# Mingrui-Yu/A-Simple-Stereo-SLAM-System-with-Deep-Loop-Closing

Measured on AMD Instinct MI355X. Metric: stereo frames/sec (ORB+match+LCD+BA-build) @1241x376, higher is better.
Workload: dtype u8/int32 (ORB, Hamming), f32 via f16x3 / bf16x6 split products on the matrix cores with f32 accumulate (CALC conv1 / conv2, DB scan), f64 (triangulation, BA)

## Files before the change

### a-simple-stereo-slam-system-with-deep-loop-closing_amd/csrc/orb_engine.hip

```cpp
#include <math.h>
#include <stdlib.h>
#include <string.h>

#include <vector>

#include "common.h"
#include "orb_plan.h"

namespace myslam_hip {

void launch_resize(const ResizeArgs& a, int batch, hipStream_t s);
void launch_resize_chain(const ResizeArgs* lv, int n, int batch, hipStream_t s);
bool resize_is_little(const ResizeArgs& a, int batch);
int resize_chain_max();
int pyr_head_levels();
void launch_pyr_head(const ResizeArgs* lv, int n, int rows, int cols, uint8_t* dst0, int dpitch0, size_t dstride0, int b0, int batch,
                     uint32_t* p0, int n0, uint32_t* p1, int n1, uint32_t* p2, int n2, uint32_t* p3, int n3, hipStream_t s);
void launch_blur(const BlurArgs& a, int batch, hipStream_t s);
bool blur_uses_strips(const BlurArgs& a);
bool resize_uses_strips(const ResizeArgs& a);
void launch_fast(const OrbPlan& P, const uint8_t* pyr, size_t pyrStride, const uint8_t* maskPyr, uint32_t* cand,
                 int32_t* candCount, const uint32_t* statPrev, uint32_t* statCur, int forceMode, int batch, hipStream_t s);
bool launch_octree(const OrbPlan& P, const uint32_t* cand, const int32_t* candCount, uint32_t* sortbuf, const uint32_t* octTab, uint32_t* selOut,
                   int32_t* selCount, int32_t* status, int batch, uint16_t* order, hipStream_t s, const BlurArgs* blurLv, int nBlur);
bool describe_uses_tile_order(bool have_order, int detectOnly, int batch);
void launch_describe(const OrbPlan& P, const uint8_t* pyr, const uint8_t* blur, size_t pyrStride, const uint32_t* selOut,
                     const int32_t* selCount, myslam_keypoint* kps, uint8_t* desc, int32_t* counts, int32_t* status,
                     int cap, int detectOnly, int batch, uint16_t* order, bool order_ready, int blocks_per_cu, hipStream_t s);
void launch_screen(const OrbPlan& P, const uint8_t* pyr, myslam_keypoint* kin, int n, myslam_keypoint* kout, uint8_t* keep,
                   hipStream_t s);
void launch_calc_desc(const OrbPlan& P, const uint8_t* blur, const myslam_keypoint* kps, int n, uint8_t* desc, hipStream_t s);
void launch_unpack_cands(const uint32_t* cand, int n, int32_t* xs, int32_t* ys, int32_t* sc, hipStream_t s);
void launch_blur_levels(const BlurArgs* lv, int n, int batch, hipStream_t s);
bool blur_mfma_tables(int w, int h, const int q[7], std::vector<uint4>& tab, size_t& offH, size_t& offV);
void blur_mfma_ident(std::vector<uint4>& tab, size_t& offI);
void launch_zero_u32(uint32_t* p0, int n0, uint32_t* p1, int n1, uint32_t* p2, int n2, uint32_t* p3, int n3, hipStream_t s);
void launch_ingest_clear(const uint8_t* src, int rows, int cols, int step, size_t sstride, uint8_t* dst, int dpitch, size_t dstride, int batch,
                         uint32_t* p0, int n0, uint32_t* p1, int n1, uint32_t* p2, int n2, uint32_t* p3, int n3, hipStream_t s);
void launch_ingest(const uint8_t* src, int rows, int cols, int step, size_t sstride, uint8_t* dst, int dpitch,
                   size_t dstride, int batch, hipStream_t s);

static inline int cv_round(float v) { return (int)lrintf(v); }
static inline size_t align_up(size_t v, size_t a) { return (v + a - 1) / a * a; }

void gauss_q8(int kind, int q[7]) {
    if (kind == 1) { const int t[7] = {8, 28, 56, 72, 56, 28, 8}; memcpy(q, t, sizeof(t)); return; }
    double g[7], sum = 0;
    for (int i = 0; i < 7; i++) { double x = i - 3; g[i] = exp(-(x * x) / 8.0); sum += g[i]; }
    for (int i = 0; i < 7; i++) q[i] = (int)lrint(g[i] / sum * 256.0);
}

[[maybe_unused]] static void resize_tables(int ssize, int dsize, bool is_x, std::vector<int32_t>& ofs, std::vector<int16_t>& coef) {
    const double inv_scale = (double)dsize / ssize;
    const double scale = 1. / inv_scale;
    ofs.resize(dsize); coef.resize(2 * dsize);
    for (int d = 0; d < dsize; d++) {
        float f = (float)((d + 0.5) * scale - 0.5);
        int s = (int)floorf(f);
        f -= s;
        if (is_x) {
            if (s < 0) { f = 0; s = 0; }
            if (s >= ssize - 1) { f = 0; s = ssize - 1; }
        }
        ofs[d] = s;
        coef[2 * d] = (int16_t)cv_round((1.f - f) * 2048.f);
        coef[2 * d + 1] = (int16_t)cv_round(f * 2048.f);
    }
}

template <typename T>
static int dev_alloc(T*& p, size_t n) {
    if (p) { (void)hipFree(p); p = nullptr; }
    if (n == 0) return MYSLAM_OK;
    MYSLAM_HIP_CHECK(hipMalloc((void**)&p, n * sizeof(T)));
    return MYSLAM_OK;
}

}

using namespace myslam_hip;

struct myslam_orb {
    int nfeatures, nlevels, iniTh, minTh;
    float scaleFactor;
    std::vector<float> scale, invScale;
    std::vector<int> nPerLevel;
    int umax[16];
    hipStream_t stream = nullptr;
    hipStream_t aux = nullptr;
    hipEvent_t evFork = nullptr, evJoin = nullptr;
    hipEvent_t evUserFast = nullptr;
    hipEvent_t evUserGate = nullptr;

    int rows = 0, cols = 0;
    OrbPlan full{}, det{};

    int batchCap = 0;
    bool maskAlloc = false;
    uint8_t *d_pyr = nullptr, *d_blur = nullptr, *d_mask = nullptr;
    uint32_t* d_cand = nullptr;
    uint32_t* d_sort = nullptr;
    int32_t *d_candCount = nullptr, *d_selCount = nullptr, *d_status = nullptr;
    uint32_t* d_sel = nullptr;
    uint16_t* d_order = nullptr;
    uint32_t* d_octTab = nullptr;
    uint32_t* d_stripTab = nullptr;
    uint32_t* d_fastStat = nullptr; int fastFlip = 0;
    int optFastMode = -1;
    int optInternalStream = 1;
    int optCopyInput = 0;
    int optStopAfter = 0;
    int tapsSet = 0, taps[7] = {0};
    int optSideBlocksPerCu = 0;
    int optBlurMfma = 0;
    uint4* d_blurTab = nullptr; bool blurTabValid = false; size_t blurOffI = 0, blurOffH[MAXL] = {0}, blurOffV[MAXL] = {0}; bool blurLvOk[MAXL] = {false}; int blurVconst = 0;
    int ensure_blur_tables();

    struct HostGraph { hipGraphExec_t exec = nullptr; hipGraph_t graph = nullptr; uint64_t gen = 0; int rows = 0, cols = 0, step = 0, dcap = 0, calls = 0; bool mask = false; };
    HostGraph hostGraph[2][2];
    uint64_t gen = 1;
    struct Clear { uint32_t* p[4]; int n[4]; } clr{{nullptr, nullptr, nullptr, nullptr}, {0, 0, 0, 0}};
    hipStream_t hostStream = nullptr;
    uint8_t* h_pin = nullptr; size_t pinBytes = 0;
    int ensure_pin(size_t bytes);
    void drop_host_graphs();
    uint8_t *d_stageImg = nullptr, *d_stageMask = nullptr; size_t stageImgBytes = 0, stageMaskBytes = 0;
    myslam_keypoint *d_stageKps = nullptr, *d_stageKps2 = nullptr; uint8_t* d_stageDesc = nullptr; uint8_t* d_stageKeep = nullptr;
    int32_t* d_stageCounts = nullptr; int stageCap = 0;
    uint8_t* d_stageOut = nullptr; size_t stageOutBytes = 0, stageDescOff = 0;

    int make_tables();
    int make_plan(int r, int c);
    int ensure(int batch, int r, int c, bool needMask);
    int ensure_stage(size_t imgBytes, size_t maskBytes, int cap);
    int build_pyramids(const uint8_t* d_imgs, int batch, int step, size_t stride, const uint8_t* d_masks, int nlev);
    ResizeArgs level_resize_args(uint8_t* base, int l) const;
    BlurArgs level_blur_args(int l) const;
    int blur_levels(int batch, int nlev, hipStream_t s);
    void fill_blur_args(BlurArgs* lv, int nlev) const;
    int run_fast(const OrbPlan& P, const uint8_t* maskPyr, int batch);
    int run_batch(const uint8_t* d_imgs, int batch, int r, int c, int step, size_t stride, const uint8_t* d_masks,
                  myslam_keypoint* d_kps, uint8_t* d_desc, int32_t* d_counts, int32_t* d_stat, int cap, bool detectOnly);
    void free_all();
};

int myslam_orb::make_tables() {
    scale.assign(nlevels, 1.f); invScale.assign(nlevels, 1.f); nPerLevel.assign(nlevels, 0);
    for (int i = 1; i < nlevels; i++) scale[i] = scale[i - 1] * scaleFactor;
    for (int i = 0; i < nlevels; i++) invScale[i] = 1.0f / scale[i];
    float factor = 1.0f / scaleFactor;
    float nDesired = nfeatures * (1 - factor) / (1 - (float)pow((double)factor, (double)nlevels));
    int sum = 0;
    for (int l = 0; l < nlevels - 1; l++) { nPerLevel[l] = cv_round(nDesired); sum += nPerLevel[l]; nDesired *= factor; }
    nPerLevel[nlevels - 1] = std::max(nfeatures - sum, 0);
    int v, v0, vmax = (int)floor(HALF_PATCH * sqrtf(2.f) / 2 + 1), vmin = (int)ceil(HALF_PATCH * sqrtf(2.f) / 2);
    const double hp2 = HALF_PATCH * HALF_PATCH;
    for (v = 0; v < 16; v++) umax[v] = 0;
    for (v = 0; v <= vmax; ++v) umax[v] = (int)lrint(sqrt(hp2 - v * v));
    for (v = HALF_PATCH, v0 = 0; v >= vmin; --v) { while (umax[v0] == umax[v0 + 1]) ++v0; umax[v] = v0; ++v0; }
    const int expect[16] = {15, 15, 15, 15, 14, 14, 14, 13, 13, 12, 11, 10, 9, 8, 6, 3};
    for (v = 0; v < 16; v++) if (umax[v] != expect[v]) return MYSLAM_ERR_INVALID;
    return MYSLAM_OK;
}

static int ceil_log2(int v) { int b = 0; while ((1 << b) < v) b++; return b; }

int myslam_orb::make_plan(int r, int c) {
    OrbPlan P{};
    P.nlevels = nlevels; P.rows = r; P.cols = c; P.iniTh = iniTh; P.minTh = minTh;
    size_t imgOff = 0, keyOff = 0; int cellBase = 0, outBase = 0, stripBase = 0;
    for (int l = 0; l < nlevels; l++) {
        LevelGeom& g = P.lv[l];
        g.w = cv_round((float)c * invScale[l]);
        g.h = cv_round((float)r * invScale[l]);
        if (g.w < 1 || g.h < 1) return MYSLAM_ERR_UNSUPPORTED;
        g.pitch = (int)align_up(g.w, 64);
        g.maxBX = g.w - EDGE_THRESHOLD + 3; g.maxBY = g.h - EDGE_THRESHOLD + 3;
        const float width = (float)(g.maxBX - MIN_BORDER), height = (float)(g.maxBY - MIN_BORDER);
        const float W = 30;
        g.nCols = (int)(width / W); g.nRows = (int)(height / W);
        if (g.nCols < 1 || g.nRows < 1) return MYSLAM_ERR_UNSUPPORTED;
        g.wCell = (int)ceilf(width / g.nCols); g.hCell = (int)ceilf(height / g.nRows);
        if (g.wCell > MAX_CELL || g.hCell > MAX_CELL) return MYSLAM_ERR_UNSUPPORTED;
        if (g.maxBX + 3 > 4095 + MIN_BORDER || g.maxBY + 3 > 4095 + MIN_BORDER) return MYSLAM_ERR_UNSUPPORTED;
        g.cellBase = cellBase; cellBase += g.nCols * g.nRows;
        g.stripBase = stripBase; stripBase += g.nRows * ((g.nCols + 3) / 4);
        g.N = nPerLevel[l];
        g.nIni = (int)roundf((float)(g.maxBX - MIN_BORDER) / (g.maxBY - MIN_BORDER));
        if (g.nIni < 1 || g.nIni > 64) return MYSLAM_ERR_UNSUPPORTED;
        g.hX = (float)(g.maxBX - MIN_BORDER) / g.nIni;
        const int rootW = (int)ceilf(g.hX) + 2, H = g.maxBY - MIN_BORDER;
        g.ndepth = std::min(MAX_DEPTH, ceil_log2(std::max(rootW, H)) + 2);
        g.sortDepth = 0;
        while (g.sortDepth + 1 <= g.ndepth && (g.nIni << (2 * (g.sortDepth + 1))) <= 1024) g.sortDepth++;
        g.keyCap = (int)std::min<size_t>(262143, std::max<size_t>(256, (size_t)((g.w + 1) / 2) * ((g.h + 1) / 2)));
        g.nodeCap = (std::max(g.N + 4, 4 * g.nIni + 4) + 3) & ~3;
        if (g.nodeCap > 4092) return MYSLAM_ERR_UNSUPPORTED;
        g.outBase = outBase; outBase += g.nodeCap;
        g.scale = scale[l];
        g.scaledPatch = (float)(int)(PATCH_SIZE * scale[l]);
        g.imgOff = imgOff; imgOff += align_up((size_t)g.pitch * align_up((size_t)g.h, 8), 256);
        g.keyOff = keyOff; keyOff += g.keyCap;
    }
    for (int l = 0; l < MAXL; l++) P.stripBaseOf[l] = l < P.nlevels ? P.lv[l].stripBase : INT32_MAX;
    P.ncells = cellBase; P.nstrips = stripBase; P.totalKeyCap = (int)keyOff; P.totalOut = outBase; P.pyrBytes = imgOff;
    {
        std::vector<uint32_t> tab;
        for (int l = 0; l < nlevels; l++) {
            LevelGeom& g = P.lv[l];
            g.tabX = g.maxBX - MIN_BORDER + 8; g.tabY = g.maxBY - MIN_BORDER + 8; g.tabOff = (int)tab.size();
            tab.resize(tab.size() + 2 * (size_t)(g.tabX + g.tabY), 0u);
            uint32_t* xcode = tab.data() + g.tabOff; uint32_t* ycode = xcode + g.tabX;
            uint32_t* xcell = ycode + g.tabY; uint32_t* ycell = xcell + g.tabX;
            for (int px = 0; px < g.tabX; px++) {
                int r = (int)((float)px / g.hX);
                r = std::min(std::max(r, 0), g.nIni - 1);
                int UL = (int)(g.hX * (float)r), UR = (int)(g.hX * (float)(r + 1));
                uint32_t code = (uint32_t)r << ROOT_SHIFT;
                for (int k = 1; k <= g.ndepth; k++) {
                    const int mid = UL + ((UR - UL + 1) >> 1);
                    const uint32_t d = px >= mid;
                    code |= d << (ROOT_SHIFT - 2 * k);
                    if (d) UL = mid; else UR = mid;
                }
                xcode[px] = code;
                xcell[px] = (uint32_t)(std::max(px - 3, 0) / g.wCell);
            }
            for (int py = 0; py < g.tabY; py++) {
                int UL = 0, BR = g.maxBY - MIN_BORDER;
                uint32_t code = 0;
                for (int k = 1; k <= g.ndepth; k++) {
                    const int mid = UL + ((BR - UL + 1) >> 1);
                    const uint32_t d = py >= mid;
                    code |= (d << 1) << (ROOT_SHIFT - 2 * k);
                    if (d) UL = mid; else BR = mid;
                }
                ycode[py] = code;
                ycell[py] = (uint32_t)((std::max(py - 3, 0) / g.hCell) * g.nCols);
            }
        }
        int rc = dev_alloc(d_octTab, tab.size());
        if (rc) return rc;
        if ((rc = upload_table(d_octTab, tab.data(), tab.size() * sizeof(uint32_t)))) return rc;
    }
    {
        std::vector<uint32_t> st((size_t)P.nstrips * 8, 0u);
        for (int l = 0; l < nlevels; l++) {
            const LevelGeom& g = P.lv[l];
            const int spr = (g.nCols + 3) / 4;
            for (int strip = 0; strip < g.nRows * spr; strip++) {
                uint32_t* e = st.data() + (size_t)(g.stripBase + strip) * 8;
                const int ci = strip / spr, cj0 = (strip - ci * spr) * 4;
                const int iniY = MIN_BORDER + ci * g.hCell;
                int ncell = 0, pairs = 0; uint32_t wcs = 0; int hr = 0;
                if (iniY < g.maxBY - 3) {
                    hr = std::min(iniY + g.hCell + 6, g.maxBY) - iniY;
                    const int hc = hr - 6;
                    if (hc > 0)
                        for (int c = 0; c < 4; c++) {
                            const int cj = cj0 + c, iniX = MIN_BORDER + cj * g.wCell;
                            int wc = 0;
                            if (cj < g.nCols && iniX < g.maxBX - 6) wc = std::max(0, std::min(iniX + g.wCell + 6, g.maxBX) - iniX - 6);
                            if (wc > 0) ncell = c + 1;
                            wcs |= (uint32_t)wc << (8 * c);
                            pairs += ((wc + 1) >> 1) * hc;
                        }
                }
                if (ncell == 0) wcs = 0;
                e[0] = (uint32_t)l | ((uint32_t)ci << 8) | ((uint32_t)cj0 << 16) | ((uint32_t)ncell << 24);
                e[1] = (uint32_t)iniY | ((uint32_t)hr << 16);
                e[2] = (uint32_t)(MIN_BORDER + cj0 * g.wCell) | ((uint32_t)g.wCell << 16);
                e[3] = wcs; e[4] = (uint32_t)g.pitch; e[5] = (uint32_t)pairs;
                e[6] = (uint32_t)(g.imgOff & 0xffffffffu); e[7] = (uint32_t)(g.imgOff >> 32);
            }
        }
        int rc = dev_alloc(d_stripTab, st.size());
        if (rc) return rc;
        if ((rc = upload_table(d_stripTab, st.data(), st.size() * sizeof(uint32_t)))) return rc;
        P.stripTab = d_stripTab;
    }
    full = P;
    det = P;
    det.nlevels = 1;
    det.ncells = P.lv[0].nCols * P.lv[0].nRows;
    det.nstrips = P.lv[0].nRows * ((P.lv[0].nCols + 3) / 4);
    det.lv[0].N = nfeatures;
    det.lv[0].nodeCap = (std::max(nfeatures + 4, 4 * P.lv[0].nIni + 4) + 3) & ~3;
    if (det.lv[0].nodeCap > 4092) return MYSLAM_ERR_UNSUPPORTED;
    det.lv[0].outBase = 0;
    det.totalOut = det.lv[0].nodeCap;
    rows = r; cols = c;
    return MYSLAM_OK;
}

int myslam_orb::ensure(int batch, int r, int c, bool needMask) {
    if (r != rows || c != cols) {
        MYSLAM_HIP_CHECK(hipStreamSynchronize(stream));
        int rc = make_plan(r, c);
        if (rc) { rows = cols = 0; return rc; }
        batchCap = 0; gen++; blurTabValid = false;
    }
    const int detOut = det.totalOut;
    const size_t selPer = (size_t)std::max(full.totalOut, detOut);
    if (batch > batchCap) {
        MYSLAM_HIP_CHECK(hipStreamSynchronize(stream));
        gen++;
        int rc;
        if ((rc = dev_alloc(d_pyr, (size_t)batch * full.pyrBytes + 64))) return rc;
        if ((rc = dev_alloc(d_blur, (size_t)batch * full.pyrBytes + 4096))) return rc;
        if ((rc = dev_alloc(d_cand, (size_t)batch * full.totalKeyCap))) return rc;
        if ((rc = dev_alloc(d_sort, (size_t)batch * full.totalKeyCap * 2))) return rc;
        if ((rc = dev_alloc(d_candCount, (size_t)batch * MAXL))) return rc;
        if ((rc = dev_alloc(d_selCount, (size_t)batch * MAXL))) return rc;
        if ((rc = dev_alloc(d_status, (size_t)batch))) return rc;
        if ((rc = dev_alloc(d_sel, (size_t)batch * selPer))) return rc;
        if ((rc = dev_alloc(d_order, (size_t)batch * selPer))) return rc;
        if ((rc = dev_alloc(d_mask, 0))) return rc;
        maskAlloc = false;
        batchCap = batch;
    }
    if (needMask && !maskAlloc) {
        int rc = dev_alloc(d_mask, (size_t)batchCap * full.pyrBytes + 64);
        if (rc) return rc;
        maskAlloc = true;
    }
    return MYSLAM_OK;
}

int myslam_orb::build_pyramids(const uint8_t* d_imgs, int batch, int step, size_t stride, const uint8_t* d_masks, int nlev) {
    const OrbPlan& P = full;
    for (int pass = 0; pass < (d_masks ? 2 : 1); pass++) {
        uint8_t* base = pass ? d_mask : d_pyr;
        const uint8_t* src = pass ? d_masks : d_imgs;
        const int n0 = pass ? 0 : P.ext0N;
        int l = 1;
        const int nhead = std::min(pyr_head_levels(), nlev - 1);
        if (nhead >= 1 && batch > n0 && (size_t)batch * P.lv[1].w * P.lv[1].h < (size_t)1500000) {
            ScopedProf sp(P_RESIZE, stream);
            ResizeArgs grp[3];
            for (int j = 0; j < nhead; j++) grp[j] = level_resize_args(base, 1 + j);
            grp[0].src = src; grp[0].spitch = step; grp[0].sstride = stride;
            const bool c0 = pass == 0 && clr.n[0] > 0;
            launch_pyr_head(grp, nhead, P.rows, P.cols, base + P.lv[0].imgOff, P.lv[0].pitch, P.pyrBytes, n0, batch,
                            c0 ? clr.p[0] : nullptr, c0 ? clr.n[0] : 0, c0 ? clr.p[1] : nullptr, c0 ? clr.n[1] : 0, c0 ? clr.p[2] : nullptr,
                            c0 ? clr.n[2] : 0, c0 ? clr.p[3] : nullptr, c0 ? clr.n[3] : 0, stream);
            if (c0) clr.n[0] = 0;
            l = 1 + nhead;
        } else if (batch > n0) {
            uint8_t* dst0 = base + (size_t)n0 * P.pyrBytes + P.lv[0].imgOff;
            if (pass == 0 && clr.n[0] > 0) {
                launch_ingest_clear(src + (size_t)n0 * stride, P.rows, P.cols, step, stride, dst0, P.lv[0].pitch, P.pyrBytes, batch - n0,
                                    clr.p[0], clr.n[0], clr.p[1], clr.n[1], clr.p[2], clr.n[2], clr.p[3], clr.n[3], stream);
                clr.n[0] = 0;
            } else {
                launch_ingest(src + (size_t)n0 * stride, P.rows, P.cols, step, stride, dst0, P.lv[0].pitch, P.pyrBytes, batch - n0, stream);
            }
        }
        for (; l < nlev;) {
            ScopedProf sp(P_RESIZE, stream);
            ResizeArgs a = level_resize_args(base, l);
            if (l == 1 && n0 > 0) { a.src0 = d_imgs; a.spitch0 = step; a.sstride0 = stride; a.n0 = n0; }
            ResizeArgs grp[4]; int ng = 0;
            const int gmax = resize_chain_max();
            if (gmax > 1 && resize_is_little(a, batch)) {
                static const double kEvals[4] = {1, 5, 21, 85};
                double evals = (double)batch * a.dw * a.dh;
                grp[ng++] = a;
                while (ng < gmax && l + ng < nlev) {
                    const ResizeArgs nx = level_resize_args(base, l + ng);
                    evals += (double)batch * nx.dw * nx.dh * kEvals[ng];
                    if (!resize_is_little(nx, batch) || evals > 6e6) break;
                    grp[ng++] = nx;
                }
            }
            if (ng > 1) { launch_resize_chain(grp, ng, batch, stream); l += ng; }
            else { launch_resize(a, batch, stream); l++; }
        }
    }
    return MYSLAM_OK;
}
ResizeArgs myslam_orb::level_resize_args(uint8_t* base, int l) const {
    const OrbPlan& P = full;
    ResizeArgs a;
    a.src = base + P.lv[l - 1].imgOff; a.sw = P.lv[l - 1].w; a.sh = P.lv[l - 1].h; a.spitch = P.lv[l - 1].pitch; a.sstride = P.pyrBytes;
    a.src0 = nullptr; a.spitch0 = 0; a.n0 = 0; a.sstride0 = 0;
    a.dst = base + P.lv[l].imgOff; a.dw = P.lv[l].w; a.dh = P.lv[l].h; a.dpitch = P.lv[l].pitch; a.dstride = P.pyrBytes;
    a.scale_x = 1. / ((double)a.dw / a.sw); a.scale_y = 1. / ((double)a.dh / a.sh);
    return a;
}
int myslam_orb::ensure_blur_tables() {
    if (blurTabValid) return MYSLAM_OK;
    std::vector<uint4> tab;
    int q[7];
    if (tapsSet) memcpy(q, taps, sizeof(q)); else gauss_q8(0, q);
    int sum = 0;
    for (int t = 0; t < 7; t++) sum += q[t];
    blurVconst = sum * 128 * sum + 32768;
    blur_mfma_ident(tab, blurOffI);
    for (int l = 0; l < full.nlevels; l++) blurLvOk[l] = blur_mfma_tables(full.lv[l].w, full.lv[l].h, q, tab, blurOffH[l], blurOffV[l]);
    MYSLAM_HIP_CHECK(hipStreamSynchronize(stream));
    int rc = dev_alloc(d_blurTab, tab.size());
    if (rc) return rc;
    if ((rc = upload_table(d_blurTab, tab.data(), tab.size() * sizeof(uint4)))) return rc;
    blurTabValid = true; gen++;
    return MYSLAM_OK;
}

BlurArgs myslam_orb::level_blur_args(int l) const {
    const OrbPlan& P = full;
    BlurArgs a;
    a.src = d_pyr + P.lv[l].imgOff; a.dst = d_blur + P.lv[l].imgOff;
    a.w = P.lv[l].w; a.h = P.lv[l].h; a.spitch = a.dpitch = P.lv[l].pitch; a.sstride = a.dstride = P.pyrBytes;
    a.src0 = nullptr; a.spitch0 = 0; a.n0 = 0; a.sstride0 = 0;
    a.dtiled = 1;
    if (tapsSet) memcpy(a.q, taps, sizeof(taps)); else gauss_q8(0, a.q);
    if (optBlurMfma && blurTabValid && blurLvOk[l]) { a.tabH = d_blurTab + blurOffH[l]; a.tabV = d_blurTab + blurOffV[l]; a.ident = d_blurTab + blurOffI; a.vconst = blurVconst; }
    return a;
}
void myslam_orb::fill_blur_args(BlurArgs* lv, int nlev) const {
    const OrbPlan& P = full;
    for (int l = 0; l < nlev; l++) {
        lv[l] = level_blur_args(l);
        if (l == 0 && P.ext0N > 0) { lv[l].src0 = P.ext0; lv[l].spitch0 = P.ext0Pitch; lv[l].sstride0 = P.ext0Stride; lv[l].n0 = P.ext0N; }
    }
}
int myslam_orb::blur_levels(int batch, int nlev, hipStream_t stream) {
    BlurArgs lv[MAXL];
    fill_blur_args(lv, nlev);
    ScopedProf sp(P_BLUR, stream);
    launch_blur_levels(lv, nlev, batch, stream);
    return MYSLAM_OK;
}

int myslam_orb::run_batch(const uint8_t* d_imgs, int batch, int r, int c, int step, size_t stride, const uint8_t* d_masks,
                          myslam_keypoint* d_kps, uint8_t* d_desc, int32_t* d_counts, int32_t* d_stat, int cap, bool detectOnly) {
    if (!d_imgs || batch <= 0 || r <= 0 || c <= 0 || step < c || cap <= 0 || !d_kps || !d_counts) return MYSLAM_ERR_INVALID;
    if (!detectOnly && !d_desc) return MYSLAM_ERR_INVALID;
    int rc = ensure(batch, r, c, d_masks != nullptr);
    if (rc) return rc;
    if (optBlurMfma && !detectOnly && (rc = ensure_blur_tables())) return rc;
    const OrbPlan& P = detectOnly ? det : full;
    int32_t* stat = d_stat ? d_stat : d_status;
    if (!d_fastStat) {
        MYSLAM_HIP_CHECK(hipMalloc((void**)&d_fastStat, sizeof(uint32_t) * 2 * MAXL * 4));
        MYSLAM_HIP_CHECK(hipMemsetAsync(d_fastStat, 0, sizeof(uint32_t) * 2 * MAXL * 4, stream));
    }
    clr = {{reinterpret_cast<uint32_t*>(d_candCount), reinterpret_cast<uint32_t*>(d_selCount), reinterpret_cast<uint32_t*>(stat), d_fastStat + (size_t)fastFlip * MAXL * 4},
           {batch * MAXL, batch * MAXL, batch, MAXL * 4}};
    const int stop = optStopAfter;
    {
        int n0 = 0;
        if (!optCopyInput && stop == 0 && batch > 1 && full.nlevels >= 1 && stride >= (size_t)r * (size_t)step) {
            bool ok = blur_uses_strips(level_blur_args(0));
            if (full.nlevels > 1) ok = ok && resize_uses_strips(level_resize_args(d_pyr, 1));
            if (ok) n0 = batch - 1;
        }
        full.ext0 = det.ext0 = d_imgs; full.ext0Stride = det.ext0Stride = stride; full.ext0Pitch = det.ext0Pitch = step; full.ext0N = det.ext0N = n0;
    }
    if (stop == 1) {
        launch_ingest_clear(d_imgs, full.rows, full.cols, step, stride, d_pyr + full.lv[0].imgOff, full.lv[0].pitch, full.pyrBytes, batch,
                            clr.p[0], clr.n[0], clr.p[1], clr.n[1], clr.p[2], clr.n[2], clr.p[3], clr.n[3], stream);
        clr.n[0] = 0;
        return MYSLAM_OK;
    }
    if ((rc = build_pyramids(d_imgs, batch, step, stride, d_masks, P.nlevels))) return rc;
    if (stop == 2) return MYSLAM_OK;
    hipStreamCaptureStatus capst = hipStreamCaptureStatusNone;
    if (stream && hipStreamIsCapturing(stream, &capst) != hipSuccess) { (void)hipGetLastError(); capst = hipStreamCaptureStatusNone; }
    const int aux_mode = capst == hipStreamCaptureStatusActive ? 0 : optInternalStream;
    const bool fork = aux_mode > 0 && !detectOnly && stop == 0;
    if (fork && !aux) {
        MYSLAM_HIP_CHECK(hipStreamCreateWithFlags(&aux, hipStreamNonBlocking));
        MYSLAM_HIP_CHECK(hipEventCreateWithFlags(&evFork, hipEventDisableTiming));
        MYSLAM_HIP_CHECK(hipEventCreateWithFlags(&evJoin, hipEventDisableTiming));
    }
    auto fork_blur = [&]() -> int {
        MYSLAM_HIP_CHECK(hipEventRecord(evFork, stream));
        MYSLAM_HIP_CHECK(hipStreamWaitEvent(aux, evFork, 0));
        int rc2 = blur_levels(batch, P.nlevels, aux);
        if (rc2) return rc2;
        MYSLAM_HIP_CHECK(hipEventRecord(evJoin, aux));
        return MYSLAM_OK;
    };
    if (fork && aux_mode == 2 && (rc = fork_blur())) return rc;
    if (evUserGate) MYSLAM_HIP_CHECK(hipStreamWaitEvent(stream, evUserGate, 0));
    if ((rc = run_fast(P, d_masks ? d_mask : nullptr, batch))) return rc;
    if (evUserFast) MYSLAM_HIP_CHECK(hipEventRecord(evUserFast, stream));
    if (fork && aux_mode != 2 && (rc = fork_blur())) return rc;
    bool blurred = false;
    {
        ScopedProf sp(P_OCTREE, stream);
        BlurArgs blv[MAXL];
        const bool tryBlur = !fork && !detectOnly && stop == 0 && !optBlurMfma;
        if (tryBlur) fill_blur_args(blv, P.nlevels);
        blurred = launch_octree(P, d_cand, d_candCount, d_sort, d_octTab, d_sel, d_selCount, stat, batch,
                                describe_uses_tile_order(d_order != nullptr, detectOnly ? 1 : 0, batch) ? d_order : nullptr, stream,
                                tryBlur ? blv : nullptr, tryBlur ? P.nlevels : 0);
    }
    if (stop == 3) return MYSLAM_OK;
    if (fork) MYSLAM_HIP_CHECK(hipStreamWaitEvent(stream, evJoin, 0));
    else if (!detectOnly && !blurred && (rc = blur_levels(batch, P.nlevels, stream))) return rc;
    if (stop == 4) return MYSLAM_OK;
    {
        ScopedProf sp(P_DESC, stream);
        launch_describe(P, d_pyr, d_blur, full.pyrBytes, d_sel, d_selCount, d_kps, d_desc, d_counts, stat, cap,
                        detectOnly ? 1 : 0, batch, d_order, true, optSideBlocksPerCu, stream);
    }
    MYSLAM_HIP_CHECK(hipGetLastError());
    return MYSLAM_OK;
}

int myslam_orb::run_fast(const OrbPlan& P, const uint8_t* maskPyr, int batch) {
    uint32_t* cur = d_fastStat + (size_t)fastFlip * MAXL * 4;
    const uint32_t* prev = d_fastStat + (size_t)(fastFlip ^ 1) * MAXL * 4;
    fastFlip ^= 1;
    ScopedProf sp(P_FAST, stream);
    launch_fast(P, d_pyr, full.pyrBytes, maskPyr, d_cand, d_candCount, prev, cur, optFastMode, batch, stream);
    return MYSLAM_OK;
}

int myslam_orb::ensure_pin(size_t bytes) {
    if (bytes <= pinBytes) return MYSLAM_OK;
    if (h_pin) { (void)hipHostFree(h_pin); h_pin = nullptr; pinBytes = 0; }
    gen++;
    const size_t want = (bytes + (bytes >> 2) + 4095) & ~(size_t)4095;
    MYSLAM_HIP_CHECK(hipHostMalloc((void**)&h_pin, want));
    pinBytes = want;
    return MYSLAM_OK;
}

void myslam_orb::drop_host_graphs() {
    for (auto& row : hostGraph)
        for (auto& g : row) { if (g.exec) (void)hipGraphExecDestroy(g.exec); if (g.graph) (void)hipGraphDestroy(g.graph); g = HostGraph(); }
}

int myslam_orb::ensure_stage(size_t imgBytes, size_t maskBytes, int cap) {
    if (imgBytes > stageImgBytes) { gen++; int rc = dev_alloc(d_stageImg, imgBytes); if (rc) return rc; stageImgBytes = imgBytes; }
    if (maskBytes > stageMaskBytes) { gen++; int rc = dev_alloc(d_stageMask, maskBytes); if (rc) return rc; stageMaskBytes = maskBytes; }
    if (cap > stageCap) {
        gen++;
        int rc;
        const size_t oK = 256, oD = oK + (((size_t)cap * sizeof(myslam_keypoint) + 255) & ~(size_t)255), total = oD + (size_t)cap * 32;
        if ((rc = dev_alloc(d_stageOut, total))) return rc;
        stageOutBytes = total; stageDescOff = oD;
        d_stageCounts = reinterpret_cast<int32_t*>(d_stageOut);
        d_stageKps = reinterpret_cast<myslam_keypoint*>(d_stageOut + oK);
        d_stageDesc = d_stageOut + oD;
        if ((rc = dev_alloc(d_stageKps2, (size_t)cap))) return rc;
        if ((rc = dev_alloc(d_stageKeep, (size_t)cap))) return rc;
        stageCap = cap;
    }
    return MYSLAM_OK;
}

void myslam_orb::free_all() {
    void* ptrs[] = {d_blurTab, d_fastStat, d_octTab, d_stripTab, d_pyr, d_blur, d_mask, d_cand, d_sort, d_candCount, d_selCount, d_status, d_sel, d_order, d_stageImg, d_stageMask,
                    d_stageOut, d_stageKps2, d_stageKeep};
    for (void* p : ptrs) if (p) (void)hipFree(p);
    if (aux) { (void)hipStreamSynchronize(aux); (void)hipStreamDestroy(aux); (void)hipEventDestroy(evFork); (void)hipEventDestroy(evJoin); aux = nullptr; }
    drop_host_graphs();
    if (hostStream) { (void)hipStreamSynchronize(hostStream); (void)hipStreamDestroy(hostStream); hostStream = nullptr; }
    if (h_pin) { (void)hipHostFree(h_pin); h_pin = nullptr; pinBytes = 0; }
}

extern "C" {

int myslam_orb_create(myslam_orb** out, int nfeatures, float scale_factor, int nlevels, int ini_th_fast, int min_th_fast) {
    if (!out || nfeatures < 1 || nlevels < 1 || nlevels > MAXL || !(scale_factor > 1.0f) || ini_th_fast < 0 ||
        min_th_fast < 1 || min_th_fast > ini_th_fast || ini_th_fast > 255 || scale_factor > 2.5f)
        return MYSLAM_ERR_INVALID;
    int ndev = 0;
    if (hipGetDeviceCount(&ndev) != hipSuccess || ndev < 1) return MYSLAM_ERR_HIP;
    myslam_orb* h = new myslam_orb();
    h->nfeatures = nfeatures; h->scaleFactor = scale_factor; h->nlevels = nlevels; h->iniTh = ini_th_fast; h->minTh = min_th_fast;
    int rc = h->make_tables();
    if (rc) { delete h; return rc; }
    *out = h;
    return MYSLAM_OK;
}

int myslam_orb_destroy(myslam_orb* h) {
    if (!h) return MYSLAM_ERR_INVALID;
    (void)hipStreamSynchronize(h->stream);
    h->free_all();
    delete h;
    return MYSLAM_OK;
}

int myslam_orb_set_stream(myslam_orb* h, void* s) {
    if (!h) return MYSLAM_ERR_INVALID;
    (void)hipStreamSynchronize(h->stream);
    h->stream = (hipStream_t)s; h->gen++;
    return MYSLAM_OK;
}

int myslam_orb_set_fast_event(myslam_orb* h, void* ev) {
    if (!h) return MYSLAM_ERR_INVALID;
    h->evUserFast = (hipEvent_t)ev; h->gen++;
    return MYSLAM_OK;
}

int myslam_orb_set_fast_gate(myslam_orb* h, void* ev) {
    if (!h) return MYSLAM_ERR_INVALID;
    h->evUserGate = (hipEvent_t)ev; h->gen++;
    return MYSLAM_OK;
}

int myslam_orb_set_option(myslam_orb* h, int option, int value) {
    if (!h) return MYSLAM_ERR_INVALID;
    h->gen++;
    switch (option) {
        case MYSLAM_ORB_OPT_FAST_MODE: if (value < -1 || value > 1) return MYSLAM_ERR_INVALID; h->optFastMode = value; return MYSLAM_OK;
        case MYSLAM_ORB_OPT_INTERNAL_STREAM: if (value < 0 || value > 2) return MYSLAM_ERR_INVALID; h->optInternalStream = value; return MYSLAM_OK;
        case MYSLAM_ORB_OPT_COPY_INPUT: if (value < 0 || value > 1) return MYSLAM_ERR_INVALID; h->optCopyInput = value; return MYSLAM_OK;
        case MYSLAM_ORB_OPT_STOP_AFTER: if (value < 0 || value > 4) return MYSLAM_ERR_INVALID; h->optStopAfter = value; return MYSLAM_OK;
        case MYSLAM_ORB_OPT_BLUR_MFMA: if (value < 0 || value > 1) return MYSLAM_ERR_INVALID; h->optBlurMfma = value; return MYSLAM_OK;
        case MYSLAM_ORB_OPT_SIDE_BLOCKS_PER_CU: if (value < 0 || value > 64) return MYSLAM_ERR_INVALID; h->optSideBlocksPerCu = value; return MYSLAM_OK;
    }
    return MYSLAM_ERR_INVALID;
}

int myslam_orb_set_gauss_taps(myslam_orb* h, const int32_t* q7) {
    if (!h) return MYSLAM_ERR_INVALID;
    h->blurTabValid = false;
    if (!q7) { h->tapsSet = 0; h->gen++; return MYSLAM_OK; }
    int sum = 0;
    for (int i = 0; i < 7; i++) { if (q7[i] < 0 || q7[i] > 255) return MYSLAM_ERR_INVALID; sum += q7[i]; }
    if (sum < 1 || sum > 257) return MYSLAM_ERR_INVALID;
    for (int i = 0; i < 7; i++) h->taps[i] = q7[i];
    h->tapsSet = 1; h->gen++;
    return MYSLAM_OK;
}

int myslam_orb_get_tables(const myslam_orb* h, float* scale, float* inv_scale, int* fpl, int* umax16) {
    if (!h) return MYSLAM_ERR_INVALID;
    for (int i = 0; i < h->nlevels; i++) {
        if (scale) scale[i] = h->scale[i];
        if (inv_scale) inv_scale[i] = h->invScale[i];
        if (fpl) fpl[i] = h->nPerLevel[i];
    }
    if (umax16) for (int i = 0; i < 16; i++) umax16[i] = h->umax[i];
    return MYSLAM_OK;
}

int myslam_orb_max_keypoints(const myslam_orb* h) {
    if (!h) return MYSLAM_ERR_INVALID;
    int s = 0;
    for (int l = 0; l < h->nlevels; l++) s += std::max(h->nPerLevel[l] + 3, 32);
    return std::max(s, std::max(h->nfeatures + 3, 32));
}

int myslam_orb_max_keypoints_for(const myslam_orb* h, int rows, int cols) {
    if (!h || rows < 1 || cols < 1) return MYSLAM_ERR_INVALID;
    int s = 0, first = 0;
    for (int l = 0; l < h->nlevels; l++) {
        const int w = cv_round((float)cols * h->invScale[l]), hh = cv_round((float)rows * h->invScale[l]);
        const int bx = w - EDGE_THRESHOLD + 3 - MIN_BORDER, by = hh - EDGE_THRESHOLD + 3 - MIN_BORDER;
        const int nIni = (bx > 0 && by > 0) ? std::max(1, (int)roundf((float)bx / (float)by)) : 1;
        s += std::max(h->nPerLevel[l] + 3, 4 * nIni);
        if (l == 0) first = std::max(h->nfeatures + 3, 4 * nIni);
    }
    return std::max(std::max(s, first), 32);
}

int myslam_orb_detect_and_compute_batch(myslam_orb* h, const uint8_t* d_imgs, int batch, int rows, int cols, int step,
                                        size_t img_stride, const uint8_t* d_masks, myslam_keypoint* d_kps, uint8_t* d_desc,
                                        int32_t* d_counts, int32_t* d_status, int cap) {
    if (!h) return MYSLAM_ERR_INVALID;
    return h->run_batch(d_imgs, batch, rows, cols, step, img_stride, d_masks, d_kps, d_desc, d_counts, d_status, cap, false);
}

int myslam_orb_detect_batch(myslam_orb* h, const uint8_t* d_imgs, int batch, int rows, int cols, int step, size_t img_stride,
                            const uint8_t* d_masks, myslam_keypoint* d_kps, int32_t* d_counts, int32_t* d_status, int cap) {
    if (!h) return MYSLAM_ERR_INVALID;
    return h->run_batch(d_imgs, batch, rows, cols, step, img_stride, d_masks, d_kps, nullptr, d_counts, d_status, cap, true);
}

static int host_extract(myslam_orb* h, const uint8_t* img, int rows, int cols, int step, const uint8_t* mask, int mask_step,
                        myslam_keypoint* kps, uint8_t* desc, int cap, int* n, bool detectOnly) {
    if (!h || !n) return MYSLAM_ERR_INVALID;
    *n = 0;
    if (!img || rows <= 0 || cols <= 0) return MYSLAM_OK;
    if (detectOnly && !mask) {  }
    if (step < cols || cap <= 0 || !kps || (!detectOnly && !desc)) return MYSLAM_ERR_INVALID;
    if (mask && mask_step < cols) return MYSLAM_ERR_INVALID;
    int rc = h->ensure(1, rows, cols, mask != nullptr);
    if (rc) return rc;
    if (mask && mask_step != step) return MYSLAM_ERR_INVALID;
    const int dcap = std::max(cap, std::max(h->full.totalOut, h->det.totalOut));
    const size_t imgBytes = (size_t)rows * step, maskBytes = mask ? imgBytes : 0;
    if ((rc = h->ensure_stage(imgBytes, maskBytes, dcap))) return rc;
    if (h->optBlurMfma && !detectOnly && (rc = h->ensure_blur_tables())) return rc;
    const size_t oOut = (imgBytes + maskBytes + 255) & ~(size_t)255, oCnt = oOut, oKps = oOut + 256, oDesc = oOut + h->stageDescOff;
    const size_t outBytes = detectOnly ? 256 + sizeof(myslam_keypoint) * (size_t)dcap : h->stageDescOff + (size_t)32 * dcap;
    if ((rc = h->ensure_pin(oOut + h->stageOutBytes))) return rc;
    hipStream_t caller = h->stream;
    if (!caller) {
        if (!h->hostStream) { MYSLAM_HIP_CHECK(hipStreamCreateWithFlags(&h->hostStream, hipStreamNonBlocking)); h->gen++; }
        MYSLAM_HIP_CHECK(hipStreamSynchronize(nullptr));
    }
    hipStream_t hs = caller ? caller : h->hostStream;
    struct Swap { myslam_orb* h; hipStream_t keep; ~Swap() { h->stream = keep; } } swap{h, caller};
    h->stream = hs;
    memcpy(h->h_pin, img, imgBytes);
    if (mask) memcpy(h->h_pin + imgBytes, mask, maskBytes);
    auto enqueue = [&]() -> int {
        MYSLAM_HIP_CHECK(hipMemcpyAsync(h->d_stageImg, h->h_pin, imgBytes, hipMemcpyHostToDevice, hs));
        if (mask) MYSLAM_HIP_CHECK(hipMemcpyAsync(h->d_stageMask, h->h_pin + imgBytes, maskBytes, hipMemcpyHostToDevice, hs));
        int r2 = h->run_batch(h->d_stageImg, 1, rows, cols, step, imgBytes, mask ? h->d_stageMask : nullptr,
                              h->d_stageKps, h->d_stageDesc, h->d_stageCounts, h->d_stageCounts + 1, dcap, detectOnly);
        if (r2) return r2;
        MYSLAM_HIP_CHECK(hipMemcpyAsync(h->h_pin + oOut, h->d_stageOut, outBytes, hipMemcpyDeviceToHost, hs));
        return MYSLAM_OK;
    };
    const bool graphable = !prof_is_on() && !h->evUserGate && !h->evUserFast && h->optStopAfter == 0;
    myslam_orb::HostGraph& G = h->hostGraph[detectOnly ? 1 : 0][h->fastFlip & 1];
    const bool same = G.gen == h->gen && G.rows == rows && G.cols == cols && G.step == step && G.dcap == dcap && G.mask == (mask != nullptr);
    if (!same) { if (G.exec) (void)hipGraphExecDestroy(G.exec); if (G.graph) (void)hipGraphDestroy(G.graph); G = myslam_orb::HostGraph(); G.gen = h->gen; G.rows = rows; G.cols = cols; G.step = step; G.dcap = dcap; G.mask = mask != nullptr; }
    bool done = false;
    if (graphable && G.exec) {
        if (hipGraphLaunch(G.exec, hs) == hipSuccess) { h->fastFlip ^= 1; done = true; }
        else { (void)hipGetLastError(); (void)hipGraphExecDestroy(G.exec); G.exec = nullptr; if (G.graph) { (void)hipGraphDestroy(G.graph); G.graph = nullptr; } G.calls = -1000000; }
    } else if (graphable && G.calls >= 1) {
        const int flip0 = h->fastFlip;
        if (hipStreamBeginCapture(hs, hipStreamCaptureModeThreadLocal) == hipSuccess) {
            const int r2 = enqueue();
            hipGraph_t graph = nullptr;
            const hipError_t e = hipStreamEndCapture(hs, &graph);
            if (r2 == MYSLAM_OK && e == hipSuccess && graph && hipGraphInstantiate(&G.exec, graph, nullptr, nullptr, 0) == hipSuccess &&
                hipGraphLaunch(G.exec, hs) == hipSuccess) {
                done = true; G.graph = graph;
            } else {
                (void)hipGetLastError();
                if (G.exec) { (void)hipGraphExecDestroy(G.exec); G.exec = nullptr; }
                if (graph) (void)hipGraphDestroy(graph);
                G.calls = -1000000; h->fastFlip = flip0;
            }
        } else {
            (void)hipGetLastError(); G.calls = -1000000;
        }
    }
    if (!done && (rc = enqueue())) return rc;
    G.calls++;
    MYSLAM_HIP_CHECK(hipStreamSynchronize(hs));
    int32_t res[2];
    memcpy(res, h->h_pin + oCnt, sizeof(res));
    if (res[1] != 0) return res[1];
    if (res[0] > cap) { *n = res[0]; return MYSLAM_ERR_CAPACITY; }
    memcpy(kps, h->h_pin + oKps, sizeof(myslam_keypoint) * (size_t)res[0]);
    if (!detectOnly) memcpy(desc, h->h_pin + oDesc, (size_t)32 * res[0]);
    *n = res[0];
    return MYSLAM_OK;
}

int myslam_orb_detect_and_compute(myslam_orb* h, const uint8_t* img, int rows, int cols, int step, const uint8_t* mask,
                                  int mask_step, myslam_keypoint* kps, uint8_t* desc, int cap, int* n) {
    return host_extract(h, img, rows, cols, step, mask, mask_step, kps, desc, cap, n, false);
}

int myslam_orb_detect(myslam_orb* h, const uint8_t* img, int rows, int cols, int step, const uint8_t* mask, int mask_step,
                      myslam_keypoint* kps, int cap, int* n) {
    return host_extract(h, img, rows, cols, step, mask, mask_step, kps, nullptr, cap, n, true);
}

static int host_pyramid(myslam_orb* h, const uint8_t* img, int rows, int cols, int step, int ncap) {
    int rc = h->ensure(1, rows, cols, false);
    if (rc) return rc;
    if ((rc = h->ensure_stage((size_t)rows * step, 0, ncap))) return rc;
    MYSLAM_HIP_CHECK(hipMemcpyAsync(h->d_stageImg, img, (size_t)rows * step, hipMemcpyHostToDevice, h->stream));
    h->full.ext0N = h->det.ext0N = 0;
    return h->build_pyramids(h->d_stageImg, 1, step, (size_t)rows * step, nullptr, h->nlevels);
}

int myslam_orb_screen_and_compute_params(myslam_orb* h, const uint8_t* img, int rows, int cols, int step,
                                         myslam_keypoint* kps_in, int n_in, myslam_keypoint* kps_out, int cap, int* n_out) {
    if (!h || !n_out) return MYSLAM_ERR_INVALID;
    *n_out = 0;
    if (!img || rows <= 0 || cols <= 0 || n_in <= 0) return MYSLAM_OK;
    if (!kps_in || !kps_out || step < cols) return MYSLAM_ERR_INVALID;
    for (int i = 0; i < n_in; i++) if (kps_in[i].octave < 0 || kps_in[i].octave >= h->nlevels) return MYSLAM_ERR_INVALID;
    int rc = host_pyramid(h, img, rows, cols, step, n_in);
    if (rc) return rc;
    MYSLAM_HIP_CHECK(hipMemcpyAsync(h->d_stageKps, kps_in, sizeof(myslam_keypoint) * n_in, hipMemcpyHostToDevice, h->stream));
    {
        ScopedProf sp(P_SCREEN, h->stream);
        launch_screen(h->full, h->d_pyr, h->d_stageKps, n_in, h->d_stageKps2, h->d_stageKeep, h->stream);
    }
    std::vector<myslam_keypoint> tmp(n_in);
    std::vector<uint8_t> keep(n_in);
    MYSLAM_HIP_CHECK(hipMemcpyAsync(kps_in, h->d_stageKps, sizeof(myslam_keypoint) * n_in, hipMemcpyDeviceToHost, h->stream));
    MYSLAM_HIP_CHECK(hipMemcpyAsync(tmp.data(), h->d_stageKps2, sizeof(myslam_keypoint) * n_in, hipMemcpyDeviceToHost, h->stream));
    MYSLAM_HIP_CHECK(hipMemcpyAsync(keep.data(), h->d_stageKeep, n_in, hipMemcpyDeviceToHost, h->stream));
    MYSLAM_HIP_CHECK(hipStreamSynchronize(h->stream));
    int m = 0;
    for (int i = 0; i < n_in; i++)
        if (keep[i]) { if (m >= cap) return MYSLAM_ERR_CAPACITY; kps_out[m++] = tmp[i]; }
    *n_out = m;
    return MYSLAM_OK;
}

int myslam_orb_calc_descriptors(myslam_orb* h, const uint8_t* img, int rows, int cols, int step, const myslam_keypoint* kps,
                                int n, uint8_t* desc) {
    if (!h) return MYSLAM_ERR_INVALID;
    if (!img || rows <= 0 || cols <= 0 || n <= 0) return MYSLAM_OK;
    if (!kps || !desc || step < cols) return MYSLAM_ERR_INVALID;
    for (int i = 0; i < n; i++) if (kps[i].octave < 0 || kps[i].octave >= h->nlevels) return MYSLAM_ERR_INVALID;
    int rc = host_pyramid(h, img, rows, cols, step, n);
    if (rc) return rc;
    if ((rc = h->blur_levels(1, h->nlevels, h->stream))) return rc;
    MYSLAM_HIP_CHECK(hipMemcpyAsync(h->d_stageKps, kps, sizeof(myslam_keypoint) * n, hipMemcpyHostToDevice, h->stream));
    {
        ScopedProf sp(P_DESC, h->stream);
        launch_calc_desc(h->full, h->d_blur, h->d_stageKps, n, h->d_stageDesc, h->stream);
    }
    MYSLAM_HIP_CHECK(hipMemcpyAsync(desc, h->d_stageDesc, (size_t)32 * n, hipMemcpyDeviceToHost, h->stream));
    MYSLAM_HIP_CHECK(hipStreamSynchronize(h->stream));
    return MYSLAM_OK;
}

static int download_tiled_plane(const uint8_t* d_plane, const LevelGeom& g, uint8_t* out, int out_step, hipStream_t stream) {
    std::vector<uint8_t> tmp((size_t)g.pitch * align_up((size_t)g.h, 8));
    MYSLAM_HIP_CHECK(hipMemcpyAsync(tmp.data(), d_plane, tmp.size(), hipMemcpyDeviceToHost, stream));
    MYSLAM_HIP_CHECK(hipStreamSynchronize(stream));
    for (int y = 0; y < g.h; y++)
        for (int x = 0; x < g.w; x++) out[(size_t)y * out_step + x] = tmp[tiled_off(x, y, g.pitch)];
    return MYSLAM_OK;
}

int myslam_orb_debug_pyramid(myslam_orb* h, const uint8_t* img, int rows, int cols, int step, int level, int blurred,
                             uint8_t* out, int out_step, int* w, int* hgt) {
    if (!h || !img || level < 0 || level >= h->nlevels) return MYSLAM_ERR_INVALID;
    int rc = host_pyramid(h, img, rows, cols, step, 16);
    if (rc) return rc;
    if (blurred && (rc = h->blur_levels(1, h->nlevels, h->stream))) return rc;
    const LevelGeom& g = h->full.lv[level];
    if (w) *w = g.w;
    if (hgt) *hgt = g.h;
    if (out) {
        if (out_step < g.w) return MYSLAM_ERR_INVALID;
        if (blurred) return download_tiled_plane(h->d_blur + g.imgOff, g, out, out_step, h->stream);
        MYSLAM_HIP_CHECK(hipMemcpy2DAsync(out, out_step, h->d_pyr + g.imgOff, g.pitch, g.w, g.h, hipMemcpyDeviceToHost, h->stream));
    }
    MYSLAM_HIP_CHECK(hipStreamSynchronize(h->stream));
    return MYSLAM_OK;
}

int myslam_orb_debug_candidates(myslam_orb* h, const uint8_t* img, int rows, int cols, int step, const uint8_t* mask,
                                int mask_step, int level, int32_t* xs, int32_t* ys, int32_t* scores, int cap, int* n) {
    if (!h || !img || !n || level < 0 || level >= h->nlevels) return MYSLAM_ERR_INVALID;
    if (mask && mask_step != step) return MYSLAM_ERR_INVALID;
    int rc = h->ensure(1, rows, cols, mask != nullptr);
    if (rc) return rc;
    if ((rc = h->ensure_stage((size_t)rows * step, mask ? (size_t)rows * step : 0, 16))) return rc;
    MYSLAM_HIP_CHECK(hipMemcpyAsync(h->d_stageImg, img, (size_t)rows * step, hipMemcpyHostToDevice, h->stream));
    if (mask) MYSLAM_HIP_CHECK(hipMemcpyAsync(h->d_stageMask, mask, (size_t)rows * step, hipMemcpyHostToDevice, h->stream));
    if (!h->d_fastStat) {
        MYSLAM_HIP_CHECK(hipMalloc((void**)&h->d_fastStat, sizeof(uint32_t) * 2 * MAXL * 4));
        MYSLAM_HIP_CHECK(hipMemsetAsync(h->d_fastStat, 0, sizeof(uint32_t) * 2 * MAXL * 4, h->stream));
    }
    launch_zero_u32(reinterpret_cast<uint32_t*>(h->d_candCount), MAXL, h->d_fastStat + (size_t)h->fastFlip * MAXL * 4, MAXL * 4, nullptr, 0, nullptr, 0, h->stream);
    h->full.ext0N = h->det.ext0N = 0;
    if ((rc = h->build_pyramids(h->d_stageImg, 1, step, (size_t)rows * step, mask ? h->d_stageMask : nullptr, h->nlevels))) return rc;
    if ((rc = h->run_fast(h->full, mask ? h->d_mask : nullptr, 1))) return rc;
    int32_t counts[MAXL];
    MYSLAM_HIP_CHECK(hipMemcpyAsync(counts, h->d_candCount, sizeof(counts), hipMemcpyDeviceToHost, h->stream));
    MYSLAM_HIP_CHECK(hipStreamSynchronize(h->stream));
    const LevelGeom& g = h->full.lv[level];
    *n = counts[level];
    if (counts[level] > g.keyCap || counts[level] > cap) return MYSLAM_ERR_CAPACITY;
    int32_t* d_tmp = nullptr;
    const int m = counts[level];
    if (m > 0) {
        MYSLAM_HIP_CHECK(hipMalloc((void**)&d_tmp, sizeof(int32_t) * 3 * m));
        launch_unpack_cands(h->d_cand + g.keyOff, m, d_tmp, d_tmp + m, d_tmp + 2 * m, h->stream);
        MYSLAM_HIP_CHECK(hipMemcpyAsync(xs, d_tmp, 4 * m, hipMemcpyDeviceToHost, h->stream));
        MYSLAM_HIP_CHECK(hipMemcpyAsync(ys, d_tmp + m, 4 * m, hipMemcpyDeviceToHost, h->stream));
        MYSLAM_HIP_CHECK(hipMemcpyAsync(scores, d_tmp + 2 * m, 4 * m, hipMemcpyDeviceToHost, h->stream));
        MYSLAM_HIP_CHECK(hipStreamSynchronize(h->stream));
        (void)hipFree(d_tmp);
    }
    return MYSLAM_OK;
}

int myslam_orb_debug_readback(myslam_orb* h, int what, int b, int level, void* out, size_t cap_bytes, int detect_plan) {
    if (!h || !out || h->rows == 0 || b < 0 || b >= h->batchCap || level < 0 || level >= h->nlevels) return MYSLAM_ERR_INVALID;
    MYSLAM_HIP_CHECK(hipStreamSynchronize(h->stream));
    const OrbPlan& P = detect_plan ? h->det : h->full;
    const LevelGeom& g = P.lv[level];
    switch (what) {
        case 0: case 1: {
            if (cap_bytes < (size_t)g.w * g.h) return MYSLAM_ERR_CAPACITY;
            const uint8_t* base = (what ? h->d_blur : h->d_pyr) + (size_t)b * h->full.pyrBytes + g.imgOff;
            if (what) return download_tiled_plane(base, g, static_cast<uint8_t*>(out), g.w, h->stream);
            MYSLAM_HIP_CHECK(hipMemcpy2D(out, g.w, base, g.pitch, g.w, g.h, hipMemcpyDeviceToHost));
            return MYSLAM_OK;
        }
        case 2: case 4: {
            if (cap_bytes < 4) return MYSLAM_ERR_CAPACITY;
            MYSLAM_HIP_CHECK(hipMemcpy(out, (what == 2 ? h->d_candCount : h->d_selCount) + b * MAXL + level, 4, hipMemcpyDeviceToHost));
            return MYSLAM_OK;
        }
        case 3: {
            if (cap_bytes < (size_t)g.keyCap * 4) return MYSLAM_ERR_CAPACITY;
            MYSLAM_HIP_CHECK(hipMemcpy(out, h->d_cand + (size_t)b * P.totalKeyCap + g.keyOff, (size_t)g.keyCap * 4, hipMemcpyDeviceToHost));
            return MYSLAM_OK;
        }
        case 6: {
            if (cap_bytes < 16) return MYSLAM_ERR_CAPACITY;
            if (!h->d_fastStat) return MYSLAM_ERR_INVALID;
            MYSLAM_HIP_CHECK(hipMemcpy(out, h->d_fastStat + ((size_t)(h->fastFlip ^ 1) * MAXL + level) * 4, 16, hipMemcpyDeviceToHost));
            return MYSLAM_OK;
        }
        case 5: {
            if (cap_bytes < (size_t)g.nodeCap * 4) return MYSLAM_ERR_CAPACITY;
            MYSLAM_HIP_CHECK(hipMemcpy(out, h->d_sel + (size_t)b * P.totalOut + g.outBase, (size_t)g.nodeCap * 4, hipMemcpyDeviceToHost));
            return MYSLAM_OK;
        }
    }
    return MYSLAM_ERR_INVALID;
}

}
```

### a-simple-stereo-slam-system-with-deep-loop-closing_amd/csrc/orb_kernels.hip

```cpp
#include <stdio.h>
#include <stdlib.h>

#include <type_traits>

#include "common.h"
#include "orb_plan.h"

namespace myslam_hip {

typedef unsigned short u16x2 __attribute__((ext_vector_type(2)));

#ifdef MYSLAM_BLOCK_TRACE
__device__ unsigned long long* g_bt_buf = nullptr;
__device__ unsigned int g_bt_cap = 0, g_bt_n = 0;
struct BlockTrace {
    unsigned long long t0 = 0, marks = 0, aux = 0; int kid; unsigned hw = 0; bool on = false;
    __device__ __forceinline__ void mark(int i) {
        if (on) marks |= ((__builtin_amdgcn_s_memrealtime() - t0) & 0xffffull) << (16 * i);
    }
    __device__ __forceinline__ BlockTrace(int kid_) : kid(kid_) {
        if (threadIdx.x != 0 || g_bt_buf == nullptr) return;
        const unsigned xcc = __builtin_amdgcn_s_getreg((3 << 11) | 20) & 0xf;
        if (xcc != 0) return;
        hw = __builtin_amdgcn_s_getreg((31 << 11) | 4);
// ... 708 lines not shown
    auto pick = [&](int row, int a) -> s16x2 {
        const int d0 = a >> 2, d1 = ((a & 3) == 3) ? d0 + 1 : d0;
        const uint32_t u = __builtin_amdgcn_perm(r[row][d1], r[row][d0],
                                                 0x0c000c00u | ((((a & 3) == 3) ? 4u : (uint32_t)(a & 3) + 1u) << 16) | (uint32_t)(a & 3));
        s16x2 q; __builtin_memcpy(&q, &u, 4);
        return q;
    };
    const s16x2 vv = pick(ROW + 3, xc);
    s16x2 p[16];
#pragma unroll
    for (int i = 0; i < 16; i++) p[i] = pick(ROW + 3 + RY[i], xc + RX[i]);
#if MYSLAM_FAST_PHASE == 3
    { s16x2 x = vv ^ thv; for (int i = 0; i < 16; i++) x = x ^ p[i]; return x; }
#endif
    s16x2 n2[8], x2[8], n4[8], x4[8], ub[8], ud[8];
#pragma unroll
    for (int k = 0; k < 8; k++) { n2[k] = pmin(p[2 * k], p[2 * k + 1]); x2[k] = pmax(p[2 * k], p[2 * k + 1]); }
#pragma unroll
    for (int k = 0; k < 8; k++) { n4[k] = pmin(n2[k], n2[(k + 1) & 7]); x4[k] = pmax(x2[k], x2[(k + 1) & 7]); }
#pragma unroll
    for (int k = 0; k < 8; k++) {
        const s16x2 a = p[(2 * k + 8) & 15], c = p[(2 * k + 15) & 15];
        ub[k] = pmin3(n4[k], n4[(k + 2) & 7], pmax(a, c));
        ud[k] = pmax3(x4[k], x4[(k + 2) & 7], pmin(a, c));
    }
    const s16x2 brt = pmax(pmax3(pmax3(ub[0], ub[1], ub[2]), pmax3(ub[3], ub[4], ub[5]), ub[6]), ub[7]);
    const s16x2 drk = pmin(pmin3(pmin3(ud[0], ud[1], ud[2]), pmin3(ud[3], ud[4], ud[5]), ud[6]), ud[7]);
    const s16x2 sraw = pmax(brt - vv, vv - drk);
    return pmax(sraw, thv) - thv;
}

template <int A>
__device__ __forceinline__ s16x2 pick16(uint32_t lo, uint32_t hi) {
    const uint32_t u = __builtin_amdgcn_perm(hi, lo, 0x0c000c00u | ((uint32_t)(A + 1) << 16) | (uint32_t)A);
    s16x2 q; __builtin_memcpy(&q, &u, 4);
    return q;
}

__device__ __forceinline__ bool fast9_compass_pair(s16x2 v, s16x2 p0, s16x2 p4, s16x2 p8, s16x2 p12, s16x2 thv) {
    const s16x2 dmin = pmin(pmin(pmax(p0, p4), pmax(p4, p8)), pmin(pmax(p8, p12), pmax(p12, p0)));
    const s16x2 bmax = pmax(pmax(pmin(p0, p4), pmin(p4, p8)), pmax(pmin(p8, p12), pmin(p12, p0)));
    const s16x2 t1 = (v - thv) - dmin;
    const s16x2 t2 = bmax - (v + thv);
    const s16x2 zero = {0, 0};
    const s16x2 m = pmax(pmax(t1, t2), zero);
    uint32_t u; __builtin_memcpy(&u, &m, 4);
    return u != 0;
}

template <int PAIR, int ROW = 0, int NR = 3>
__device__ __forceinline__ int nms_pair(const uint32_t (&m)[NR][3], uint32_t& zc) {
    constexpr int x = 4 + 2 * PAIR;
    auto pick = [&](int row, int a) -> s16x2 {
        const int d0 = a >> 2, d1 = ((a & 3) == 3) ? d0 + 1 : d0;
        const uint32_t u = __builtin_amdgcn_perm(m[row][d1], m[row][d0],
                                                 0x0c000c00u | ((((a & 3) == 3) ? 4u : (uint32_t)(a & 3) + 1u) << 16) | (uint32_t)(a & 3));
        s16x2 q; __builtin_memcpy(&q, &u, 4);
        return q;
    };
    const s16x2 c = pick(ROW + 1, x);
    s16x2 nb = pmax(pick(ROW, x - 1), pick(ROW, x));
    nb = pmax(nb, pick(ROW, x + 1));
    nb = pmax(nb, pmax(pick(ROW + 1, x - 1), pick(ROW + 1, x + 1)));
    nb = pmax(nb, pmax(pick(ROW + 2, x - 1), pick(ROW + 2, x)));
    nb = pmax(nb, pick(ROW + 2, x + 1));
    const s16x2 d = c - nb;
    __builtin_memcpy(&zc, &c, 4);
    return ((int)d.x > 0 ? 1 : 0) | ((int)d.y > 0 ? 2 : 0);
}

struct NmsRow { s16x2 hA, hB, lrA, lrB, cA, cB; };
__device__ __forceinline__ NmsRow nms_row(uint32_t d0, uint32_t d1, uint32_t d2) {
    const s16x2 pm1 = pick16<3>(d0, d1), p0 = pick16<0>(d1, d1), p1 = pick16<1>(d1, d1), p2 = pick16<2>(d1, d1), p3 = pick16<3>(d1, d2);
    NmsRow r;
    r.lrA = pmax(pm1, p1); r.hA = pmax(r.lrA, p0);
    r.lrB = pmax(p1, p3);  r.hB = pmax(r.lrB, p2);
    r.cA = p0; r.cB = p2;
    return r;
}
struct NmsRowH { s16x2 hA, hB; };
__device__ __forceinline__ NmsRowH nms_row_h(uint32_t d0, uint32_t d1, uint32_t d2) {
    const s16x2 pm1 = pick16<3>(d0, d1), p0 = pick16<0>(d1, d1), p1 = pick16<1>(d1, d1), p2 = pick16<2>(d1, d1), p3 = pick16<3>(d1, d2);
    NmsRowH r;
    r.hA = pmax3(pm1, p0, p1); r.hB = pmax3(p1, p2, p3);
    return r;
}
typedef unsigned short u16x2 __attribute__((ext_vector_type(2)));
template <class RU, class RD>
__device__ __forceinline__ uint32_t nms_strict4(const RU& U, const NmsRow& M, const RD& D, u16x2& zacc) {
    auto keep = [](s16x2 c, s16x2 nb) -> s16x2 {
        u16x2 cu, nu; __builtin_memcpy(&cu, &c, 4); __builtin_memcpy(&nu, &nb, 4);
        const u16x2 t = __builtin_elementwise_sub_sat(cu, nu);
        const u16x2 k = __builtin_elementwise_min(cu, (u16x2)(t << (unsigned short)8));
        s16x2 ks; __builtin_memcpy(&ks, &k, 4);
        return ks;
    };
    const s16x2 ka = keep(M.cA, pmax3(U.hA, D.hA, M.lrA)), kb = keep(M.cB, pmax3(U.hB, D.hB, M.lrB));
    s16x2 zs; __builtin_memcpy(&zs, &zacc, 4);
    zs = pmax3(zs, ka, kb);
    __builtin_memcpy(&zacc, &zs, 4);
    uint32_t za, zb; __builtin_memcpy(&za, &ka, 4); __builtin_memcpy(&zb, &kb, 4);
    return __builtin_amdgcn_perm(zb, za, 0x06040200u);
}

__device__ __forceinline__ int wave_incl_scan_dpp(int v) {
    v += __builtin_amdgcn_update_dpp(0, v, 0x111, 0xf, 0xf, false);
    v += __builtin_amdgcn_update_dpp(0, v, 0x112, 0xf, 0xf, false);
    v += __builtin_amdgcn_update_dpp(0, v, 0x114, 0xf, 0xf, false);
    v += __builtin_amdgcn_update_dpp(0, v, 0x118, 0xf, 0xf, false);
    v += __builtin_amdgcn_update_dpp(0, v, 0x142, 0xa, 0xf, false);
    v += __builtin_amdgcn_update_dpp(0, v, 0x143, 0xc, 0xf, false);
    return v;
}

__device__ __forceinline__ int rank_below(unsigned long long ballot, int acc) {
    return (int)__builtin_amdgcn_mbcnt_hi((uint32_t)(ballot >> 32), __builtin_amdgcn_mbcnt_lo((uint32_t)ballot, (uint32_t)acc));
}

struct FastCtl { const uint32_t* prev; uint32_t* cur; int force; };

#ifndef MYSLAM_FAST_LDS_BLOCK
#define MYSLAM_FAST_LDS_BLOCK (163840 / 6 - 128)
#endif
#ifndef MYSLAM_FAST_BLOCKS_PER_CU
#define MYSLAM_FAST_BLOCKS_PER_CU 6
#endif
#ifndef MYSLAM_FAST_MS_BLOCKS_PER_CU
#define MYSLAM_FAST_MS_BLOCKS_PER_CU 5
#endif
template <int CW, int G, int CH, int NS = 1>
struct FastLds {
    static constexpr int CP = (CW + 6 + 15) & ~15, TP = G * CP, TROWS = CH + 6 + 1, SP = (CW + 4 + 8 + 3) & ~3, SROWS = CH + 2 + 4;
    static constexpr int NPAIR = G * CH * ((CW + 1) / 2);
    static constexpr int EST = (NS > 1 ? 2 : 1) * (TROWS * TP + 16) + G * (SROWS * SP + 16) + 2 * NPAIR + (NS > 1 ? 128 : 64);
    static constexpr int BLOCKS = NS > 1 ? MYSLAM_FAST_MS_BLOCKS_PER_CU : MYSLAM_FAST_BLOCKS_PER_CU;
    static constexpr int BLOCK = NS > 1 ? 163840 / MYSLAM_FAST_MS_BLOCKS_PER_CU - 128 : MYSLAM_FAST_LDS_BLOCK;
    static constexpr int PAD = (CW <= 32 && EST < (NS > 1 ? BLOCK : 163840 / 7)) ? BLOCK - EST : 0;
    static_assert(CW > 32 || (BLOCKS * (EST + PAD) <= 163840 && (BLOCKS + 1) * (EST + PAD) > 163840), "exactly BLOCKS blocks per CU");
};
#ifndef MYSLAM_FAST_WAVES_PER_EU
#define MYSLAM_FAST_WAVES_PER_EU 6
#endif
#ifndef MYSLAM_FAST_NS
#define MYSLAM_FAST_NS 1
#endif
#ifdef MYSLAM_FAST_NUM_VGPR
#define MYSLAM_FAST_VGPR_ATTR __attribute__((amdgpu_num_vgpr(MYSLAM_FAST_NUM_VGPR)))
#else
#define MYSLAM_FAST_VGPR_ATTR
#endif
template <int CW, int G, int CH = CW, int NS = 1>
__global__ __launch_bounds__(256) __attribute__((amdgpu_waves_per_eu(CW <= 40 ? MYSLAM_FAST_WAVES_PER_EU : 3))) MYSLAM_FAST_VGPR_ATTR void k_fast_strip(OrbPlan P, const uint8_t* __restrict__ pyr, size_t pyrStride,
                                                    const uint8_t* __restrict__ maskPyr,
                                                    uint32_t* __restrict__ cand, int32_t* __restrict__ candCount, FastCtl ctl, int batch) {
    constexpr int T = 256;
    constexpr int CP = (CW + 6 + 15) & ~15;
    constexpr int TP = G * CP;
    constexpr int NQC = CP / 16;
    constexpr int TROWS = CH + 6 + 1;
    constexpr int SP = (CW + 4 + 8 + 3) & ~3;
    constexpr int SROWS = CH + 2 + 4;
    constexpr int NLIST = G * ((CW + 1) / 2) * ((CH + 1) / 2);
    constexpr int NPAIR = G * CH * ((CW + 1) / 2);
    static_assert(CW <= 63 && CH <= 63 && G <= 4, "pair list entry = cell << 11 | row << 5 | pair index");
    constexpr int NB2 = NS > 1 ? 2 : 1;
    static_assert(NS == 1 || (CW <= 32 && G == 4 && MYSLAM_FAST_PHASE == 0), "the multi-strip form exists for the usual plans' instance only");
    __shared__ __attribute__((aligned(16))) uint8_t s_tile0[TROWS * TP + 16];
    extern __shared__ __attribute__((aligned(16))) uint8_t s_dyn[];
    __shared__ __attribute__((aligned(16))) uint8_t s_score[G][SROWS * SP + 16];
    __shared__ uint16_t s_pairs[NPAIR];
    static_assert(NLIST * 5 <= TROWS * TP, "maxima list must fit into the staged tile");
    static_assert(NLIST * 4 <= TROWS * TP && NLIST <= NPAIR, "row records must fit");
    __shared__ int s_ini2[NB2][G], s_wc2[NB2][G], s_cnt2[NB2][4];
    static_assert(FastLds<CW, G, CH, NS>::CP == CP && FastLds<CW, G, CH, NS>::TROWS == TROWS && FastLds<CW, G, CH, NS>::SP == SP && FastLds<CW, G, CH, NS>::SROWS == SROWS && FastLds<CW, G, CH, NS>::NPAIR == NPAIR,
                  "FastLds restates this kernel's LDS arrays");

    const int nwg = gridDim.x, bid = blockIdx.x;
    const int xq = nwg >> 3, xr = nwg & 7, xcd = bid & 7;
    const int logical = (xcd < xr ? xcd * (xq + 1) : xr * (xq + 1) + (xcd - xr) * xq) + (bid >> 3);
    MYSLAM_BT(0);
    int a_nstrips = P.nstrips, a_batch = batch, a_ext0N = P.ext0N, a_ext0Pitch = P.ext0Pitch;
    size_t a_ext0Stride = P.ext0Stride, a_pyrStride = pyrStride;
    uintptr_t a_ext0i = (uintptr_t)P.ext0, a_pyri = (uintptr_t)pyr, a_tabi = (uintptr_t)P.stripTab;
    asm volatile("" : "+s"(a_nstrips), "+s"(a_batch), "+s"(a_ext0N), "+s"(a_ext0Pitch), "+s"(a_ext0Stride), "+s"(a_pyrStride), "+s"(a_ext0i), "+s"(a_pyri), "+s"(a_tabi));
    typedef const uint8_t __attribute__((address_space(1))) * GlobalU8;
    const GlobalU8 a_ext0 = (GlobalU8)a_ext0i, a_pyr = (GlobalU8)a_pyri;
    const int total_strips = a_nstrips * a_batch;
    const int gs_first = logical * NS, gs_end = min(gs_first + NS, total_strips);
    if (gs_first >= total_strips) return;
    typedef const uint32_t __attribute__((address_space(4))) * ConstU32;
    struct StripRec { uint32_t t[8]; int b; };
    auto load_rec = [&](int gs) __attribute__((always_inline)) -> StripRec {
        StripRec r;
        r.b = gs / a_nstrips;
        const int sidx = gs - r.b * a_nstrips;
        const ConstU32 tb = (ConstU32)(a_tabi + (uintptr_t)sidx * 32);
        uint32_t t0 = tb[0], t1 = tb[1], t2 = tb[2], t3 = tb[3], t4 = tb[4], t5 = tb[5], t6 = tb[6], t7 = tb[7];
        asm volatile("" : "+s"(t0), "+s"(t1), "+s"(t2), "+s"(t3), "+s"(t4), "+s"(t5), "+s"(t6), "+s"(t7));
        r.t[0] = t0; r.t[1] = t1; r.t[2] = t2; r.t[3] = t3; r.t[4] = t4; r.t[5] = t5; r.t[6] = t6; r.t[7] = t7;
        return r;
    };
    auto issue_tile = [&](const StripRec& r, int q, int tid) __attribute__((always_inline)) {
        const int level = (int)(r.t[0] & 0xffu), hr = (int)(r.t[1] >> 16), iniY = (int)(r.t[1] & 0xffffu), iniX0 = (int)(r.t[2] & 0xffffu), wCell = (int)(r.t[2] >> 16);
        const bool ext = level == 0 && r.b < a_ext0N;
        const uint8_t* img = (const uint8_t*)(ext ? a_ext0 + (size_t)r.b * a_ext0Stride : a_pyr + (size_t)r.b * a_pyrStride + ((size_t)r.t[6] | ((size_t)r.t[7] << 32)));
        const int ipitch = ext ? a_ext0Pitch : (int)r.t[4];
        const uint32_t lds = (uint32_t)__builtin_amdgcn_readfirstlane((int)(uint32_t)(uintptr_t)(q ? &s_dyn[0] : &s_tile0[0])) + 1024u * (uint32_t)__builtin_amdgcn_readfirstlane(tid >> 6);
#pragma unroll
        for (int j = 0; j < (TROWS * 12 + 255) / 256; j++) {
            const int pc = 256 * j + tid;
            const int rr = pc / 12, col = pc - 12 * rr, c = col / 3, k = col - 3 * c;
            const int x = min(iniX0 + c * wCell + 16 * k, ipitch - 16);
            const uint8_t* src = img + (size_t)(iniY + min(rr, hr - 1)) * ipitch + x;
            const uint32_t d = lds + 4096u * (uint32_t)j;
            uint32_t keep;
            if (pc < TROWS * 12)
                asm volatile("s_mov_b32 %0, m0\n\ts_mov_b32 m0, %2\n\ts_nop 0\n\tglobal_load_lds_dwordx4 %1, off\n\ts_mov_b32 m0, %0" : "=&s"(keep) : "v"(src), "s"(d) : "memory");
        }
    };
    StripRec rec = load_rec(gs_first);
    if constexpr (NS > 1) {
        static_assert(NS == 1 || (G * ((CW + 6 + 15) / 16) == 12), "a tile row of the multi-strip form is 12 pieces");
        if ((rec.t[0] >> 24) != 0) issue_tile(rec, 0, (int)threadIdx.x);
    }
    int par = 0;
    bool fresh = true;
  for (int gs = gs_first; gs < gs_end; gs++) {
    int tid_ = threadIdx.x;
    if constexpr (NS > 1) asm volatile("" : "+v"(tid_));
    const int tid = tid_;
    uint8_t* const s_tile = (NS > 1 && par) ? s_dyn : s_tile0;
    uint32_t* const s_list = reinterpret_cast<uint32_t*>(s_tile);
    uint8_t* const s_listc = s_tile + 4 * NLIST;
    uint32_t* const s_recz = reinterpret_cast<uint32_t*>(s_tile);
    int* const s_ini = s_ini2[par];
    int* const s_wc = s_wc2[par];
    int& s_nlist = s_cnt2[par][0]; int& s_npair = s_cnt2[par][1]; int& s_ncorner = s_cnt2[par][2];
    const int b = rec.b;
    StripRec rec_next = rec;
    if constexpr (NS > 1) { if (gs + 1 < gs_end) rec_next = load_rec(gs + 1); }
    const bool sampled = gs % max(1, total_strips >> 12) == 0;
    const uint4 e0 = make_uint4(rec.t[0], rec.t[1], rec.t[2], rec.t[3]), e1 = make_uint4(rec.t[4], rec.t[5], rec.t[6], rec.t[7]);
    const int level = (int)(e0.x & 0xffu), ci = (int)((e0.x >> 8) & 0xffu), cj0 = (int)((e0.x >> 16) & 0xffu), ncell = (int)(e0.x >> 24);
    if (ncell == 0) { rec = rec_next; if constexpr (NS > 1) { if (gs + 1 < gs_end && (rec.t[0] >> 24) != 0) { issue_tile(rec, par, tid); fresh = true; } } continue; }
    const int iniY = (int)(e0.y & 0xffffu), hr = (int)(e0.y >> 16), hc = hr - 6;
    const int iniX0 = (int)(e0.z & 0xffffu), t_wCell = (int)(e0.z >> 16);
    const int pairs_total = (int)e1.y;
    if (tid < G) s_wc[tid] = (int)((e0.w >> (8 * tid)) & 0xffu);
    auto wc_of = [&](int c) __attribute__((always_inline)) -> int { return s_wc[c]; };
    const bool ext = level == 0 && b < a_ext0N;
    const uint8_t* img = (const uint8_t*)(ext ? a_ext0 + (size_t)b * a_ext0Stride : a_pyr + (size_t)b * a_pyrStride + ((size_t)e1.z | ((size_t)e1.w << 32)));
    const int ipitch = ext ? a_ext0Pitch : (int)e1.x;
    const LevelGeom g = P.lv[level];
    bool dense = false;
    auto prep = [&]() __attribute__((always_inline)) {
        {
            constexpr int NB = G * (SROWS * SP + 16), NV = NB / 16;
            for (int i = tid; i < NV; i += T) reinterpret_cast<uint4*>(&s_score[0][0])[i] = make_uint4(0, 0, 0, 0);
            if (NB % 16 != 0 && tid < (NB - 16 * NV) / 4) reinterpret_cast<uint32_t*>(&s_score[0][0])[4 * NV + tid] = 0;
        }
        if (tid < G) s_ini[tid] = 0;
        if (tid == 0) { s_nlist = 0; s_npair = 0; s_ncorner = 0; }
        {
            typedef const uint32_t __attribute__((address_space(4))) * ConstStat;
            const ConstStat pv = (ConstStat)((uintptr_t)ctl.prev + (uintptr_t)level * 16);
            const uint32_t pv0 = pv[0], pv1 = pv[1], pv2 = pv[2];
            const float ps = (float)pv0, pt = (float)pv1;
            const bool was_dense = pv2 != 0;
            dense = ctl.force >= 0 ? ctl.force != 0 : (pt > 0.f && (was_dense ? ps > 0.165f * pt : ps > 0.41f * pt));
        }
    };
    MYSLAM_BT_MARK(3);
    if constexpr (NS > 1) {
        prep();
        if (fresh) { asm volatile("s_waitcnt vmcnt(0)" ::: "memory"); fresh = false; }
        __syncthreads();
        if (gs + 1 < gs_end && (rec_next.t[0] >> 24) != 0) issue_tile(rec_next, par ^ 1, tid);
    } else if constexpr (G * NQC <= 16) {
        constexpr int CPR = G * NQC, NIT = (TROWS + 15) / 16;
        const int col = threadIdx.x & 15, r0 = threadIdx.x >> 4;
        const int c = col / NQC, k = col - c * NQC;
        const int x = iniX0 + c * t_wCell + 16 * k;
        const bool lane_on = col < CPR && c < ncell, in_row = x < ipitch;
        const uint8_t* src = img + (size_t)(iniY + r0) * ipitch + x;
        uint4 v[NIT];
#pragma unroll
        for (int u = 0; u < NIT; u++) {
            if (lane_on && in_row && r0 + 16 * u < hr) {
                uint4 t;
                __builtin_memcpy(&t, src + (size_t)(16 * u) * ipitch, 16);
                v[u] = t;
            } else v[u] = make_uint4(0, 0, 0, 0);
        }
        prep();
#pragma unroll
        for (int u = 0; u < NIT; u++)
            if (lane_on && r0 + 16 * u < hr) *reinterpret_cast<uint4*>(&s_tile[(r0 + 16 * u) * TP + 16 * col]) = v[u];
        __syncthreads();
    } else {
        constexpr int NIT = (TROWS * G * NQC + T - 1) / T;
        uint4 v[NIT];
#pragma unroll
        for (int u = 0; u < NIT; u++) {
            const int i = threadIdx.x + u * T, r = i / (G * NQC), rem = i - r * (G * NQC), c = rem / NQC, k = rem - c * NQC;
            const int x = iniX0 + c * t_wCell + 16 * k;
            if (r < hr && c < ncell && x < ipitch) {
                const uint8_t* src = img + (size_t)(iniY + r) * ipitch + x;
                uint4 t;
                __builtin_memcpy(&t, src, 16);
                v[u] = t;
            } else v[u] = make_uint4(0, 0, 0, 0);
        }
        prep();
#pragma unroll
        for (int u = 0; u < NIT; u++) {
            const int i = threadIdx.x + u * T, r = i / (G * NQC), rem = i - r * (G * NQC), c = rem / NQC, k = rem - c * NQC;
            if (r < hr && c < ncell) *reinterpret_cast<uint4*>(&s_tile[r * TP + c * CP + 16 * k]) = v[u];
        }
        __syncthreads();
    }
    MYSLAM_BT_MARK(0);
#if MYSLAM_FAST_PHASE == 1
    if (dense) return;
#endif

    const s16x2 thv = {(short)P.minTh, (short)P.minTh};
    const int zoff = P.minTh - 1;
    const int hc2 = (hc + 1) >> 1;
    const int ngr = (g.wCell + 3) >> 2, per_cell = ngr * hc2, nitems = ncell * per_cell;
    auto split = [&](int q, float inv_pc, float inv_ngr, int& c, int& cy, int& gi) __attribute__((always_inline)) {
        c = (int)(((float)q + 0.5f) * inv_pc);
        int rem = q - c * per_cell;
        if (rem < 0) { c--; rem += per_cell; } else if (rem >= per_cell) { c++; rem -= per_cell; }
        cy = (int)(((float)rem + 0.5f) * inv_ngr);
        gi = rem - cy * ngr;
        if (gi < 0) { cy--; gi += ngr; } else if (gi >= ngr) { cy++; gi -= ngr; }
    };
    const int lane = (unsigned)tid & 63;
    auto push_maxima = [&](int mk, uint32_t zc0, uint32_t zc1, int zshift, int c, int px0, int py0) __attribute__((always_inline)) {
        int incl = __popc(mk);
        const int cnt = incl;
        incl = wave_incl_scan_dpp(incl);
        const int total = __builtin_amdgcn_readlane(incl, 63);
        if (total == 0) return;
        int base = 0;
        if (lane == 63) base = atomicAdd(&s_nlist, total);
        base = __builtin_amdgcn_readlane(base, 63);
        if (mk) {
            int dst = base + incl - cnt, zmax = 0, bits = mk;
            while (bits) {
                const int k2 = __ffs(bits) - 1;
                bits &= bits - 1;
                const uint32_t z = (((k2 & 4) ? zc1 : zc0) >> (zshift * (k2 & 3))) & 0xff;
                if (dst < NLIST) { s_list[dst] = ((uint32_t)(py0 + (k2 >> 2)) << 20) | ((uint32_t)(px0 + (k2 & 3)) << 8) | z; s_listc[dst] = (uint8_t)c; }
                dst++;
                zmax = max(zmax, (int)z);
            }
            if (zmax + zoff >= P.iniTh) s_ini[c] = 1;
        }
    };

    constexpr bool BITMAP = CW <= 32 && G == 4;
    if (!dense) {
        const float inv_pc = 1.0f / (float)per_cell, inv_ngr = 1.0f / (float)ngr;
        for (int q0 = 0; q0 < nitems; q0 += T) {
            const int q = q0 + (unsigned)tid;
            int pm = 0, c = 0, cy = 0, cx = 0;
            if (q < nitems) {
                int cy2, gi;
                split(q, inv_pc, inv_ngr, c, cy2, gi);
                cx = 4 * gi; cy = 2 * cy2;
                const int wc = wc_of(c);
                if (cx < wc) {
                    const uint8_t* base = &s_tile[cy * TP + c * CP + cx];
                    uint32_t rc[2][3], ru[2][2], rd[2][2];
#pragma unroll
                    for (int r = 0; r < 2; r++) {
                        const uint32_t* pu = reinterpret_cast<const uint32_t*>(base + (r + 0) * TP);
                        const uint32_t* pc = reinterpret_cast<const uint32_t*>(base + (r + 3) * TP);
                        const uint32_t* pd = reinterpret_cast<const uint32_t*>(base + (r + 6) * TP);
                        ru[r][0] = pu[0]; ru[r][1] = pu[1];
                        rc[r][0] = pc[0]; rc[r][1] = pc[1]; rc[r][2] = pc[2];
                        rd[r][0] = pd[0]; rd[r][1] = pd[1];
                    }
#pragma unroll
                    for (int r = 0; r < 2; r++) {
                        const uint32_t c0 = rc[r][0], c1 = rc[r][1], c2 = rc[r][2];
                        const bool a = fast9_compass_pair(pick16<3>(c0, c1), pick16<3>(rd[r][0], rd[r][1]), pick16<2>(c1, c1), pick16<3>(ru[r][0], ru[r][1]),
                                                          pick16<0>(c0, c0), thv);
                        const bool bb = fast9_compass_pair(pick16<1>(c1, c1), pick16<1>(rd[r][1], rd[r][1]), pick16<0>(c2, c2), pick16<1>(ru[r][1], ru[r][1]),
                                                           pick16<2>(c0, c0), thv);
                        pm |= (a ? 1 : 0) << (2 * r);
                        pm |= (bb ? 2 : 0) << (2 * r);
                    }
                    if (cx + 2 >= wc) pm &= 5;
                    if (cy + 1 >= hc) pm &= 3;
                }
            }
            int incl = __popc(pm);
            const int cnt = incl;
            incl = wave_incl_scan_dpp(incl);
            const int total = __builtin_amdgcn_readlane(incl, 63);
            if (total == 0) continue;
            int base = 0;
            if (lane == 63) base = atomicAdd(&s_npair, total);
            base = __builtin_amdgcn_readlane(base, 63);
            int dst = base + incl - cnt;
#pragma unroll
            for (int k2 = 0; k2 < 4; k2++)
                if (pm & (1 << k2)) s_pairs[dst++] = (uint16_t)((c << 11) | ((cy + (k2 >> 1)) << 5) | ((cx >> 1) + (k2 & 1)));
        }
        __syncthreads();
        const int np = min(s_npair, NPAIR);
        for (int q = (unsigned)tid; q < np; q += T) {
            const uint32_t e = s_pairs[q];
// ... 34 lines not shown
                        m[j][0] = __builtin_amdgcn_alignbyte(w1, w0, sh2);
                        m[j][1] = __builtin_amdgcn_alignbyte(w2, w1, sh2);
                        m[j][2] = 0u;
                    }
                    uint32_t z16;
                    mk = nms_pair<0, 0, 3>(m, z16);
                    zc = z16;
                }
            }
            push_maxima(mk, zc, 0u, 16, c, cx + 3 + (cj0 + c) * g.wCell, row + 3 + ci * g.hCell);
        }
    } else {
        auto score_item = [&](int c, int cy, int cx, uint32_t keepm) __attribute__((always_inline)) {
            uint32_t r[8][3];
#pragma unroll
            for (int j = 0; j < 8; j++) {
                const uint32_t* rp = reinterpret_cast<const uint32_t*>(&s_tile[(cy + j) * TP + c * CP + cx]);
                r[j][0] = rp[0]; r[j][1] = rp[1]; r[j][2] = rp[2];
            }
#if MYSLAM_FAST_PHASE == 2
            {
                uint32_t x = 0;
                for (int j = 0; j < 8; j++) x ^= r[j][0] ^ r[j][1] ^ r[j][2];
                *reinterpret_cast<uint32_t*>(&s_score[c][(cy + 1) * SP + 4 + cx]) = x & keepm;
                if (cy + 1 < hc) *reinterpret_cast<uint32_t*>(&s_score[c][(cy + 2) * SP + 4 + cx]) = ~x & keepm;
                return;
            }
#endif
            {
                const s16x2 za = fast9_score_pair<0, 0, 8>(r, thv), zb = fast9_score_pair<1, 0, 8>(r, thv);
                uint32_t ua, ub;
                __builtin_memcpy(&ua, &za, 4); __builtin_memcpy(&ub, &zb, 4);
                const uint32_t z4 = __builtin_amdgcn_perm(ub, ua, 0x06040200u) & keepm;
                *reinterpret_cast<uint32_t*>(&s_score[c][(cy + 1) * SP + 4 + cx]) = z4;
            }
            if (cy + 1 < hc) {
                const s16x2 za = fast9_score_pair<0, 1, 8>(r, thv), zb = fast9_score_pair<1, 1, 8>(r, thv);
                uint32_t ua, ub;
                __builtin_memcpy(&ua, &za, 4); __builtin_memcpy(&ub, &zb, 4);
                const uint32_t z4 = __builtin_amdgcn_perm(ub, ua, 0x06040200u) & keepm;
                *reinterpret_cast<uint32_t*>(&s_score[c][(cy + 2) * SP + 4 + cx]) = z4;
            }
        };
        if constexpr (BITMAP) {
            const int gi = tid & 7, c = (tid >> 3) & 3, cx = 4 * gi;
            const int wc = wc_of(c);
            if (cx < wc) {
                const uint32_t keepm = (wc - cx < 4) ? (1u << (8 * (wc - cx))) - 1u : 0xffffffffu;
                for (int cy2 = tid >> 5; cy2 < hc2; cy2 += T / 32) score_item(c, 2 * cy2, cx, keepm);
            }
        } else {
            const float inv_pc = 1.0f / (float)per_cell, inv_ngr = 1.0f / (float)ngr;
            int c, cy2, gi;
            split(tid, inv_pc, inv_ngr, c, cy2, gi);
            const int dc = T / per_cell, drem = T - dc * per_cell, dcy = drem / ngr, dgi = drem - dcy * ngr;
            auto advance = [&](int& c_, int& cy2_, int& gi_) __attribute__((always_inline)) {
                gi_ += dgi; cy2_ += dcy; c_ += dc;
                if (gi_ >= ngr) { gi_ -= ngr; cy2_++; }
                if (cy2_ >= hc2) { cy2_ -= hc2; c_++; }
            };
            for (int q = (unsigned)tid; q < nitems; q += T, advance(c, cy2, gi)) {
                const int wc = wc_of(c);
                const int cx = 4 * gi, cy = 2 * cy2;
                if (cx >= wc) continue;
                score_item(c, cy, cx, (wc - cx < 4) ? (1u << (8 * (wc - cx))) - 1u : 0xffffffffu);
            }
        }
        __syncthreads();
        MYSLAM_BT_MARK(1);
#if MYSLAM_FAST_PHASE >= 2 && MYSLAM_FAST_PHASE <= 4
        return;
#endif
        int nquad = 0;
        const int hc4 = (hc + 3) >> 2, per_cell4 = ngr * hc4;
        const int nitems4 = BITMAP ? 32 * hc4 : ncell * per_cell4;
        int c, gi, cy4;
        int ec = 0, ecy = 0, egi = 0;
        if constexpr (BITMAP) {
            gi = tid & 7; c = (tid >> 3) & 3; cy4 = tid >> 5;
        } else {
            const float inv_ngr = 1.0f / (float)ngr;
            const int q = tid;
            c = (int)(((float)q + 0.5f) * (1.0f / (float)per_cell4));
            int rem = q - c * per_cell4;
            if (rem < 0) { c--; rem += per_cell4; } else if (rem >= per_cell4) { c++; rem -= per_cell4; }
            cy4 = (int)(((float)rem + 0.5f) * inv_ngr);
            gi = rem - cy4 * ngr;
            if (gi < 0) { cy4--; gi += ngr; } else if (gi >= ngr) { cy4++; gi -= ngr; }
            ec = T / per_cell4; const int erem = T - ec * per_cell4; ecy = erem / ngr; egi = erem - ecy * ngr;
        }
        const int wc_lane = BITMAP ? wc_of(c) : 0;
        const int zini = P.iniTh - zoff;
        for (int q0 = 0; q0 < nitems4; q0 += T) {
            const int q = q0 + (unsigned)tid;
            uint32_t zm[4] = {0u, 0u, 0u, 0u};
            u16x2 zacc = {0, 0};
            if (BITMAP ? (cy4 < hc4 && 4 * gi < wc_lane) : (q < nitems4 && 4 * gi < wc_of(c))) {
                uint32_t m[6][3];
#pragma unroll
                for (int j = 0; j < 6; j++) {
                    const uint32_t* rp = reinterpret_cast<const uint32_t*>(&s_score[c][(4 * cy4 + j) * SP + 4 * gi]);
                    m[j][0] = rp[0]; m[j][1] = rp[1]; m[j][2] = rp[2];
                }
                if (sampled)
                    nquad += __popcll(__ballot(m[1][1] != 0)) + __popcll(__ballot(m[2][1] != 0)) + __popcll(__ballot(m[3][1] != 0)) + __popcll(__ballot(m[4][1] != 0));
                if ((m[1][1] | m[2][1] | m[3][1] | m[4][1]) != 0) {
                    const NmsRowH Rt = nms_row_h(m[0][0], m[0][1], m[0][2]), Rb = nms_row_h(m[5][0], m[5][1], m[5][2]);
                    NmsRow R[4];
#pragma unroll
                    for (int j = 0; j < 4; j++) R[j] = nms_row(m[j + 1][0], m[j + 1][1], m[j + 1][2]);
                    zm[0] = nms_strict4(Rt, R[0], R[1], zacc);
                    zm[1] = nms_strict4(R[0], R[1], R[2], zacc);
                    zm[2] = nms_strict4(R[1], R[2], R[3], zacc);
                    zm[3] = nms_strict4(R[2], R[3], Rb, zacc);
                }
            }
            const unsigned long long b0 = __ballot(zm[0] != 0), b1 = __ballot(zm[1] != 0), b2 = __ballot(zm[2] != 0), b3 = __ballot(zm[3] != 0);
            const int total = (int)(__popcll(b0) + __popcll(b1) + __popcll(b2) + __popcll(b3));
            if (total != 0) {
                int base = 0;
                if (lane == 0) base = atomicAdd(&s_nlist, total);
                base = __builtin_amdgcn_readfirstlane(base);
                const int code = (c << 10) | (cy4 << 6) | gi;
                int pos = rank_below(b0, rank_below(b1, rank_below(b2, rank_below(b3, base))));
#pragma unroll
                for (int j = 0; j < 4; j++)
                    if (zm[j] != 0) {
                        s_recz[pos] = zm[j]; s_pairs[pos] = (uint16_t)(code | (j << 4));
                        pos++;
                    }
                if (max((int)zacc.x, (int)zacc.y) >= zini) s_ini[c] = 1;
            }
            if constexpr (BITMAP) cy4 += T / 32;
            else {
                gi += egi; cy4 += ecy; c += ec;
                if (gi >= ngr) { gi -= ngr; cy4++; }
                if (cy4 >= hc4) { cy4 -= hc4; c++; }
            }
        }
        if (lane == 0 && nquad) atomicAdd(&s_ncorner, nquad);
#if MYSLAM_FAST_PHASE == 5
        return;
#endif
    }
    __syncthreads();
    MYSLAM_BT_MARK(2);
    if constexpr (NS > 1) asm volatile("s_waitcnt vmcnt(0)" ::: "memory");
    if ((unsigned)tid == 0 && sampled) {
        atomicAdd(&ctl.cur[level * 4], (uint32_t)(dense ? s_ncorner : min(s_npair, NPAIR)));
        atomicAdd(&ctl.cur[level * 4 + 1], (uint32_t)pairs_total);
        ctl.cur[level * 4 + 2] = dense ? 1u : 0u;
    }
    const uint8_t* mimg = maskPyr ? maskPyr + (size_t)b * pyrStride + g.imgOff : nullptr;
    uint32_t* out = cand + (size_t)b * P.totalKeyCap + g.keyOff;
    if (dense) {
        const int nrec = min(s_nlist, NLIST);
        for (int i0 = 0; i0 < nrec; i0 += T) {
            if (i0 + (int)((unsigned)tid & ~63u) >= nrec) continue;
            const int i = i0 + (unsigned)tid;
            uint32_t z = 0;
            int px0 = 0, py = 0, ini = 0;
            if (i < nrec) {
                const int code = s_pairs[i], c = code >> 10;
                z = s_recz[i];
                px0 = 4 * (code & 15) + 3 + (cj0 + c) * g.wCell;
                py = ((code >> 4) & 63) + 3 + ci * g.hCell;
                ini = s_ini[c];
            }
            uint32_t kp[2];
            unsigned long long bm[2];
            bool passk[2];
#pragma unroll
            for (int k = 0; k < 2; k++) {
                const uint32_t h = k ? z >> 16 : z & 0xffffu;
                const uint32_t second = h >> 8;
                const int sc = (int)(second ? second : h) + zoff;
                const int px = px0 + 2 * k + (second ? 1 : 0);
                bool pass = h != 0 && !(ini && sc < P.iniTh);
                if (pass && mimg) pass = mimg[(size_t)py * g.pitch + px] != 0;
                kp[k] = ((uint32_t)py << 20) | ((uint32_t)px << 8) | (uint32_t)sc;
                bm[k] = __ballot(pass); passk[k] = pass;
            }
            const int total = (int)(__popcll(bm[0]) + __popcll(bm[1]));
            if (total == 0) continue;
            int gbase = 0;
            if (lane == 0) gbase = atomicAdd(&candCount[b * MAXL + level], total);
            gbase = __builtin_amdgcn_readfirstlane(gbase);
            int dst = rank_below(bm[0], rank_below(bm[1], gbase));
            if (passk[0]) {
                if (dst < g.keyCap) out[dst] = kp[0];
                dst++;
            }
            if (passk[1]) {
                if (dst < g.keyCap) out[dst] = kp[1];
            }
        }
    } else {
    const int nl = min(s_nlist, NLIST);
    for (int i0 = 0; i0 < nl; i0 += T) {
        const int i = i0 + (unsigned)tid;
        bool pass = false;
        uint32_t kp = 0;
        if (i < nl) {
            const uint32_t e = s_list[i];
            const int sc = (int)(e & 0xff) + zoff;
            kp = (e & 0xffffff00u) | (uint32_t)sc;
            pass = !(s_ini[s_listc[i]] && sc < P.iniTh);
            if (pass && mimg) pass = mimg[(size_t)(e >> 20) * g.pitch + ((e >> 8) & 0xfff)] != 0;
        }
        const unsigned long long bm = __ballot(pass);
        if (bm == 0) continue;
        int gbase = 0;
        if (lane == 0) gbase = atomicAdd(&candCount[b * MAXL + level], __popcll(bm));
        gbase = __builtin_amdgcn_readfirstlane(gbase);
        if (pass) {
            const int dst = gbase + __popcll(bm & ((1ull << lane) - 1ull));
            if (dst < g.keyCap) out[dst] = kp;
        }
    }
    }
    rec = rec_next; par ^= (NS > 1 ? 1 : 0);
  }
}

constexpr int OT_MAXB = 1024;

__device__ __forceinline__ uint64_t wave_incl_scan64(uint64_t v) {
#define MYSLAM_SCAN64_STEP(CTRL, ROWS)                                                                                   \
    {                                                                                                                    \
        const uint32_t l2 = (uint32_t)__builtin_amdgcn_update_dpp(0, (int)(uint32_t)v, CTRL, ROWS, 0xf, false);          \
        const uint32_t h2 = (uint32_t)__builtin_amdgcn_update_dpp(0, (int)(uint32_t)(v >> 32), CTRL, ROWS, 0xf, false);  \
        v += ((uint64_t)h2 << 32) | l2;                                                                                  \
    }
    MYSLAM_SCAN64_STEP(0x111, 0xf)
    MYSLAM_SCAN64_STEP(0x112, 0xf)
    MYSLAM_SCAN64_STEP(0x114, 0xf)
    MYSLAM_SCAN64_STEP(0x118, 0xf)
    MYSLAM_SCAN64_STEP(0x142, 0xa)
    MYSLAM_SCAN64_STEP(0x143, 0xc)
#undef MYSLAM_SCAN64_STEP
    return v;
}

template <int OT>
__device__ __forceinline__ uint64_t block_excl_scan64(uint64_t v, uint64_t* s_w, uint64_t& total) {
    const int lane = threadIdx.x & 63, wid = threadIdx.x >> 6;
    const uint64_t incl = wave_incl_scan64(v);
    __syncthreads();
    if (lane == 63) s_w[wid] = incl;
    __syncthreads();
    uint64_t base = 0, tot = 0;
#pragma unroll
    for (int w = 0; w < OT / 64; w++) { const uint64_t x = s_w[w]; if (w < wid) base += x; tot += x; }
    total = tot;
    return base + incl - v;
}

__device__ __forceinline__ uint32_t oct_code(int px, int py, const LevelGeom& g) {
    int r = (int)__fdiv_rn((float)px, g.hX);
    r = min(max(r, 0), g.nIni - 1);
    int ULx = (int)__fmul_rn(g.hX, (float)r), URx = (int)__fmul_rn(g.hX, (float)(r + 1));
    int ULy = 0, BRy = g.maxBY - MIN_BORDER;
    uint32_t code = (uint32_t)r << ROOT_SHIFT;
    for (int k = 1; k <= g.ndepth; k++) {
        const int midX = ULx + ((URx - ULx + 1) >> 1);
        const int midY = ULy + ((BRy - ULy + 1) >> 1);
        const uint32_t dx = px >= midX, dy = py >= midY;
        code |= (dx | (dy << 1)) << (ROOT_SHIFT - 2 * k);
        if (dx) ULx = midX; else URx = midX;
        if (dy) ULy = midY; else BRy = midY;
    }
    return code;
}

__device__ __noinline__ void partition4(uint32_t* __restrict__ S, uint32_t* __restrict__ Cd, int lo, int hi, int sh, int& b1, int& b2, int& b3) {
    int c0 = 0, c1 = 0, c2 = 0;
    for (int i = lo; i < hi; i++) {
        const int d = (int)((Cd[i] >> sh) & 3);
        c0 += (d == 0); c1 += (d == 1); c2 += (d == 2);
    }
    b1 = lo + c0; b2 = b1 + c1; b3 = b2 + c2;
    int p0 = lo, p1 = b1, p2 = b2, p3 = b3;
    auto take = [&](int d) -> int { int r; if (d == 0) r = p0++; else if (d == 1) r = p1++; else if (d == 2) r = p2++; else r = p3++; return r; };
    const int ends[4] = {b1, b2, b3, hi};
#pragma unroll
    for (int k = 0; k < 3; k++) {
        int i = (k == 0) ? p0 : (k == 1) ? p1 : p2;
        while (i < ends[k]) {
            uint32_t v = S[i], cv = Cd[i];
            int d = (int)((cv >> sh) & 3);
            while (d != k) {
                const int j = take(d);
                const uint32_t w = S[j], cw = Cd[j];
                S[j] = v; Cd[j] = cv; v = w; cv = cw;
                d = (int)((cv >> sh) & 3);
            }
            S[i] = v; Cd[i] = cv;
            i++;
            if (k == 0) p0 = i; else if (k == 1) p1 = i; else p2 = i;
        }
    }
}

struct OctLds {
    uint32_t *lo0, *lo1, *hi0, *hi1;
    uint16_t *pfx0, *pfx1;
    uint8_t *dep0, *dep1;
    uint32_t *nb1, *nb2, *nb3;
    uint32_t *ckey0, *ckey1;
    uint16_t *cpos0, *cpos1;
    uint16_t* ord;
    uint16_t *kinc, *binc;
    uint8_t* kk;
    uint8_t* mark;
    uint32_t* offs;
    __device__ __forceinline__ uint32_t* lo(int i) const { return i ? lo1 : lo0; }
    __device__ __forceinline__ uint32_t* hi(int i) const { return i ? hi1 : hi0; }
    __device__ __forceinline__ uint16_t* pfx(int i) const { return i ? pfx1 : pfx0; }
    __device__ __forceinline__ uint8_t* dep(int i) const { return i ? dep1 : dep0; }
    __device__ __forceinline__ uint32_t* ckey(int i) const { return i ? ckey1 : ckey0; }
    __device__ __forceinline__ uint16_t* cpos(int i) const { return i ? cpos1 : cpos0; }
};

__device__ __forceinline__ void child_bounds(const OctLds& L, uint32_t* __restrict__ S, uint32_t* __restrict__ Cd, int D, int lo, int hi, int d, int pfx,
                                             int& b1, int& b2, int& b3) {
    if (d < D) {
        const int sb = 2 * (D - d - 1);
        const int base = pfx << 2;
        b1 = L.offs[(base + 1) << sb]; b2 = L.offs[(base + 2) << sb]; b3 = L.offs[(base + 3) << sb];
    } else {
        partition4(S, Cd, lo, hi, ROOT_SHIFT - 2 * (d + 1), b1, b2, b3);
    }
}

__device__ __forceinline__ uint32_t half_row_max_u32(uint32_t v) {
    v = max(v, (uint32_t)__builtin_amdgcn_update_dpp(0, (int)v, 0x141, 0xf, 0xf, false));
    v = max(v, (uint32_t)__builtin_amdgcn_update_dpp(0, (int)v, 0xb1, 0xf, 0xf, false));
    v = max(v, (uint32_t)__builtin_amdgcn_update_dpp(0, (int)v, 0x4e, 0xf, 0xf, false));
    return v;
}

__device__ __forceinline__ int sel_order_bin(uint32_t pay, int ts) {
    const int tx = (int)((pay >> 8) & 0xfff) >> ts, ty = (int)(pay >> 20) >> ts;
    int z = 0;
#pragma unroll
    for (int k = 0; k < 4; k++) z |= (((tx >> k) & 1) << (2 * k)) | (((ty >> k) & 1) << (2 * k + 1));
    return ((tx >> 4) << 8) | z;
}

constexpr int OCT_WIDE_BELOW = 64;
constexpr int OCT_FL = 4;
template <int OT>
__global__ __launch_bounds__(OT) void k_octree(OrbPlan P, const uint32_t* __restrict__ cand,
                                               const int32_t* __restrict__ candCount, uint32_t* __restrict__ sortbuf,
                                               const uint32_t* __restrict__ octTab,
                                               uint32_t* __restrict__ selOut, int32_t* __restrict__ selCount,
                                               int32_t* __restrict__ status, int NCmax, uint16_t* __restrict__ order, BlurMulti BM) {
    MYSLAM_SIDE_PRIO();
    MYSLAM_BT(2);
    extern __shared__ __attribute__((aligned(16))) uint8_t smem[];
    const int t = threadIdx.x;
    if constexpr (OT == 512) {
        if ((int)blockIdx.y >= P.nlevels) {
            const int wv = __builtin_amdgcn_readfirstlane(t >> 6);
            blur7_strip_wave(BM, ((int)blockIdx.y - P.nlevels) * 8 + wv, blockIdx.x, smem + wv * (16 * B3_TS));
            return;
        }
    }
    const int level = blockIdx.y, b = blockIdx.x;
    const LevelGeom& g = P.lv[level];
    const int NC = NCmax;

    uint64_t* s_w = reinterpret_cast<uint64_t*>(smem);
    int* s_i = reinterpret_cast<int*>(smem + 128);
    uint8_t* pcur = smem + 192;
    uint32_t* s_cursor = reinterpret_cast<uint32_t*>(pcur); pcur += 4 * OT_MAXB;
    OctLds L;
    L.offs = reinterpret_cast<uint32_t*>(pcur); pcur += 4 * (OT_MAXB + 2);
    uint32_t* const s_tab = reinterpret_cast<uint32_t*>(pcur);
    L.lo0 = reinterpret_cast<uint32_t*>(pcur); pcur += 4 * NC;
    L.lo1 = reinterpret_cast<uint32_t*>(pcur); pcur += 4 * NC;
    L.hi0 = reinterpret_cast<uint32_t*>(pcur); pcur += 4 * NC;
    L.hi1 = reinterpret_cast<uint32_t*>(pcur); pcur += 4 * NC;
    L.nb1 = reinterpret_cast<uint32_t*>(pcur); pcur += 4 * NC;
    L.nb2 = reinterpret_cast<uint32_t*>(pcur); pcur += 4 * NC;
    L.nb3 = reinterpret_cast<uint32_t*>(pcur); pcur += 4 * NC;
    L.ckey0 = reinterpret_cast<uint32_t*>(pcur); pcur += 4 * NC;
    L.ckey1 = reinterpret_cast<uint32_t*>(pcur); pcur += 4 * NC;
    L.pfx0 = reinterpret_cast<uint16_t*>(pcur); pcur += 2 * NC;
    L.pfx1 = reinterpret_cast<uint16_t*>(pcur); pcur += 2 * NC;
    L.cpos0 = reinterpret_cast<uint16_t*>(pcur); pcur += 2 * NC;
    L.cpos1 = reinterpret_cast<uint16_t*>(pcur); pcur += 2 * NC;
    L.ord = reinterpret_cast<uint16_t*>(pcur); pcur += 2 * NC;
    L.kinc = reinterpret_cast<uint16_t*>(pcur); pcur += 2 * NC;
    L.binc = reinterpret_cast<uint16_t*>(pcur); pcur += 2 * NC;
    L.dep0 = pcur; pcur += NC;
    L.dep1 = pcur; pcur += NC;
    L.kk = pcur; pcur += NC;
    L.mark = pcur; pcur += NC;

    const int cnt = candCount[b * MAXL + level];
    int32_t* myCount = selCount + b * MAXL + level;
    if (cnt > g.keyCap) {
        if (t == 0) { *myCount = 0; status[b] = MYSLAM_ERR_CAPACITY; }
        return;
    }
    const int n = cnt;
    if (n == 0) { if (t == 0) *myCount = 0; return; }

    const uint32_t* keys = cand + (size_t)b * P.totalKeyCap + g.keyOff;
    uint32_t* S = sortbuf + ((size_t)b * P.totalKeyCap + g.keyOff) * 2;
    uint32_t* Cd = S + g.keyCap;
    const int D = g.sortDepth;
    const int NB = g.nIni << (2 * D);
    const int bsh = ROOT_SHIFT - 2 * D;

    const uint32_t* xcode = octTab + g.tabOff; const uint32_t* ycode = xcode + g.tabX;
    const uint32_t* xcell = ycode + g.tabY; const uint32_t* ycell = xcell + g.tabX;
    const int ntab = 2 * (g.tabX + g.tabY);
    const bool tabLds = (size_t)ntab * 4 <= (size_t)54 * NC;
    for (int i = t; i < NB; i += OT) s_cursor[i] = 0;
    if (tabLds) for (int i = t; i < ntab; i += OT) s_tab[i] = xcode[i];
    __syncthreads();
    const bool rankkey = g.nCols * g.nRows <= 1024;
    const float inv_ncols = 1.0f / (float)g.nCols;
    auto passes = [&](auto in_lds) __attribute__((always_inline)) {
        constexpr bool LDS = decltype(in_lds)::value;
        const int oyc = g.tabX, oxl = g.tabX + g.tabY, oyl = 2 * g.tabX + g.tabY;
        auto XC = [&](uint32_t i) -> uint32_t { if constexpr (LDS) return s_tab[i]; else return xcode[i]; };
        auto YC = [&](uint32_t i) -> uint32_t { if constexpr (LDS) return s_tab[oyc + i]; else return ycode[i]; };
        auto XL = [&](uint32_t i) -> uint32_t { if constexpr (LDS) return s_tab[oxl + i]; else return xcell[i]; };
        auto YL = [&](uint32_t i) -> uint32_t { if constexpr (LDS) return s_tab[oyl + i]; else return ycell[i]; };
        for (int i0 = t; i0 < n; i0 += OCT_FL * OT) {
            uint32_t pay[OCT_FL], cx[OCT_FL], cy[OCT_FL];
#pragma unroll
            for (int u = 0; u < OCT_FL; u++) pay[u] = (i0 + u * OT < n) ? keys[i0 + u * OT] : 0u;
#pragma unroll
            for (int u = 0; u < OCT_FL; u++) { cx[u] = XC((pay[u] >> 8) & 0xfff); cy[u] = YC(pay[u] >> 20); }
#pragma unroll
            for (int u = 0; u < OCT_FL; u++)
                if (i0 + u * OT < n) atomicAdd(&s_cursor[(cx[u] | cy[u]) >> bsh], 1u);
        }
        __syncthreads();
        {
            const int c = (NB + OT - 1) / OT;
            const int beg = min(NB, t * c), end = min(NB, beg + c);
            uint64_t sum = 0;
            for (int i = beg; i < end; i++) sum += s_cursor[i];
            uint64_t total;
            uint64_t run = block_excl_scan64<OT>(sum, s_w, total);
            for (int i = beg; i < end; i++) {
                const uint32_t h = s_cursor[i];
                L.offs[i] = (uint32_t)run;
                s_cursor[i] = (uint32_t)run;
                run += h;
            }
            if (t == 0) L.offs[NB] = (uint32_t)n;
        }
        __syncthreads();
        for (int i0 = t; i0 < n; i0 += OCT_FL * OT) {
            uint32_t pay[OCT_FL], cx[OCT_FL], cy[OCT_FL], qx[OCT_FL], qy[OCT_FL];
#pragma unroll
            for (int u = 0; u < OCT_FL; u++) pay[u] = (i0 + u * OT < n) ? keys[i0 + u * OT] : 0u;
#pragma unroll
            for (int u = 0; u < OCT_FL; u++) {
                const uint32_t px = (pay[u] >> 8) & 0xfff, py = pay[u] >> 20;
                cx[u] = XC(px); cy[u] = YC(py);
                qx[u] = rankkey ? XL(px) : 0u; qy[u] = rankkey ? YL(py) : 0u;
            }
#pragma unroll
            for (int u = 0; u < OCT_FL; u++) {
                if (i0 + u * OT >= n) continue;
                uint32_t low = pay[u];
                if (rankkey) {
                    const int px = (int)((pay[u] >> 8) & 0xfff), py = (int)(pay[u] >> 20);
                    const int ci = (int)(((float)qy[u] + 0.5f) * inv_ncols);
                    const uint32_t pxc = (uint32_t)(px - 3 - (int)qx[u] * g.wCell), pyc = (uint32_t)(py - 3 - ci * g.hCell);
                    low = ((pay[u] & 0xffu) << 22) | (0x3fffffu - (((qy[u] + qx[u]) << 12) | (pyc << 6) | pxc));
                }
                const uint32_t code = cx[u] | cy[u];
                const uint32_t pos = atomicAdd(&s_cursor[code >> bsh], 1u);
                S[pos] = low; Cd[pos] = code;
            }
        }
        __syncthreads();
    };
    if (tabLds) passes(std::true_type{}); else passes(std::false_type{});

    MYSLAM_BT_MARK(0);
    MYSLAM_BT_AUX((unsigned long long)level | ((unsigned long long)n << 8));
    if (t == 0) {
        int m = 0;
        for (int r = 0; r < g.nIni; r++) {
            const int lo = L.offs[r << (2 * D)], hi = L.offs[(r + 1) << (2 * D)];
            if (hi > lo) { L.lo0[m] = (uint32_t)lo; L.hi0[m] = (uint32_t)hi; L.dep0[m] = 0; L.pfx0[m] = (uint16_t)r; m++; }
        }
        s_i[0] = m; s_i[1] = 0;
    }
    __syncthreads();

    int cur = 0, ccur = 0, mode = 0;
    const int N = g.N;
    for (int round = 0; round < 96; round++) {
        const int m = s_i[0];
        const int prevSize = m;
        int newM;
        if (mode == 0) {
            const int c = (m + OT - 1) / OT;
            const int beg = min(m, t * c), end = min(m, beg + c);
            uint64_t packed = 0;
            for (int p = beg; p < end; p++) {
                const int lo = (int)L.lo(cur)[p], hi = (int)L.hi(cur)[p], d = L.dep(cur)[p];
                int k = 0;
                if (hi - lo > 1 && d < g.ndepth) {
                    int b1, b2, b3;
                    child_bounds(L, S, Cd, D, lo, hi, d, L.pfx(cur)[p], b1, b2, b3);
                    L.nb1[p] = (uint32_t)b1; L.nb2[p] = (uint32_t)b2; L.nb3[p] = (uint32_t)b3;
                    const int c0 = b1 - lo, c1 = b2 - b1, c2 = b3 - b2, c3 = hi - b3;
                    k = (c0 > 0) + (c1 > 0) + (c2 > 0) + (c3 > 0);
                    const int big = (c0 > 1) + (c1 > 1) + (c2 > 1) + (c3 > 1);
                    packed += (uint64_t)k | ((uint64_t)big << 42);
                } else {
                    packed += 1ull << 21;
                }
                L.kk[p] = (uint8_t)k;
            }
            uint64_t total;
            uint64_t run = block_excl_scan64<OT>(packed, s_w, total);
            const int Ktot = (int)(total & 0x1fffff), Ntot = (int)((total >> 21) & 0x1fffff), Btot = (int)(total >> 42);
            const int nxt = cur ^ 1, cnxt = ccur ^ 1;
            for (int p = beg; p < end; p++) {
                const int lo = (int)L.lo(cur)[p], hi = (int)L.hi(cur)[p], d = L.dep(cur)[p];
                const int pf = L.pfx(cur)[p];
                const int k = L.kk[p];
                if (k) {
                    const int bnd[5] = {lo, (int)L.nb1[p], (int)L.nb2[p], (int)L.nb3[p], hi};
                    const int rk = (int)(run & 0x1fffff);
                    int pos = Ktot - (rk + k);
                    int cidx = (int)(run >> 42);
                    int childPos[4];
#pragma unroll
                    for (int q = 3; q >= 0; q--) {
                        childPos[q] = pos;
                        if (bnd[q + 1] > bnd[q]) {
                            L.lo(nxt)[pos] = (uint32_t)bnd[q]; L.hi(nxt)[pos] = (uint32_t)bnd[q + 1];
                            L.dep(nxt)[pos] = (uint8_t)(d + 1);
                            L.pfx(nxt)[pos] = (uint16_t)((pf << 2) | q);
                            pos++;
                        }
                    }
#pragma unroll
                    for (int q = 0; q < 4; q++) {
                        const int sz = bnd[q + 1] - bnd[q];
                        if (sz > 1) {
                            L.ckey(cnxt)[cidx] = ((uint32_t)sz << 14) | (uint32_t)cidx;
                            L.cpos(cnxt)[cidx] = (uint16_t)childPos[q];
                            cidx++;
                        }
                    }
                    const int big = cidx - (int)(run >> 42);
                    run += (uint64_t)k | ((uint64_t)big << 42);
                } else {
                    const int rn = (int)((run >> 21) & 0x1fffff);
                    L.lo(nxt)[Ktot + rn] = (uint32_t)lo; L.hi(nxt)[Ktot + rn] = (uint32_t)hi;
                    L.dep(nxt)[Ktot + rn] = (uint8_t)d;
                    L.pfx(nxt)[Ktot + rn] = (uint16_t)pf;
                    run += 1ull << 21;
                }
            }
            newM = Ktot + Ntot;
            __syncthreads();
            if (t == 0) { s_i[0] = newM; s_i[1] = Btot; }
            cur = nxt; ccur = cnxt;
            __syncthreads();
            if (newM >= N || newM == prevSize) break;
            if (newM + 3 * Btot > N) mode = 1;
        } else {
            const int nc = s_i[1];
            if (nc == 0) break;
            for (int ci = t; ci < nc; ci += OT) {
                const uint32_t key = L.ckey(ccur)[ci];
                int rank = 0;
                for (int cj = 0; cj < nc; cj++) rank += (L.ckey(ccur)[cj] > key);
                L.ord[rank] = (uint16_t)ci;
            }
            for (int p = t; p < m; p += OT) L.mark[p] = 0;
            if (t == 0) s_i[2] = nc - 1;
            __syncthreads();
            const int c = (nc + OT - 1) / OT;
            const int beg = min(nc, t * c), end = min(nc, beg + c);
            uint64_t packed = 0;
            for (int j = beg; j < end; j++) {
                const int p = L.cpos(ccur)[L.ord[j]];
                const int lo = (int)L.lo(cur)[p], hi = (int)L.hi(cur)[p], d = L.dep(cur)[p];
                int k = 1, big = 1, b1 = hi, b2 = hi, b3 = hi;
                if (d < g.ndepth) {
                    child_bounds(L, S, Cd, D, lo, hi, d, L.pfx(cur)[p], b1, b2, b3);
                    const int c0 = b1 - lo, c1 = b2 - b1, c2 = b3 - b2, c3 = hi - b3;
                    k = (c0 > 0) + (c1 > 0) + (c2 > 0) + (c3 > 0);
                    big = (c0 > 1) + (c1 > 1) + (c2 > 1) + (c3 > 1);
                }
                L.nb1[j] = (uint32_t)b1; L.nb2[j] = (uint32_t)b2; L.nb3[j] = (uint32_t)b3;
                L.kk[j] = (uint8_t)(k | (big << 4));
                packed += (uint64_t)k | ((uint64_t)big << 32);
            }
            uint64_t total;
            uint64_t run = block_excl_scan64<OT>(packed, s_w, total);
            for (int j = beg; j < end; j++) {
                const int k = L.kk[j] & 15, big = L.kk[j] >> 4;
                run += (uint64_t)k | ((uint64_t)big << 32);
                const int kincl = (int)(run & 0xffffffffu);
                L.kinc[j] = (uint16_t)kincl;
                L.binc[j] = (uint16_t)(run >> 32);
                if (m + kincl - (j + 1) >= N) atomicMin(&s_i[2], j);
            }
            __syncthreads();
            const int ncmt = min(s_i[2] + 1, nc);
            const int Kc = L.kinc[ncmt - 1];
            const int nxt = cur ^ 1, cnxt = ccur ^ 1;
            for (int j = t; j < ncmt; j += OT) L.mark[L.cpos(ccur)[L.ord[j]]] = 1;
            __syncthreads();
            for (int j = t; j < ncmt; j += OT) {
                const int p = L.cpos(ccur)[L.ord[j]];
                const int lo = (int)L.lo(cur)[p], hi = (int)L.hi(cur)[p], d = L.dep(cur)[p];
                const int pf = L.pfx(cur)[p];
// ... 482 lines not shown
            const uint8_t* center = reinterpret_cast<const uint8_t*>(s_b[wave]) + (j % NBUF) * (DB_N * 16) + DB_R * DB_P + offB + DB_R;
            uint32_t nib = 0;
#pragma unroll
            for (int q = 0; q < 4; q++) {
                const float x0 = pat[4 * q], y0 = pat[4 * q + 1], x1 = pat[4 * q + 2], y1 = pat[4 * q + 3];
                constexpr float RM = 12582912.f; constexpr uint32_t RK = 0x4B400000u;
                const uint32_t r0 = __float_as_uint(__fadd_rn(__fadd_rn(__fmul_rn(x0, sb), __fmul_rn(y0, ca)), RM));
                const uint32_t c0 = __float_as_uint(__fadd_rn(__fsub_rn(__fmul_rn(x0, ca), __fmul_rn(y0, sb)), RM));
                const uint32_t r1 = __float_as_uint(__fadd_rn(__fadd_rn(__fmul_rn(x1, sb), __fmul_rn(y1, ca)), RM));
                const uint32_t c1 = __float_as_uint(__fadd_rn(__fsub_rn(__fmul_rn(x1, ca), __fmul_rn(y1, sb)), RM));
                static_assert(DB_P == 64, "row pitch of the LDS window as a shift");
                const int t0 = center[(int)((r0 << 6) + c0 - 65u * RK)], t1 = center[(int)((r1 << 6) + c1 - 65u * RK)];
                nib |= (uint32_t)(t0 < t1) << q;
            }
            const uint32_t byte = nib | (__shfl_down(nib, 1, 64) << 4);
            uint32_t w = byte | (__shfl_down(byte, 2, 64) << 8);
            w |= (__shfl_down(byte, 4, 64) << 16) | (__shfl_down(byte, 6, 64) << 24);
            if ((lane & 7) == 0) reinterpret_cast<uint32_t*>(desc + ((size_t)b * cap + s_out[k]) * 32)[lane >> 3] = w;
        }
    }
    return;
#endif
    for (int j = 0; j < KD_KPB / 4; j++) {
        const int k = 4 * j + wave;
        const int level = __builtin_amdgcn_readfirstlane(s_lv[k]);
        if (level < 0) continue;
        const LevelGeom& g = P.lv[level];
        const int x = __builtin_amdgcn_readfirstlane(s_x[k]), y = __builtin_amdgcn_readfirstlane(s_y[k]);
        const float ca = s_ca[k], sb = s_sb[k];
        const int xb0 = (x - DB_R) & ~15, offB = (x - DB_R) - xb0;
        const int y0 = y - DB_R;
        const uint8_t* bl = blur + (size_t)b * pyrStride + g.imgOff + (size_t)(y0 >> 3) * g.pitch * 8 + (size_t)(xb0 >> 4) * 128;
        uint4 rb[DB_IT];
#pragma unroll
        for (int q = 0; q < DB_IT; q++) {
            const int i = lane + 64 * q;
            const int wr = ((i >> 5) << 3) + (i & 7) - (y0 & 7);
            rb[q] = (wr >= 0 && wr < DB_ROWS) ? *reinterpret_cast<const uint4*>(bl + (uint32_t)(__mul24(i >> 5, g.pitch * 8) + 16 * (i & 31))) : make_uint4(0, 0, 0, 0);
        }
        __builtin_amdgcn_wave_barrier();
#pragma unroll
        for (int q = 0; q < DB_IT; q++) {
            const int i = lane + 64 * q;
            const int wr = ((i >> 5) << 3) + (i & 7) - (y0 & 7);
            if (wr >= 0 && wr < DB_ROWS) s_b[wave][wr * 4 + ((i >> 3) & 3)] = rb[q];
        }
        __builtin_amdgcn_fence(__ATOMIC_RELEASE, "wavefront");
        __builtin_amdgcn_wave_barrier();
        __builtin_amdgcn_fence(__ATOMIC_ACQUIRE, "wavefront");
        const uint8_t* center = reinterpret_cast<const uint8_t*>(s_b[wave]) + DB_R * DB_P + offB + DB_R;
        uint32_t nib = 0;
#pragma unroll
        for (int q = 0; q < 4; q++) {
            const float x0 = pat[4 * q], y0 = pat[4 * q + 1], x1 = pat[4 * q + 2], y1 = pat[4 * q + 3];
            constexpr float RM = 12582912.f; constexpr uint32_t RK = 0x4B400000u;
            const uint32_t r0 = __float_as_uint(__fadd_rn(__fadd_rn(__fmul_rn(x0, sb), __fmul_rn(y0, ca)), RM));
            const uint32_t c0 = __float_as_uint(__fadd_rn(__fsub_rn(__fmul_rn(x0, ca), __fmul_rn(y0, sb)), RM));
            const uint32_t r1 = __float_as_uint(__fadd_rn(__fadd_rn(__fmul_rn(x1, sb), __fmul_rn(y1, ca)), RM));
            const uint32_t c1 = __float_as_uint(__fadd_rn(__fsub_rn(__fmul_rn(x1, ca), __fmul_rn(y1, sb)), RM));
            static_assert(DB_P == 64, "row pitch of the LDS window as a shift");
            const int t0 = center[(int)((r0 << 6) + c0 - 65u * RK)], t1 = center[(int)((r1 << 6) + c1 - 65u * RK)];
            nib |= (uint32_t)(t0 < t1) << q;
        }
        const uint32_t byte = nib | (__shfl_down(nib, 1, 64) << 4);
        uint32_t w = byte | (__shfl_down(byte, 2, 64) << 8);
        w |= (__shfl_down(byte, 4, 64) << 16) | (__shfl_down(byte, 6, 64) << 24);
        if ((lane & 7) == 0) reinterpret_cast<uint32_t*>(desc + ((size_t)b * cap + s_out[k]) * 32)[lane >> 3] = w;
    }
}

__global__ __launch_bounds__(256) void k_describe2(OrbPlan P, const uint8_t* __restrict__ pyr, const uint8_t* __restrict__ blur,
                                                   size_t pyrStride, const uint32_t* __restrict__ selOut,
                                                   const int32_t* __restrict__ selCount, myslam_keypoint* __restrict__ kps,
                                                   uint8_t* __restrict__ desc, int32_t* __restrict__ counts,
                                                   int32_t* __restrict__ status, int cap, int nchunk, int batch, int detectOnly,
                                                   const uint16_t* __restrict__ order) {
    MYSLAM_SIDE_PRIO();
    const int total = nchunk * batch, nwg = gridDim.x, bid = blockIdx.x;
    const int xcd = bid & 7, j = bid >> 3, per = (nwg + 7 - xcd) >> 3;
    const int tq = total >> 3, tr = total & 7;
    const int lo = xcd < tr ? xcd * (tq + 1) : tr * (tq + 1) + (xcd - tr) * tq, n = tq + (xcd < tr ? 1 : 0);
#pragma nounroll
    for (int k = j; k < n; k += per) {
        MYSLAM_BT(4);
        describe_block(P, pyr, blur, pyrStride, selOut, selCount, kps, desc, counts, status, cap, nchunk, batch, detectOnly, order, lo + k MYSLAM_BT_ARG);
        __syncthreads();
    }
}

__device__ __forceinline__ bool is_fast_corner(const uint8_t* __restrict__ img, int pitch, int x, int y, int th) {
    constexpr int RX[16] = {0, 1, 2, 3, 3, 3, 2, 1, 0, -1, -2, -3, -3, -3, -2, -1};
    constexpr int RY[16] = {3, 3, 2, 1, 0, -1, -2, -3, -3, -3, -2, -1, 0, 1, 2, 3};
    th = min(max(th, 0), 255);
    const uint8_t* p = img + (size_t)y * pitch + x;
    const int v = p[0];
    unsigned dm = 0, bm = 0;
#pragma unroll
    for (int k = 0; k < 16; k++) {
        const int pv = p[RX[k] + RY[k] * pitch];
        dm |= (unsigned)(pv < v - th) << k;
        bm |= (unsigned)(pv > v + th) << k;
    }
    auto run9 = [](unsigned m) {
        unsigned x = m | (m << 16);
        unsigned r = x & (x >> 1);
        r &= r >> 2;
        r &= r >> 4;
        r &= x >> 8;
        return (r & 0xffffu) != 0;
    };
    return run9(dm) || run9(bm);
}

__global__ __launch_bounds__(256) void k_screen(OrbPlan P, const uint8_t* __restrict__ pyr, myslam_keypoint* __restrict__ kin,
                                                int n, myslam_keypoint* __restrict__ kout, uint8_t* __restrict__ keep) {
    const int i = blockIdx.x * 4 + (threadIdx.x >> 6);
    const int lane = threadIdx.x & 63;
    if (i >= n) return;
    myslam_keypoint k = kin[i];
    const int level = k.octave;
    if (level < 0 || level >= P.nlevels) { if (lane == 0) keep[i] = 0; return; }
    const LevelGeom& g = P.lv[level];
    const float scale = g.scale;
    k.x = __fdiv_rn(k.x, scale); k.y = __fdiv_rn(k.y, scale);
    bool ok = (__fsub_rn(k.y, (float)EDGE_THRESHOLD) >= 0 && __fadd_rn(k.y, (float)EDGE_THRESHOLD) < (float)g.h &&
               __fsub_rn(k.x, (float)EDGE_THRESHOLD) >= 0 && __fadd_rn(k.x, (float)EDGE_THRESHOLD) < (float)g.w);
    const uint8_t* img = pyr + g.imgOff;
    int px = 0, py = 0;
    if (ok) {
        px = __float2int_rn(k.x); py = __float2int_rn(k.y);
        ok = is_fast_corner(img, g.pitch, px, py, P.minTh);
    }
    if (ok) {
        k.angle = wave_ic_angle(img, g.pitch, px, py);
        k.size = __fmul_rn((float)PATCH_SIZE, scale);
    }
    k.x = __fmul_rn(k.x, scale); k.y = __fmul_rn(k.y, scale);
    if (lane == 0) { kin[i] = k; kout[i] = k; keep[i] = ok ? 1 : 0; }
}

__global__ __launch_bounds__(256) void k_calc_desc(OrbPlan P, const uint8_t* __restrict__ blur, const myslam_keypoint* __restrict__ kps,
                                                   int n, uint8_t* __restrict__ desc) {
    const int i = blockIdx.x * 4 + (threadIdx.x >> 6);
    const int lane = threadIdx.x & 63;
    if (i >= n) return;
    const myslam_keypoint k = kps[i];
    const int level = min(max(k.octave, 0), P.nlevels - 1);
    const LevelGeom& g = P.lv[level];
    const int px = __float2int_rn(__fdiv_rn(k.x, g.scale)), py = __float2int_rn(__fdiv_rn(k.y, g.scale));
    const uint32_t w = wave_brief<true>(blur + g.imgOff, g.pitch, px, py, k.angle);
    if ((lane & 7) == 0) reinterpret_cast<uint32_t*>(desc + (size_t)i * 32)[lane >> 3] = w;
}

__global__ void k_unpack_cands(const uint32_t* __restrict__ cand, int n, int32_t* xs, int32_t* ys, int32_t* sc) {
    const int i = blockIdx.x * blockDim.x + threadIdx.x;
    if (i >= n) return;
    const uint32_t p = cand[i];
    xs[i] = (p >> 8) & 0xfff; ys[i] = p >> 20; sc[i] = p & 0xff;
}

struct ZeroArgs { uint32_t* p[4]; int n[4]; };
__device__ __forceinline__ void zero_part(const ZeroArgs& z, int tid, int T) {
#pragma unroll
    for (int k = 0; k < 4; k++)
        for (int i = tid; i < z.n[k]; i += T) z.p[k][i] = 0u;
}
__device__ __forceinline__ void ingest_part(const uint8_t* __restrict__ src, int rows, int cols, int step, size_t sstride,
                                            uint8_t* __restrict__ dst, int dpitch, size_t dstride, int tpr, int rpb, int bx, int by, int b) {
    const int y = by * rpb + (int)threadIdx.x / tpr;
    const int x16 = (bx * 256 + (int)threadIdx.x % tpr) * 16;
    if ((int)threadIdx.x >= tpr * rpb || y >= rows || x16 >= cols) return;
    const uint8_t* s = src + (size_t)b * sstride + (size_t)y * step + x16;
    const uint32_t sh = (uint32_t)(reinterpret_cast<uintptr_t>(s) & 3);
    const uint32_t* sa = reinterpret_cast<const uint32_t*>(s - sh);
    const int nvalid = cols - x16;
    uint32_t d[5];
#pragma unroll
    for (int j = 0; j < 5; j++) d[j] = (4 * j < (int)sh + nvalid) ? sa[j] : 0u;
    uint4 o;
    o.x = __builtin_amdgcn_alignbyte(d[1], d[0], sh); o.y = __builtin_amdgcn_alignbyte(d[2], d[1], sh);
    o.z = __builtin_amdgcn_alignbyte(d[3], d[2], sh); o.w = __builtin_amdgcn_alignbyte(d[4], d[3], sh);
    uint8_t* q = dst + (size_t)b * dstride + (size_t)y * dpitch + x16;
    if (x16 + 16 <= dpitch) *reinterpret_cast<uint4*>(q) = o;
    else { uint32_t w[4] = {o.x, o.y, o.z, o.w}; for (int j = 0; j < 4 && x16 + 4 * j < dpitch; j++) reinterpret_cast<uint32_t*>(q)[j] = w[j]; }
}
__global__ __launch_bounds__(256) void k_ingest(const uint8_t* __restrict__ src, int rows, int cols, int step, size_t sstride,
                                                uint8_t* __restrict__ dst, int dpitch, size_t dstride, int tpr, int rpb, ZeroArgs z) {
    zero_part(z, (int)((blockIdx.z * gridDim.y + blockIdx.y) * gridDim.x + blockIdx.x) * 256 + (int)threadIdx.x, (int)(gridDim.x * gridDim.y * gridDim.z) * 256);
    ingest_part(src, rows, cols, step, sstride, dst, dpitch, dstride, tpr, rpb, blockIdx.x, blockIdx.y, blockIdx.z);
}

struct IngestPart { const uint8_t* src; int rows, cols, step; size_t sstride; uint8_t* dst; int dpitch; size_t dstride; int tpr, rpb, gx, b0; };
__global__ __launch_bounds__(256) void k_pyr_head(ResizeChain c, IngestPart g, ZeroArgs z) {
    const int blk = blockIdx.x, b = blockIdx.y;
    zero_part(z, (int)(blockIdx.y * gridDim.x + blockIdx.x) * 256 + (int)threadIdx.x, (int)(gridDim.x * gridDim.y) * 256);
    if (blk < c.blk0[RC_MAX]) { rc_block(c, blk, b); return; }
    if (b < g.b0) return;
    const int ib = blk - c.blk0[RC_MAX];
    ingest_part(g.src, g.rows, g.cols, g.step, g.sstride, g.dst, g.dpitch, g.dstride, g.tpr, g.rpb, ib % g.gx, ib / g.gx, b);
}

__global__ __launch_bounds__(256) void k_zero_u32(ZeroArgs a) {
    const int i = blockIdx.x * 256 + threadIdx.x;
#pragma unroll
    for (int k = 0; k < 4; k++)
        if (a.p[k] && i < a.n[k]) a.p[k][i] = 0u;
}
void launch_zero_u32(uint32_t* p0, int n0, uint32_t* p1, int n1, uint32_t* p2, int n2, uint32_t* p3, int n3, hipStream_t s) {
    ZeroArgs a{{p0, p1, p2, p3}, {n0, n1, n2, n3}};
    const int n = max(max(n0, n1), max(n2, n3));
    if (n > 0) hipLaunchKernelGGL(k_zero_u32, dim3((n + 255) / 256), dim3(256), 0, s, a);
}

static void ingest_launch(const uint8_t* src, int rows, int cols, int step, size_t sstride, uint8_t* dst, int dpitch,
                          size_t dstride, int batch, const ZeroArgs& z, hipStream_t s) {
    const int t = (cols + 15) / 16;
    const int tpr = t < 256 ? t : 256, rpb = t < 256 ? 256 / t : 1;
    dim3 grid((t + 255) / 256, (rows + rpb - 1) / rpb, batch);
    hipLaunchKernelGGL(k_ingest, grid, dim3(256), 0, s, src, rows, cols, step, sstride, dst, dpitch, dstride, tpr, rpb, z);
}
void launch_ingest(const uint8_t* src, int rows, int cols, int step, size_t sstride, uint8_t* dst, int dpitch,
                   size_t dstride, int batch, hipStream_t s) {
    ingest_launch(src, rows, cols, step, sstride, dst, dpitch, dstride, batch, ZeroArgs{{nullptr, nullptr, nullptr, nullptr}, {0, 0, 0, 0}}, s);
}
void launch_ingest_clear(const uint8_t* src, int rows, int cols, int step, size_t sstride, uint8_t* dst, int dpitch, size_t dstride, int batch,
                         uint32_t* p0, int n0, uint32_t* p1, int n1, uint32_t* p2, int n2, uint32_t* p3, int n3, hipStream_t s) {
    ingest_launch(src, rows, cols, step, sstride, dst, dpitch, dstride, batch, ZeroArgs{{p0, p1, p2, p3}, {n0, n1, n2, n3}}, s);
}

bool resize_uses_strips(const ResizeArgs& a) { return (double)RS_R * a.scale_y + 2.0 <= (double)RS_MAXR && a.scale_x <= 1.6; }

bool resize_is_little(const ResizeArgs& a, int batch) { return a.n0 == 0 && (size_t)batch * a.dw * a.dh < (size_t)1500000; }

#ifndef MYSLAM_RESIZE_CHAIN_MAX
#define MYSLAM_RESIZE_CHAIN_MAX 3
#endif
int resize_chain_max() { return MYSLAM_RESIZE_CHAIN_MAX < RC_MAX ? MYSLAM_RESIZE_CHAIN_MAX : RC_MAX; }

static ResizeChain make_chain(const ResizeArgs* lv, int n) {
    ResizeChain c;
    c.src = lv[0].src; c.sw = lv[0].sw; c.sh = lv[0].sh; c.spitch = lv[0].spitch; c.sstride = lv[0].sstride;
    c.n = n; c.dstride = lv[0].dstride; c.blk0[0] = 0;
    for (int j = 0; j < RC_MAX; j++) {
        const ResizeArgs& a = lv[j < n ? j : n - 1];
        c.dst[j] = a.dst; c.dw[j] = a.dw; c.dh[j] = a.dh; c.dpitch[j] = a.dpitch; c.scale_x[j] = a.scale_x; c.scale_y[j] = a.scale_y;
        c.blk0[j + 1] = c.blk0[j] + (j < n ? (((a.dw + 3) / 4) * (4 / rc_px(j + 1)) * a.dh + 255) / 256 : 0);
    }
    return c;
}
void launch_resize_chain(const ResizeArgs* lv, int n, int batch, hipStream_t s) {
    const ResizeChain c = make_chain(lv, n);
    hipLaunchKernelGGL(k_resize_chain, dim3(c.blk0[RC_MAX], batch), dim3(256), 0, s, c);
}
void launch_pyr_head(const ResizeArgs* lv, int n, int rows, int cols, uint8_t* dst0, int dpitch0, size_t dstride0, int b0, int batch,
                     uint32_t* p0, int n0, uint32_t* p1, int n1, uint32_t* p2, int n2, uint32_t* p3, int n3, hipStream_t s) {
    const ResizeChain c = make_chain(lv, n);
    const int t = (cols + 15) / 16;
    IngestPart g{lv[0].src, rows, cols, lv[0].spitch, lv[0].sstride, dst0, dpitch0, dstride0, t < 256 ? t : 256, t < 256 ? 256 / t : 1, (t + 255) / 256, b0};
    const int iblocks = g.gx * ((rows + g.rpb - 1) / g.rpb);
    hipLaunchKernelGGL(k_pyr_head, dim3(c.blk0[RC_MAX] + iblocks, batch), dim3(256), 0, s, c, g, ZeroArgs{{p0, p1, p2, p3}, {n0, n1, n2, n3}});
}
#ifndef MYSLAM_PYR_HEAD_LEVELS
#define MYSLAM_PYR_HEAD_LEVELS 2
#endif
int pyr_head_levels() { return MYSLAM_PYR_HEAD_LEVELS < 3 ? MYSLAM_PYR_HEAD_LEVELS : 3; }

void launch_resize(const ResizeArgs& a, int batch, hipStream_t s) {
    const bool little = resize_is_little(a, batch);
    if (resize_uses_strips(a) && !little) {
        const int nstrips = (a.dw + 255) / 256, nbands = (a.dh + RS_R - 1) / RS_R;
        const int ngroups = (nbands + RS_NB - 1) / RS_NB;
        hipLaunchKernelGGL(k_resize_strip, dim3((nstrips * ngroups + 3) / 4, 1, batch), dim3(256), 0, s, a, nstrips, nbands);
        return;
    }
    dim3 grid((a.dw + 255) / 256, (a.dh + 3) / 4, batch);
    hipLaunchKernelGGL(k_resize, grid, dim3(256), 0, s, a);
}

bool blur_uses_strips(const BlurArgs& a) {
    return a.w >= 8 && a.h >= 8 && (a.spitch & 3) == 0 && ((reinterpret_cast<uintptr_t>(a.src) | a.sstride) & 3) == 0;
}

void launch_blur_levels(const BlurArgs* lv, int n, int batch, hipStream_t s) {
    BlurMulti M; M.n = 0; M.wave0[0] = 0;
    BlurMfmaMulti X; X.n = 0; X.wave0[0] = 0;
    for (int i = 0; i < n; i++) {
        const BlurArgs& a = lv[i];
        if (a.tabH && a.tabV && a.ident && a.dtiled && (a.dpitch & 15) == 0 && ((reinterpret_cast<uintptr_t>(a.dst) | a.dstride) & 15) == 0) {
            X.a[X.n] = a; X.tabHOff[X.n] = 0; X.tabVOff[X.n] = 0; X.wave0[X.n + 1] = X.wave0[X.n] + (a.w + 31) / 32; X.n++;
        } else if (blur_uses_strips(a)) {
            const int nstrips = (a.w + 255) / 256, nbands = (a.h + B3_R - 1) / B3_R;
            M.a[M.n] = a; M.nstrips[M.n] = nstrips; M.wave0[M.n + 1] = M.wave0[M.n] + nstrips * nbands; M.n++;
        } else {
            dim3 grid((a.w + B2_W - 1) / B2_W, (a.h + B2_H - 1) / B2_H, batch);
            hipLaunchKernelGGL(k_blur7_dot, grid, dim3(256), 0, s, a);
        }
    }
    if (M.n) hipLaunchKernelGGL(k_blur7_strip, dim3((M.wave0[M.n] + 3) / 4, 1, batch), dim3(256), 0, s, M);
    if (X.n) hipLaunchKernelGGL(k_blur7_mfma, dim3((X.wave0[X.n] + 3) / 4, 1, batch), dim3(256), 0, s, X);
}
void launch_blur(const BlurArgs& a, int batch, hipStream_t s) { launch_blur_levels(&a, 1, batch, s); }

#ifndef MYSLAM_BLUR_WITH_OCTREE
#define MYSLAM_BLUR_WITH_OCTREE 1
#endif
bool blur_multi_for_octree(const BlurArgs* lv, int n, int batch, BlurMulti& M) {
    if (!MYSLAM_BLUR_WITH_OCTREE || batch >= OCT_WIDE_BELOW || batch >= 16) return false;
    M.n = 0; M.wave0[0] = 0;
    for (int i = 0; i < n; i++) {
        const BlurArgs& a = lv[i];
        if ((a.tabH && a.tabV) || !blur_uses_strips(a)) return false;
        const int nstrips = (a.w + 255) / 256, nbands = (a.h + B3_R - 1) / B3_R;
        M.a[M.n] = a; M.nstrips[M.n] = nstrips; M.wave0[M.n + 1] = M.wave0[M.n] + nstrips * nbands; M.n++;
    }
    return M.n > 0;
}

void launch_fast(const OrbPlan& P, const uint8_t* pyr, size_t pyrStride, const uint8_t* maskPyr, uint32_t* cand,
                 int32_t* candCount, const uint32_t* statPrev, uint32_t* statCur, int forceMode, int batch, hipStream_t s) {
    int cw = 0, ch = 0;
    for (int l = 0; l < P.nlevels; l++) { cw = max(cw, P.lv[l].wCell); ch = max(ch, P.lv[l].hCell); }
    const FastCtl ctl{statPrev, statCur, forceMode};
    const dim3 grid((unsigned)P.nstrips * (unsigned)batch);
    constexpr int pad = FastLds<32, 4, 40>::PAD;
#if MYSLAM_FAST_NS > 1
    if (cw <= 32 && ch <= 40 && (size_t)P.nstrips * batch >= (size_t)MYSLAM_FAST_NS * 256 * 6 * 4) {
        const dim3 gridms((unsigned)(((size_t)P.nstrips * batch + MYSLAM_FAST_NS - 1) / MYSLAM_FAST_NS));
        constexpr int padms = FastLds<32, 4, 40, MYSLAM_FAST_NS>::PAD + FastLds<32, 4, 40, MYSLAM_FAST_NS>::TROWS * FastLds<32, 4, 40, MYSLAM_FAST_NS>::TP + 16;
        hipLaunchKernelGGL((k_fast_strip<32, 4, 40, MYSLAM_FAST_NS>), gridms, dim3(256), padms, s, P, pyr, pyrStride, maskPyr, cand, candCount, ctl, batch);
        return;
    }
#endif
    if (cw <= 32 && ch <= 40) hipLaunchKernelGGL((k_fast_strip<32, 4, 40>), grid, dim3(256), pad, s, P, pyr, pyrStride, maskPyr, cand, candCount, ctl, batch);
    else if (max(cw, ch) <= 40) hipLaunchKernelGGL((k_fast_strip<40, 4>), grid, dim3(256), 0, s, P, pyr, pyrStride, maskPyr, cand, candCount, ctl, batch);
    else hipLaunchKernelGGL((k_fast_strip<MAX_CELL, 4>), grid, dim3(256), 0, s, P, pyr, pyrStride, maskPyr, cand, candCount, ctl, batch);
}

size_t octree_lds_bytes(int nodeCap) { return 192 + 4 * (size_t)OT_MAXB + 4 * (size_t)(OT_MAXB + 2) + (size_t)nodeCap * 54 + 16; }

bool blur_multi_for_octree(const BlurArgs* lv, int n, int batch, BlurMulti& M);
bool launch_octree(const OrbPlan& P, const uint32_t* cand, const int32_t* candCount, uint32_t* sortbuf, const uint32_t* octTab, uint32_t* selOut,
                   int32_t* selCount, int32_t* status, int batch, uint16_t* order, hipStream_t s, const BlurArgs* blurLv, int nBlur) {
    BlurMulti BMh;
    const BlurMulti* blurWith = (blurLv && nBlur > 0 && blur_multi_for_octree(blurLv, nBlur, batch, BMh)) ? &BMh : nullptr;
    int ncmax = 0;
    for (int l = 0; l < P.nlevels; l++) ncmax = max(ncmax, P.lv[l].nodeCap);
    const size_t lds = std::max(octree_lds_bytes(ncmax), (size_t)8 * 16 * B3_TS);
    (void)hipFuncSetAttribute(reinterpret_cast<const void*>(k_octree<256>), hipFuncAttributeMaxDynamicSharedMemorySize, 160 * 1024);
    (void)hipFuncSetAttribute(reinterpret_cast<const void*>(k_octree<512>), hipFuncAttributeMaxDynamicSharedMemorySize, 160 * 1024);
    if (batch >= OCT_WIDE_BELOW)
        hipLaunchKernelGGL(k_octree<256>, dim3(batch, P.nlevels), dim3(256), lds, s, P, cand, candCount, sortbuf, octTab, selOut, selCount, status, ncmax, order, BlurMulti{});
    else
    {
        BlurMulti M = blurWith ? *blurWith : BlurMulti{};
        if (!blurWith) M.n = 0;
        const int brows = blurWith ? (M.wave0[M.n] + 7) / 8 : 0;
        hipLaunchKernelGGL(k_octree<512>, dim3(batch, P.nlevels + brows), dim3(512), lds, s, P, cand, candCount, sortbuf, octTab, selOut, selCount, status, ncmax, order, M);
    }
    return blurWith != nullptr;
}

bool describe_uses_tile_order(bool have_order, int detectOnly, int batch) { return have_order && !detectOnly && batch >= 8; }

void launch_describe(const OrbPlan& P, const uint8_t* pyr, const uint8_t* blur, size_t pyrStride, const uint32_t* selOut,
                     const int32_t* selCount, myslam_keypoint* kps, uint8_t* desc, int32_t* counts, int32_t* status,
                     int cap, int detectOnly, int batch, uint16_t* order, bool order_ready, int blocks_per_cu, hipStream_t s) {
    const int slots = min(cap, P.totalOut);
    const int nchunk = (slots + KD_KPB - 1) / KD_KPB;
    const bool tiled = describe_uses_tile_order(order != nullptr, detectOnly, batch);
    if (tiled && !order_ready) hipLaunchKernelGGL(k_sel_order, dim3(P.nlevels, batch), dim3(256), 0, s, P, selOut, selCount, order, batch);
    const int total = nchunk * batch;
    const int grid = blocks_per_cu > 0 ? min(total, 256 * blocks_per_cu) : total;
    hipLaunchKernelGGL(k_describe2, dim3(grid), dim3(256), 0, s, P, pyr, blur, pyrStride, selOut, selCount,
                       kps, desc, counts, status, cap, nchunk, batch, detectOnly, tiled ? order : nullptr);
}

void launch_screen(const OrbPlan& P, const uint8_t* pyr, myslam_keypoint* kin, int n, myslam_keypoint* kout, uint8_t* keep,
                   hipStream_t s) {
    hipLaunchKernelGGL(k_screen, dim3((n + 3) / 4), dim3(256), 0, s, P, pyr, kin, n, kout, keep);
}

void launch_calc_desc(const OrbPlan& P, const uint8_t* blur, const myslam_keypoint* kps, int n, uint8_t* desc, hipStream_t s) {
    hipLaunchKernelGGL(k_calc_desc, dim3((n + 3) / 4), dim3(256), 0, s, P, blur, kps, n, desc);
}

void launch_unpack_cands(const uint32_t* cand, int n, int32_t* xs, int32_t* ys, int32_t* sc, hipStream_t s) {
    if (n <= 0) return;
    hipLaunchKernelGGL(k_unpack_cands, dim3((n + 255) / 256), dim3(256), 0, s, cand, n, xs, ys, sc);
}

}

#ifdef MYSLAM_BLOCK_TRACE
extern "C" int myslam_debug_block_trace(void* d_buf, unsigned cap_records, unsigned* n) {
    using namespace myslam_hip;
    unsigned long long* p = (unsigned long long*)d_buf;
    const unsigned zero = 0;
    if (n) MYSLAM_HIP_CHECK(hipMemcpyFromSymbol(n, HIP_SYMBOL(g_bt_n), sizeof(unsigned)));
    if (d_buf) MYSLAM_HIP_CHECK(hipMemcpyToSymbol(HIP_SYMBOL(g_bt_n), &zero, sizeof(unsigned)));
    MYSLAM_HIP_CHECK(hipMemcpyToSymbol(HIP_SYMBOL(g_bt_cap), &cap_records, sizeof(unsigned)));
    MYSLAM_HIP_CHECK(hipMemcpyToSymbol(HIP_SYMBOL(g_bt_buf), &p, sizeof(p)));
    return MYSLAM_OK;
}
#endif
```

### a-simple-stereo-slam-system-with-deep-loop-closing_amd/csrc/orb_plan.h

```cpp
#pragma once
#include <stddef.h>
#include <stdint.h>

namespace myslam_hip {

constexpr int MAXL = 12;
constexpr int EDGE_THRESHOLD = 19;
constexpr int MIN_BORDER = 16;
constexpr int PATCH_SIZE = 31;
constexpr int HALF_PATCH = 15;
constexpr int MAX_CELL = 59;
constexpr int MAX_DEPTH = 13;
constexpr int ROOT_SHIFT = 26;

struct LevelGeom {
    int w, h, pitch;
    int nCols, nRows, wCell, hCell;
    int maxBX, maxBY;
    int cellBase;
    int stripBase;
    int N;
    int nIni;
    float hX;
    int sortDepth;
    int ndepth;
    int keyCap;
    int nodeCap;
    int outBase;
    float scale;
    float scaledPatch;
    size_t imgOff;
    size_t keyOff;
    int tabOff, tabX, tabY;
};

struct OrbPlan {
    int nlevels;
    int rows, cols;
    int ncells;
    int nstrips;
    int iniTh, minTh;
    int totalKeyCap;
    int totalOut;
    size_t pyrBytes;
    const uint8_t* ext0; size_t ext0Stride; int ext0Pitch, ext0N;
    int stripBaseOf[MAXL];
    const uint32_t* stripTab;
    LevelGeom lv[MAXL];
};

struct ResizeArgs {
    const uint8_t* src; int sw, sh, spitch; size_t sstride;
    const uint8_t* src0 = nullptr; int spitch0 = 0, n0 = 0; size_t sstride0 = 0;
    uint8_t* dst; int dw, dh, dpitch; size_t dstride;
    double scale_x, scale_y;
};

struct BlurArgs {
    const uint8_t* src; uint8_t* dst; int w, h, spitch, dpitch; size_t sstride, dstride;
    const uint8_t* src0 = nullptr; int spitch0 = 0, n0 = 0; size_t sstride0 = 0;
    int q[7];
    int dtiled = 0;
    const uint4* tabH = nullptr; const uint4* tabV = nullptr; const uint4* ident = nullptr; int vconst = 0;
};

__host__ __device__ inline size_t tiled_off(int x, int y, int pitch) {
    return (size_t)(y >> 3) * (size_t)pitch * 8 + (size_t)((x >> 4) << 7) + (size_t)(((y & 7) << 4) | (x & 15));
}

}
```

Before: 79200.

## Write FAST candidates into per-strip segments instead of per-level atomic append

FAST now writes candidates into fixed per-strip segments, sized at plan time from a worst-case bound, and records a count per strip. Before, every strip appended to one per-level list through a shared counter. The octree kernel walks the strip segments with a prefix table in LDS to gather keys, and the host debug paths gather per strip. This removes per-level global atomic contention and the clearing of those counters, at the cost of larger candidate buffers, an indirect gather, and more LDS in the octree kernel.

```diff
diff --git a/a-simple-stereo-slam-system-with-deep-loop-closing_amd/csrc/orb_engine.hip b/a-simple-stereo-slam-system-with-deep-loop-closing_amd/csrc/orb_engine.hip
--- a/a-simple-stereo-slam-system-with-deep-loop-closing_amd/csrc/orb_engine.hip
+++ b/a-simple-stereo-slam-system-with-deep-loop-closing_amd/csrc/orb_engine.hip
@@ -20,8 +20,8 @@
 bool blur_uses_strips(const BlurArgs& a);
 bool resize_uses_strips(const ResizeArgs& a);
 void launch_fast(const OrbPlan& P, const uint8_t* pyr, size_t pyrStride, const uint8_t* maskPyr, uint32_t* cand,
-                 int32_t* candCount, const uint32_t* statPrev, uint32_t* statCur, int forceMode, int batch, hipStream_t s);
-bool launch_octree(const OrbPlan& P, const uint32_t* cand, const int32_t* candCount, uint32_t* sortbuf, const uint32_t* octTab, uint32_t* selOut,
+                 int32_t* stripCount, const uint32_t* statPrev, uint32_t* statCur, int forceMode, int batch, hipStream_t s);
+bool launch_octree(const OrbPlan& P, const uint32_t* cand, const int32_t* stripCount, uint32_t* sortbuf, const uint32_t* octTab, uint32_t* selOut,
                    int32_t* selCount, int32_t* status, int batch, uint16_t* order, hipStream_t s, const BlurArgs* blurLv, int nBlur);
 bool describe_uses_tile_order(bool have_order, int detectOnly, int batch);
 void launch_describe(const OrbPlan& P, const uint8_t* pyr, const uint8_t* blur, size_t pyrStride, const uint32_t* selOut,
@@ -30,7 +30,6 @@
 void launch_screen(const OrbPlan& P, const uint8_t* pyr, myslam_keypoint* kin, int n, myslam_keypoint* kout, uint8_t* keep,
                    hipStream_t s);
 void launch_calc_desc(const OrbPlan& P, const uint8_t* blur, const myslam_keypoint* kps, int n, uint8_t* desc, hipStream_t s);
-void launch_unpack_cands(const uint32_t* cand, int n, int32_t* xs, int32_t* ys, int32_t* sc, hipStream_t s);
 void launch_blur_levels(const BlurArgs* lv, int n, int batch, hipStream_t s);
 bool blur_mfma_tables(int w, int h, const int q[7], std::vector<uint4>& tab, size_t& offH, size_t& offV);
 void blur_mfma_ident(std::vector<uint4>& tab, size_t& offI);
@@ -100,7 +99,9 @@
     uint8_t *d_pyr = nullptr, *d_blur = nullptr, *d_mask = nullptr;
     uint32_t* d_cand = nullptr;
     uint32_t* d_sort = nullptr;
-    int32_t *d_candCount = nullptr, *d_selCount = nullptr, *d_status = nullptr;
+    int32_t *d_stripCount = nullptr;
+    std::vector<uint32_t> segOff;
+    int32_t *d_selCount = nullptr, *d_status = nullptr;
     uint32_t* d_sel = nullptr;
     uint16_t* d_order = nullptr;
     uint32_t* d_octTab = nullptr;
@@ -139,6 +140,7 @@
     int blur_levels(int batch, int nlev, hipStream_t s);
     void fill_blur_args(BlurArgs* lv, int nlev) const;
     int run_fast(const OrbPlan& P, const uint8_t* maskPyr, int batch);
+    int gather_cands(const OrbPlan& P, int b, int level, std::vector<uint32_t>* list, int* total);
     int run_batch(const uint8_t* d_imgs, int batch, int r, int c, int step, size_t stride, const uint8_t* d_masks,
                   myslam_keypoint* d_kps, uint8_t* d_desc, int32_t* d_counts, int32_t* d_stat, int cap, bool detectOnly);
     void free_all();
@@ -168,7 +170,7 @@
 int myslam_orb::make_plan(int r, int c) {
     OrbPlan P{};
     P.nlevels = nlevels; P.rows = r; P.cols = c; P.iniTh = iniTh; P.minTh = minTh;
-    size_t imgOff = 0, keyOff = 0; int cellBase = 0, outBase = 0, stripBase = 0;
+    size_t imgOff = 0; int cellBase = 0, outBase = 0, stripBase = 0;
     for (int l = 0; l < nlevels; l++) {
         LevelGeom& g = P.lv[l];
         g.w = cv_round((float)c * invScale[l]);
@@ -200,10 +202,9 @@
         g.scale = scale[l];
         g.scaledPatch = (float)(int)(PATCH_SIZE * scale[l]);
         g.imgOff = imgOff; imgOff += align_up((size_t)g.pitch * align_up((size_t)g.h, 8), 256);
-        g.keyOff = keyOff; keyOff += g.keyCap;
     }
     for (int l = 0; l < MAXL; l++) P.stripBaseOf[l] = l < P.nlevels ? P.lv[l].stripBase : INT32_MAX;
-    P.ncells = cellBase; P.nstrips = stripBase; P.totalKeyCap = (int)keyOff; P.totalOut = outBase; P.pyrBytes = imgOff;
+    P.ncells = cellBase; P.nstrips = stripBase; P.totalOut = outBase; P.pyrBytes = imgOff;
     {
         std::vector<uint32_t> tab;
         for (int l = 0; l < nlevels; l++) {
@@ -245,14 +246,17 @@
     }
     {
         std::vector<uint32_t> st((size_t)P.nstrips * 8, 0u);
+        segOff.assign((size_t)P.nstrips, 0u);
+        size_t keyOff = 0;
         for (int l = 0; l < nlevels; l++) {
-            const LevelGeom& g = P.lv[l];
+            LevelGeom& g = P.lv[l];
             const int spr = (g.nCols + 3) / 4;
+            size_t seg = 0;
             for (int strip = 0; strip < g.nRows * spr; strip++) {
                 uint32_t* e = st.data() + (size_t)(g.stripBase + strip) * 8;
                 const int ci = strip / spr, cj0 = (strip - ci * spr) * 4;
                 const int iniY = MIN_BORDER + ci * g.hCell;
-                int ncell = 0, pairs = 0; uint32_t wcs = 0; int hr = 0;
+                int ncell = 0, pairs = 0, worst = 0; uint32_t wcs = 0; int hr = 0;
                 if (iniY < g.maxBY - 3) {
                     hr = std::min(iniY + g.hCell + 6, g.maxBY) - iniY;
                     const int hc = hr - 6;
@@ -264,16 +268,24 @@
                             if (wc > 0) ncell = c + 1;
                             wcs |= (uint32_t)wc << (8 * c);
                             pairs += ((wc + 1) >> 1) * hc;
+                            worst += ((wc + 1) >> 1) * ((hc + 1) >> 1);
                         }
                 }
                 if (ncell == 0) wcs = 0;
+                if (seg >= ((size_t)1 << 25)) return MYSLAM_ERR_UNSUPPORTED;
+                segOff[(size_t)g.stripBase + strip] = (uint32_t)seg;
                 e[0] = (uint32_t)l | ((uint32_t)ci << 8) | ((uint32_t)cj0 << 16) | ((uint32_t)ncell << 24);
                 e[1] = (uint32_t)iniY | ((uint32_t)hr << 16);
                 e[2] = (uint32_t)(MIN_BORDER + cj0 * g.wCell) | ((uint32_t)g.wCell << 16);
-                e[3] = wcs; e[4] = (uint32_t)g.pitch; e[5] = (uint32_t)pairs;
+                e[3] = wcs; e[4] = (uint32_t)(g.pitch >> 6) | ((uint32_t)seg << 7); e[5] = (uint32_t)pairs;
                 e[6] = (uint32_t)(g.imgOff & 0xffffffffu); e[7] = (uint32_t)(g.imgOff >> 32);
+                seg += (size_t)worst;
             }
-        }
+            g.candCap = (int)std::max<size_t>(seg, (size_t)g.keyCap);
+            g.keyOff = keyOff; keyOff += (size_t)g.candCap;
+        }
+        if (keyOff > (size_t)INT32_MAX) return MYSLAM_ERR_UNSUPPORTED;
+        P.totalKeyCap = (int)keyOff;
         int rc = dev_alloc(d_stripTab, st.size());
         if (rc) return rc;
         if ((rc = upload_table(d_stripTab, st.data(), st.size() * sizeof(uint32_t)))) return rc;
@@ -310,7 +322,7 @@
         if ((rc = dev_alloc(d_blur, (size_t)batch * full.pyrBytes + 4096))) return rc;
         if ((rc = dev_alloc(d_cand, (size_t)batch * full.totalKeyCap))) return rc;
         if ((rc = dev_alloc(d_sort, (size_t)batch * full.totalKeyCap * 2))) return rc;
-        if ((rc = dev_alloc(d_candCount, (size_t)batch * MAXL))) return rc;
+        if ((rc = dev_alloc(d_stripCount, (size_t)batch * full.nstrips))) return rc;
         if ((rc = dev_alloc(d_selCount, (size_t)batch * MAXL))) return rc;
         if ((rc = dev_alloc(d_status, (size_t)batch))) return rc;
         if ((rc = dev_alloc(d_sel, (size_t)batch * selPer))) return rc;
@@ -445,8 +457,8 @@
         MYSLAM_HIP_CHECK(hipMalloc((void**)&d_fastStat, sizeof(uint32_t) * 2 * MAXL * 4));
         MYSLAM_HIP_CHECK(hipMemsetAsync(d_fastStat, 0, sizeof(uint32_t) * 2 * MAXL * 4, stream));
     }
-    clr = {{reinterpret_cast<uint32_t*>(d_candCount), reinterpret_cast<uint32_t*>(d_selCount), reinterpret_cast<uint32_t*>(stat), d_fastStat + (size_t)fastFlip * MAXL * 4},
-           {batch * MAXL, batch * MAXL, batch, MAXL * 4}};
+    clr = {{reinterpret_cast<uint32_t*>(d_selCount), reinterpret_cast<uint32_t*>(stat), d_fastStat + (size_t)fastFlip * MAXL * 4, nullptr},
+           {batch * MAXL, batch, MAXL * 4, 0}};
     const int stop = optStopAfter;
     {
         int n0 = 0;
@@ -493,7 +505,7 @@
         BlurArgs blv[MAXL];
         const bool tryBlur = !fork && !detectOnly && stop == 0 && !optBlurMfma;
         if (tryBlur) fill_blur_args(blv, P.nlevels);
-        blurred = launch_octree(P, d_cand, d_candCount, d_sort, d_octTab, d_sel, d_selCount, stat, batch,
+        blurred = launch_octree(P, d_cand, d_stripCount, d_sort, d_octTab, d_sel, d_selCount, stat, batch,
                                 describe_uses_tile_order(d_order != nullptr, detectOnly ? 1 : 0, batch) ? d_order : nullptr, stream,
                                 tryBlur ? blv : nullptr, tryBlur ? P.nlevels : 0);
     }
@@ -515,7 +527,28 @@
     const uint32_t* prev = d_fastStat + (size_t)(fastFlip ^ 1) * MAXL * 4;
     fastFlip ^= 1;
     ScopedProf sp(P_FAST, stream);
-    launch_fast(P, d_pyr, full.pyrBytes, maskPyr, d_cand, d_candCount, prev, cur, optFastMode, batch, stream);
+    launch_fast(P, d_pyr, full.pyrBytes, maskPyr, d_cand, d_stripCount, prev, cur, optFastMode, batch, stream);
+    return MYSLAM_OK;
+}
+
+int myslam_orb::gather_cands(const OrbPlan& P, int b, int level, std::vector<uint32_t>* list, int* total) {
+    const LevelGeom& g = P.lv[level];
+    const int ns = g.nRows * ((g.nCols + 3) / 4);
+    std::vector<int32_t> cnt((size_t)ns);
+    MYSLAM_HIP_CHECK(hipMemcpyAsync(cnt.data(), d_stripCount + (size_t)b * P.nstrips + g.stripBase, sizeof(int32_t) * ns, hipMemcpyDeviceToHost, stream));
+    MYSLAM_HIP_CHECK(hipStreamSynchronize(stream));
+    long long n = 0;
+    for (int s = 0; s < ns; s++) n += cnt[s];
+    *total = (int)n;
+    if (!list) return MYSLAM_OK;
+    std::vector<uint32_t> blk((size_t)g.candCap);
+    MYSLAM_HIP_CHECK(hipMemcpy(blk.data(), d_cand + (size_t)b * P.totalKeyCap + g.keyOff, sizeof(uint32_t) * blk.size(), hipMemcpyDeviceToHost));
+    list->clear(); list->reserve((size_t)n);
+    for (int s = 0; s < ns; s++) {
+        const size_t o = segOff[(size_t)g.stripBase + s];
+        if (cnt[s] < 0 || o + (size_t)cnt[s] > blk.size()) return MYSLAM_ERR_CAPACITY;
+        list->insert(list->end(), blk.begin() + o, blk.begin() + o + cnt[s]);
+    }
     return MYSLAM_OK;
 }
 
@@ -554,7 +587,7 @@
 }
 
 void myslam_orb::free_all() {
-    void* ptrs[] = {d_blurTab, d_fastStat, d_octTab, d_stripTab, d_pyr, d_blur, d_mask, d_cand, d_sort, d_candCount, d_selCount, d_status, d_sel, d_order, d_stageImg, d_stageMask,
+    void* ptrs[] = {d_blurTab, d_fastStat, d_octTab, d_stripTab, d_pyr, d_blur, d_mask, d_cand, d_sort, d_stripCount, d_selCount, d_status, d_sel, d_order, d_stageImg, d_stageMask,
                     d_stageOut, d_stageKps2, d_stageKeep};
     for (void* p : ptrs) if (p) (void)hipFree(p);
     if (aux) { (void)hipStreamSynchronize(aux); (void)hipStreamDestroy(aux); (void)hipEventDestroy(evFork); (void)hipEventDestroy(evJoin); aux = nullptr; }
@@ -858,26 +891,19 @@
         MYSLAM_HIP_CHECK(hipMalloc((void**)&h->d_fastStat, sizeof(uint32_t) * 2 * MAXL * 4));
         MYSLAM_HIP_CHECK(hipMemsetAsync(h->d_fastStat, 0, sizeof(uint32_t) * 2 * MAXL * 4, h->stream));
     }
-    launch_zero_u32(reinterpret_cast<uint32_t*>(h->d_candCount), MAXL, h->d_fastStat + (size_t)h->fastFlip * MAXL * 4, MAXL * 4, nullptr, 0, nullptr, 0, h->stream);
+    launch_zero_u32(h->d_fastStat + (size_t)h->fastFlip * MAXL * 4, MAXL * 4, nullptr, 0, nullptr, 0, nullptr, 0, h->stream);
     h->full.ext0N = h->det.ext0N = 0;
     if ((rc = h->build_pyramids(h->d_stageImg, 1, step, (size_t)rows * step, mask ? h->d_stageMask : nullptr, h->nlevels))) return rc;
     if ((rc = h->run_fast(h->full, mask ? h->d_mask : nullptr, 1))) return rc;
-    int32_t counts[MAXL];
-    MYSLAM_HIP_CHECK(hipMemcpyAsync(counts, h->d_candCount, sizeof(counts), hipMemcpyDeviceToHost, h->stream));
-    MYSLAM_HIP_CHECK(hipStreamSynchronize(h->stream));
     const LevelGeom& g = h->full.lv[level];
-    *n = counts[level];
-    if (counts[level] > g.keyCap || counts[level] > cap) return MYSLAM_ERR_CAPACITY;
-    int32_t* d_tmp = nullptr;
-    const int m = counts[level];
+    int m = 0;
+    std::vector<uint32_t> list;
+    if ((rc = h->gather_cands(h->full, 0, level, &list, &m))) return rc;
+    *n = m;
+    if (m > g.keyCap || m > cap) return MYSLAM_ERR_CAPACITY;
     if (m > 0) {
-        MYSLAM_HIP_CHECK(hipMalloc((void**)&d_tmp, sizeof(int32_t) * 3 * m));
-        launch_unpack_cands(h->d_cand + g.keyOff, m, d_tmp, d_tmp + m, d_tmp + 2 * m, h->stream);
-        MYSLAM_HIP_CHECK(hipMemcpyAsync(xs, d_tmp, 4 * m, hipMemcpyDeviceToHost, h->stream));
-        MYSLAM_HIP_CHECK(hipMemcpyAsync(ys, d_tmp + m, 4 * m, hipMemcpyDeviceToHost, h->stream));
-        MYSLAM_HIP_CHECK(hipMemcpyAsync(scores, d_tmp + 2 * m, 4 * m, hipMemcpyDeviceToHost, h->stream));
-        MYSLAM_HIP_CHECK(hipStreamSynchronize(h->stream));
-        (void)hipFree(d_tmp);
+        if (!xs || !ys || !scores) return MYSLAM_ERR_INVALID;
+        for (int i = 0; i < m; i++) { const uint32_t p = list[i]; xs[i] = (int32_t)((p >> 8) & 0xfff); ys[i] = (int32_t)(p >> 20); scores[i] = (int32_t)(p & 0xff); }
     }
     return MYSLAM_OK;
 }
@@ -895,14 +921,28 @@
             MYSLAM_HIP_CHECK(hipMemcpy2D(out, g.w, base, g.pitch, g.w, g.h, hipMemcpyDeviceToHost));
             return MYSLAM_OK;
         }
-        case 2: case 4: {
+        case 2: {
             if (cap_bytes < 4) return MYSLAM_ERR_CAPACITY;
-            MYSLAM_HIP_CHECK(hipMemcpy(out, (what == 2 ? h->d_candCount : h->d_selCount) + b * MAXL + level, 4, hipMemcpyDeviceToHost));
+            int m = 0;
+            const int rc = h->gather_cands(P, b, level, nullptr, &m);
+            if (rc) return rc;
+            *static_cast<int32_t*>(out) = m;
+            return MYSLAM_OK;
+        }
+        case 4: {
+            if (cap_bytes < 4) return MYSLAM_ERR_CAPACITY;
+            MYSLAM_HIP_CHECK(hipMemcpy(out, h->d_selCount + b * MAXL + level, 4, hipMemcpyDeviceToHost));
             return MYSLAM_OK;
         }
         case 3: {
             if (cap_bytes < (size_t)g.keyCap * 4) return MYSLAM_ERR_CAPACITY;
-            MYSLAM_HIP_CHECK(hipMemcpy(out, h->d_cand + (size_t)b * P.totalKeyCap + g.keyOff, (size_t)g.keyCap * 4, hipMemcpyDeviceToHost));
+            int m = 0;
+            std::vector<uint32_t> list;
+            const int rc = h->gather_cands(P, b, level, &list, &m);
+            if (rc) return rc;
+            if (m > g.keyCap) return MYSLAM_ERR_CAPACITY;
+            memset(out, 0, (size_t)g.keyCap * 4);
+            if (m > 0) memcpy(out, list.data(), (size_t)m * 4);
             return MYSLAM_OK;
         }
         case 6: {
diff --git a/a-simple-stereo-slam-system-with-deep-loop-closing_amd/csrc/orb_kernels.hip b/a-simple-stereo-slam-system-with-deep-loop-closing_amd/csrc/orb_kernels.hip
--- a/a-simple-stereo-slam-system-with-deep-loop-closing_amd/csrc/orb_kernels.hip
+++ b/a-simple-stereo-slam-system-with-deep-loop-closing_amd/csrc/orb_kernels.hip
@@ -884,7 +884,7 @@
 template <int CW, int G, int CH = CW, int NS = 1>
 __global__ __launch_bounds__(256) __attribute__((amdgpu_waves_per_eu(CW <= 40 ? MYSLAM_FAST_WAVES_PER_EU : 3))) MYSLAM_FAST_VGPR_ATTR void k_fast_strip(OrbPlan P, const uint8_t* __restrict__ pyr, size_t pyrStride,
                                                     const uint8_t* __restrict__ maskPyr,
-                                                    uint32_t* __restrict__ cand, int32_t* __restrict__ candCount, FastCtl ctl, int batch) {
+                                                    uint32_t* __restrict__ cand, int32_t* __restrict__ stripCount, FastCtl ctl, int batch) {
     constexpr int T = 256;
     constexpr int CP = (CW + 6 + 15) & ~15;
     constexpr int TP = G * CP;
@@ -903,7 +903,7 @@
     __shared__ uint16_t s_pairs[NPAIR];
     static_assert(NLIST * 5 <= TROWS * TP, "maxima list must fit into the staged tile");
     static_assert(NLIST * 4 <= TROWS * TP && NLIST <= NPAIR, "row records must fit");
-    __shared__ int s_ini2[NB2][G], s_wc2[NB2][G], s_cnt2[NB2][4];
+    __shared__ int s_ini2[NB2][G], s_wc2[NB2][G], s_cnt2[NB2][6];
     static_assert(FastLds<CW, G, CH, NS>::CP == CP && FastLds<CW, G, CH, NS>::TROWS == TROWS && FastLds<CW, G, CH, NS>::SP == SP && FastLds<CW, G, CH, NS>::SROWS == SROWS && FastLds<CW, G, CH, NS>::NPAIR == NPAIR,
                   "FastLds restates this kernel's LDS arrays");
 
@@ -936,7 +936,7 @@
         const int level = (int)(r.t[0] & 0xffu), hr = (int)(r.t[1] >> 16), iniY = (int)(r.t[1] & 0xffffu), iniX0 = (int)(r.t[2] & 0xffffu), wCell = (int)(r.t[2] >> 16);
         const bool ext = level == 0 && r.b < a_ext0N;
         const uint8_t* img = (const uint8_t*)(ext ? a_ext0 + (size_t)r.b * a_ext0Stride : a_pyr + (size_t)r.b * a_pyrStride + ((size_t)r.t[6] | ((size_t)r.t[7] << 32)));
-        const int ipitch = ext ? a_ext0Pitch : (int)r.t[4];
+        const int ipitch = ext ? a_ext0Pitch : (int)((r.t[4] & 127u) << 6);
         const uint32_t lds = (uint32_t)__builtin_amdgcn_readfirstlane((int)(uint32_t)(uintptr_t)(q ? &s_dyn[0] : &s_tile0[0])) + 1024u * (uint32_t)__builtin_amdgcn_readfirstlane(tid >> 6);
 #pragma unroll
         for (int j = 0; j < (TROWS * 12 + 255) / 256; j++) {
@@ -967,14 +967,14 @@
     uint32_t* const s_recz = reinterpret_cast<uint32_t*>(s_tile);
     int* const s_ini = s_ini2[par];
     int* const s_wc = s_wc2[par];
-    int& s_nlist = s_cnt2[par][0]; int& s_npair = s_cnt2[par][1]; int& s_ncorner = s_cnt2[par][2];
+    int& s_nlist = s_cnt2[par][0]; int& s_npair = s_cnt2[par][1]; int& s_ncorner = s_cnt2[par][2]; int& s_napp = s_cnt2[par][3]; int& s_ndone = s_cnt2[par][4];
     const int b = rec.b;
     StripRec rec_next = rec;
     if constexpr (NS > 1) { if (gs + 1 < gs_end) rec_next = load_rec(gs + 1); }
     const bool sampled = gs % max(1, total_strips >> 12) == 0;
     const uint4 e0 = make_uint4(rec.t[0], rec.t[1], rec.t[2], rec.t[3]), e1 = make_uint4(rec.t[4], rec.t[5], rec.t[6], rec.t[7]);
     const int level = (int)(e0.x & 0xffu), ci = (int)((e0.x >> 8) & 0xffu), cj0 = (int)((e0.x >> 16) & 0xffu), ncell = (int)(e0.x >> 24);
-    if (ncell == 0) { rec = rec_next; if constexpr (NS > 1) { if (gs + 1 < gs_end && (rec.t[0] >> 24) != 0) { issue_tile(rec, par, tid); fresh = true; } } continue; }
+    if (ncell == 0) { if ((unsigned)tid == 0) stripCount[gs] = 0; rec = rec_next; if constexpr (NS > 1) { if (gs + 1 < gs_end && (rec.t[0] >> 24) != 0) { issue_tile(rec, par, tid); fresh = true; } } continue; }
     const int iniY = (int)(e0.y & 0xffffu), hr = (int)(e0.y >> 16), hc = hr - 6;
     const int iniX0 = (int)(e0.z & 0xffffu), t_wCell = (int)(e0.z >> 16);
     const int pairs_total = (int)e1.y;
@@ -982,7 +982,7 @@
     auto wc_of = [&](int c) __attribute__((always_inline)) -> int { return s_wc[c]; };
     const bool ext = level == 0 && b < a_ext0N;
     const uint8_t* img = (const uint8_t*)(ext ? a_ext0 + (size_t)b * a_ext0Stride : a_pyr + (size_t)b * a_pyrStride + ((size_t)e1.z | ((size_t)e1.w << 32)));
-    const int ipitch = ext ? a_ext0Pitch : (int)e1.x;
+    const int ipitch = ext ? a_ext0Pitch : (int)((e1.x & 127u) << 6);
     const LevelGeom g = P.lv[level];
     bool dense = false;
     auto prep = [&]() __attribute__((always_inline)) {
@@ -992,7 +992,7 @@
             if (NB % 16 != 0 && tid < (NB - 16 * NV) / 4) reinterpret_cast<uint32_t*>(&s_score[0][0])[4 * NV + tid] = 0;
         }
         if (tid < G) s_ini[tid] = 0;
-        if (tid == 0) { s_nlist = 0; s_npair = 0; s_ncorner = 0; }
+        if (tid == 0) { s_nlist = 0; s_npair = 0; s_ncorner = 0; s_napp = 0; s_ndone = 0; }
         {
             typedef const uint32_t __attribute__((address_space(4))) * ConstStat;
             const ConstStat pv = (ConstStat)((uintptr_t)ctl.prev + (uintptr_t)level * 16);
@@ -1333,7 +1333,7 @@
         ctl.cur[level * 4 + 2] = dense ? 1u : 0u;
     }
     const uint8_t* mimg = maskPyr ? maskPyr + (size_t)b * pyrStride + g.imgOff : nullptr;
-    uint32_t* out = cand + (size_t)b * P.totalKeyCap + g.keyOff;
+    uint32_t* out = cand + (size_t)b * P.totalKeyCap + g.keyOff + (e1.x >> 7);
     if (dense) {
         const int nrec = min(s_nlist, NLIST);
         for (int i0 = 0; i0 < nrec; i0 += T) {
@@ -1364,17 +1364,12 @@
             }
             const int total = (int)(__popcll(bm[0]) + __popcll(bm[1]));
             if (total == 0) continue;
-            int gbase = 0;
-            if (lane == 0) gbase = atomicAdd(&candCount[b * MAXL + level], total);
-            gbase = __builtin_amdgcn_readfirstlane(gbase);
-            int dst = rank_below(bm[0], rank_below(bm[1], gbase));
-            if (passk[0]) {
-                if (dst < g.keyCap) out[dst] = kp[0];
-                dst++;
-            }
-            if (passk[1]) {
-                if (dst < g.keyCap) out[dst] = kp[1];
-            }
+            int sbase = 0;
+            if (lane == 0) sbase = atomicAdd(&s_napp, total);
+            sbase = __builtin_amdgcn_readfirstlane(sbase);
+            int dst = rank_below(bm[0], rank_below(bm[1], sbase));
+            if (passk[0]) out[dst++] = kp[0];
+            if (passk[1]) out[dst] = kp[1];
         }
     } else {
     const int nl = min(s_nlist, NLIST);
@@ -1391,14 +1386,17 @@
         }
         const unsigned long long bm = __ballot(pass);
         if (bm == 0) continue;
-        int gbase = 0;
-        if (lane == 0) gbase = atomicAdd(&candCount[b * MAXL + level], __popcll(bm));
-        gbase = __builtin_amdgcn_readfirstlane(gbase);
-        if (pass) {
-            const int dst = gbase + __popcll(bm & ((1ull << lane) - 1ull));
-            if (dst < g.keyCap) out[dst] = kp;
-        }
-    }
+        int sbase = 0;
+        if (lane == 0) sbase = atomicAdd(&s_napp, (int)__popcll(bm));
+        sbase = __builtin_amdgcn_readfirstlane(sbase);
+        if (pass) out[sbase + __popcll(bm & ((1ull << lane) - 1ull))] = kp;
+    }
+    }
+    if (lane == 0) {
+        asm volatile("" ::: "memory");
+        const int arrived = atomicAdd(&s_ndone, 1);
+        asm volatile("" ::: "memory");
+        if (arrived == T / 64 - 1) stripCount[gs] = *reinterpret_cast<volatile int*>(&s_napp);
     }
     rec = rec_next; par ^= (NS > 1 ? 1 : 0);
   }
@@ -1533,7 +1531,7 @@
 constexpr int OCT_FL = 4;
 template <int OT>
 __global__ __launch_bounds__(OT) void k_octree(OrbPlan P, const uint32_t* __restrict__ cand,
-                                               const int32_t* __restrict__ candCount, uint32_t* __restrict__ sortbuf,
+                                               const int32_t* __restrict__ stripCount, uint32_t* __restrict__ sortbuf,
                                                const uint32_t* __restrict__ octTab,
                                                uint32_t* __restrict__ selOut, int32_t* __restrict__ selCount,
                                                int32_t* __restrict__ status, int NCmax, uint16_t* __restrict__ order, BlurMulti BM) {
@@ -1580,7 +1578,32 @@
     L.kk = pcur; pcur += NC;
     L.mark = pcur; pcur += NC;
 
-    const int cnt = candCount[b * MAXL + level];
+    const int ns = g.nRows * ((g.nCols + 3) >> 2);
+    int32_t* const s_scnt = reinterpret_cast<int32_t*>(s_tab);
+    uint32_t* const s_sseg = s_tab + ns;
+    uint32_t* const s_cpre = s_tab + 2 * ns;
+    uint32_t* const s_tabT = s_tab + 3 * ns + 1;
+    int cnt, nchunk;
+    {
+        const int32_t* gcnt = stripCount + (size_t)b * P.nstrips + g.stripBase;
+        const uint32_t* gtab = P.stripTab + (size_t)g.stripBase * 8 + 4;
+        const int c = (ns + OT - 1) / OT;
+        const int beg = min(ns, t * c), end = min(ns, beg + c);
+        uint64_t sum = 0;
+        for (int i = beg; i < end; i++) {
+            int k = gcnt[i];
+            const bool bad = (unsigned)k > 4u * 30u * 30u;
+            if (bad) k = 0;
+            s_scnt[i] = k; s_sseg[i] = gtab[8 * i] >> 7;
+            sum += (bad ? (uint64_t)1 << 20 : (uint64_t)k) | ((uint64_t)((k + 63) >> 6) << 40);
+        }
+        uint64_t total;
+        uint64_t run = block_excl_scan64<OT>(sum, s_w, total);
+        for (int i = beg; i < end; i++) { s_cpre[i] = (uint32_t)(run >> 40); run += (uint64_t)((s_scnt[i] + 63) >> 6) << 40; }
+        if (t == 0) s_cpre[ns] = (uint32_t)(total >> 40);
+        cnt = (int)min(total & (((uint64_t)1 << 40) - 1), (uint64_t)INT32_MAX);
+        nchunk = (int)(total >> 40);
+    }
     int32_t* myCount = selCount + b * MAXL + level;
     if (cnt > g.keyCap) {
         if (t == 0) { *myCount = 0; status[b] = MYSLAM_ERR_CAPACITY; }
@@ -1599,28 +1622,43 @@
     const uint32_t* xcode = octTab + g.tabOff; const uint32_t* ycode = xcode + g.tabX;
     const uint32_t* xcell = ycode + g.tabY; const uint32_t* ycell = xcell + g.tabX;
     const int ntab = 2 * (g.tabX + g.tabY);
-    const bool tabLds = (size_t)ntab * 4 <= (size_t)54 * NC;
+    const bool tabLds = (size_t)(3 * ns + 1 + ntab) * 4 <= (size_t)54 * NC;
     for (int i = t; i < NB; i += OT) s_cursor[i] = 0;
-    if (tabLds) for (int i = t; i < ntab; i += OT) s_tab[i] = xcode[i];
+    if (tabLds) for (int i = t; i < ntab; i += OT) s_tabT[i] = xcode[i];
     __syncthreads();
     const bool rankkey = g.nCols * g.nRows <= 1024;
     const float inv_ncols = 1.0f / (float)g.nCols;
     auto passes = [&](auto in_lds) __attribute__((always_inline)) {
         constexpr bool LDS = decltype(in_lds)::value;
         const int oyc = g.tabX, oxl = g.tabX + g.tabY, oyl = 2 * g.tabX + g.tabY;
-        auto XC = [&](uint32_t i) -> uint32_t { if constexpr (LDS) return s_tab[i]; else return xcode[i]; };
-        auto YC = [&](uint32_t i) -> uint32_t { if constexpr (LDS) return s_tab[oyc + i]; else return ycode[i]; };
-        auto XL = [&](uint32_t i) -> uint32_t { if constexpr (LDS) return s_tab[oxl + i]; else return xcell[i]; };
-        auto YL = [&](uint32_t i) -> uint32_t { if constexpr (LDS) return s_tab[oyl + i]; else return ycell[i]; };
-        for (int i0 = t; i0 < n; i0 += OCT_FL * OT) {
+        auto XC = [&](uint32_t i) -> uint32_t { if constexpr (LDS) return s_tabT[i]; else return xcode[i]; };
+        auto YC = [&](uint32_t i) -> uint32_t { if constexpr (LDS) return s_tabT[oyc + i]; else return ycode[i]; };
+        auto XL = [&](uint32_t i) -> uint32_t { if constexpr (LDS) return s_tabT[oxl + i]; else return xcell[i]; };
+        auto YL = [&](uint32_t i) -> uint32_t { if constexpr (LDS) return s_tabT[oyl + i]; else return ycell[i]; };
+        constexpr int NW = OT / 64;
+        const int lane = t & 63, wv = __builtin_amdgcn_readfirstlane(t >> 6);
+        auto fetch = [&](int k0, int& sc, uint32_t (&pay)[OCT_FL], bool (&on)[OCT_FL]) __attribute__((always_inline)) {
+#pragma unroll
+            for (int u = 0; u < OCT_FL; u++) {
+                const int k = k0 + u * NW;
+                pay[u] = 0u; on[u] = false;
+                if (k < nchunk) {
+                    while ((int)s_cpre[sc + 1] <= k) sc++;
+                    const int j = ((k - (int)s_cpre[sc]) << 6) + lane;
+                    on[u] = j < s_scnt[sc];
+                    if (on[u]) pay[u] = keys[s_sseg[sc] + j];
+                }
+            }
+        };
+        for (int k0 = wv, sc = 0; k0 < nchunk; k0 += OCT_FL * NW) {
             uint32_t pay[OCT_FL], cx[OCT_FL], cy[OCT_FL];
-#pragma unroll
-            for (int u = 0; u < OCT_FL; u++) pay[u] = (i0 + u * OT < n) ? keys[i0 + u * OT] : 0u;
+            bool on[OCT_FL];
+            fetch(k0, sc, pay, on);
 #pragma unroll
             for (int u = 0; u < OCT_FL; u++) { cx[u] = XC((pay[u] >> 8) & 0xfff); cy[u] = YC(pay[u] >> 20); }
 #pragma unroll
             for (int u = 0; u < OCT_FL; u++)
-                if (i0 + u * OT < n) atomicAdd(&s_cursor[(cx[u] | cy[u]) >> bsh], 1u);
+                if (on[u]) atomicAdd(&s_cursor[(cx[u] | cy[u]) >> bsh], 1u);
         }
         __syncthreads();
         {
@@ -1639,10 +1677,10 @@
             if (t == 0) L.offs[NB] = (uint32_t)n;
         }
         __syncthreads();
-        for (int i0 = t; i0 < n; i0 += OCT_FL * OT) {
+        for (int k0 = wv, sc = 0; k0 < nchunk; k0 += OCT_FL * NW) {
             uint32_t pay[OCT_FL], cx[OCT_FL], cy[OCT_FL], qx[OCT_FL], qy[OCT_FL];
-#pragma unroll
-            for (int u = 0; u < OCT_FL; u++) pay[u] = (i0 + u * OT < n) ? keys[i0 + u * OT] : 0u;
+            bool on[OCT_FL];
+            fetch(k0, sc, pay, on);
 #pragma unroll
             for (int u = 0; u < OCT_FL; u++) {
                 const uint32_t px = (pay[u] >> 8) & 0xfff, py = pay[u] >> 20;
@@ -1651,7 +1689,7 @@
             }
 #pragma unroll
             for (int u = 0; u < OCT_FL; u++) {
-                if (i0 + u * OT >= n) continue;
+                if (!on[u]) continue;
                 uint32_t low = pay[u];
                 if (rankkey) {
                     const int px = (int)((pay[u] >> 8) & 0xfff), py = (int)(pay[u] >> 20);
@@ -2440,13 +2478,6 @@
     if ((lane & 7) == 0) reinterpret_cast<uint32_t*>(desc + (size_t)i * 32)[lane >> 3] = w;
 }
 
-__global__ void k_unpack_cands(const uint32_t* __restrict__ cand, int n, int32_t* xs, int32_t* ys, int32_t* sc) {
-    const int i = blockIdx.x * blockDim.x + threadIdx.x;
-    if (i >= n) return;
-    const uint32_t p = cand[i];
-    xs[i] = (p >> 8) & 0xfff; ys[i] = p >> 20; sc[i] = p & 0xff;
-}
-
 struct ZeroArgs { uint32_t* p[4]; int n[4]; };
 __device__ __forceinline__ void zero_part(const ZeroArgs& z, int tid, int T) {
 #pragma unroll
@@ -2605,7 +2636,7 @@
 }
 
 void launch_fast(const OrbPlan& P, const uint8_t* pyr, size_t pyrStride, const uint8_t* maskPyr, uint32_t* cand,
-                 int32_t* candCount, const uint32_t* statPrev, uint32_t* statCur, int forceMode, int batch, hipStream_t s) {
+                 int32_t* stripCount, const uint32_t* statPrev, uint32_t* statCur, int forceMode, int batch, hipStream_t s) {
     int cw = 0, ch = 0;
     for (int l = 0; l < P.nlevels; l++) { cw = max(cw, P.lv[l].wCell); ch = max(ch, P.lv[l].hCell); }
     const FastCtl ctl{statPrev, statCur, forceMode};
@@ -2615,35 +2646,35 @@
     if (cw <= 32 && ch <= 40 && (size_t)P.nstrips * batch >= (size_t)MYSLAM_FAST_NS * 256 * 6 * 4) {
         const dim3 gridms((unsigned)(((size_t)P.nstrips * batch + MYSLAM_FAST_NS - 1) / MYSLAM_FAST_NS));
         constexpr int padms = FastLds<32, 4, 40, MYSLAM_FAST_NS>::PAD + FastLds<32, 4, 40, MYSLAM_FAST_NS>::TROWS * FastLds<32, 4, 40, MYSLAM_FAST_NS>::TP + 16;
-        hipLaunchKernelGGL((k_fast_strip<32, 4, 40, MYSLAM_FAST_NS>), gridms, dim3(256), padms, s, P, pyr, pyrStride, maskPyr, cand, candCount, ctl, batch);
+        hipLaunchKernelGGL((k_fast_strip<32, 4, 40, MYSLAM_FAST_NS>), gridms, dim3(256), padms, s, P, pyr, pyrStride, maskPyr, cand, stripCount, ctl, batch);
         return;
     }
 #endif
-    if (cw <= 32 && ch <= 40) hipLaunchKernelGGL((k_fast_strip<32, 4, 40>), grid, dim3(256), pad, s, P, pyr, pyrStride, maskPyr, cand, candCount, ctl, batch);
-    else if (max(cw, ch) <= 40) hipLaunchKernelGGL((k_fast_strip<40, 4>), grid, dim3(256), 0, s, P, pyr, pyrStride, maskPyr, cand, candCount, ctl, batch);
-    else hipLaunchKernelGGL((k_fast_strip<MAX_CELL, 4>), grid, dim3(256), 0, s, P, pyr, pyrStride, maskPyr, cand, candCount, ctl, batch);
-}
-
-size_t octree_lds_bytes(int nodeCap) { return 192 + 4 * (size_t)OT_MAXB + 4 * (size_t)(OT_MAXB + 2) + (size_t)nodeCap * 54 + 16; }
+    if (cw <= 32 && ch <= 40) hipLaunchKernelGGL((k_fast_strip<32, 4, 40>), grid, dim3(256), pad, s, P, pyr, pyrStride, maskPyr, cand, stripCount, ctl, batch);
+    else if (max(cw, ch) <= 40) hipLaunchKernelGGL((k_fast_strip<40, 4>), grid, dim3(256), 0, s, P, pyr, pyrStride, maskPyr, cand, stripCount, ctl, batch);
+    else hipLaunchKernelGGL((k_fast_strip<MAX_CELL, 4>), grid, dim3(256), 0, s, P, pyr, pyrStride, maskPyr, cand, stripCount, ctl, batch);
+}
+
+size_t octree_lds_bytes(int nodeCap, int nstrips) { return 192 + 4 * (size_t)OT_MAXB + 4 * (size_t)(OT_MAXB + 2) + std::max((size_t)nodeCap * 54, (size_t)nstrips * 12 + 4) + 16; }
 
 bool blur_multi_for_octree(const BlurArgs* lv, int n, int batch, BlurMulti& M);
-bool launch_octree(const OrbPlan& P, const uint32_t* cand, const int32_t* candCount, uint32_t* sortbuf, const uint32_t* octTab, uint32_t* selOut,
+bool launch_octree(const OrbPlan& P, const uint32_t* cand, const int32_t* stripCount, uint32_t* sortbuf, const uint32_t* octTab, uint32_t* selOut,
                    int32_t* selCount, int32_t* status, int batch, uint16_t* order, hipStream_t s, const BlurArgs* blurLv, int nBlur) {
     BlurMulti BMh;
     const BlurMulti* blurWith = (blurLv && nBlur > 0 && blur_multi_for_octree(blurLv, nBlur, batch, BMh)) ? &BMh : nullptr;
-    int ncmax = 0;
-    for (int l = 0; l < P.nlevels; l++) ncmax = max(ncmax, P.lv[l].nodeCap);
-    const size_t lds = std::max(octree_lds_bytes(ncmax), (size_t)8 * 16 * B3_TS);
+    int ncmax = 0, nsmax = 0;
+    for (int l = 0; l < P.nlevels; l++) { ncmax = max(ncmax, P.lv[l].nodeCap); nsmax = max(nsmax, P.lv[l].nRows * ((P.lv[l].nCols + 3) / 4)); }
+    const size_t lds = std::max(octree_lds_bytes(ncmax, nsmax), (size_t)8 * 16 * B3_TS);
     (void)hipFuncSetAttribute(reinterpret_cast<const void*>(k_octree<256>), hipFuncAttributeMaxDynamicSharedMemorySize, 160 * 1024);
     (void)hipFuncSetAttribute(reinterpret_cast<const void*>(k_octree<512>), hipFuncAttributeMaxDynamicSharedMemorySize, 160 * 1024);
     if (batch >= OCT_WIDE_BELOW)
-        hipLaunchKernelGGL(k_octree<256>, dim3(batch, P.nlevels), dim3(256), lds, s, P, cand, candCount, sortbuf, octTab, selOut, selCount, status, ncmax, order, BlurMulti{});
+        hipLaunchKernelGGL(k_octree<256>, dim3(batch, P.nlevels), dim3(256), lds, s, P, cand, stripCount, sortbuf, octTab, selOut, selCount, status, ncmax, order, BlurMulti{});
     else
     {
         BlurMulti M = blurWith ? *blurWith : BlurMulti{};
         if (!blurWith) M.n = 0;
         const int brows = blurWith ? (M.wave0[M.n] + 7) / 8 : 0;
-        hipLaunchKernelGGL(k_octree<512>, dim3(batch, P.nlevels + brows), dim3(512), lds, s, P, cand, candCount, sortbuf, octTab, selOut, selCount, status, ncmax, order, M);
+        hipLaunchKernelGGL(k_octree<512>, dim3(batch, P.nlevels + brows), dim3(512), lds, s, P, cand, stripCount, sortbuf, octTab, selOut, selCount, status, ncmax, order, M);
     }
     return blurWith != nullptr;
 }
@@ -2672,11 +2703,6 @@
     hipLaunchKernelGGL(k_calc_desc, dim3((n + 3) / 4), dim3(256), 0, s, P, blur, kps, n, desc);
 }
 
-void launch_unpack_cands(const uint32_t* cand, int n, int32_t* xs, int32_t* ys, int32_t* sc, hipStream_t s) {
-    if (n <= 0) return;
-    hipLaunchKernelGGL(k_unpack_cands, dim3((n + 255) / 256), dim3(256), 0, s, cand, n, xs, ys, sc);
-}
-
 }
 
 #ifdef MYSLAM_BLOCK_TRACE
diff --git a/a-simple-stereo-slam-system-with-deep-loop-closing_amd/csrc/orb_plan.h b/a-simple-stereo-slam-system-with-deep-loop-closing_amd/csrc/orb_plan.h
--- a/a-simple-stereo-slam-system-with-deep-loop-closing_amd/csrc/orb_plan.h
+++ b/a-simple-stereo-slam-system-with-deep-loop-closing_amd/csrc/orb_plan.h
@@ -25,6 +25,7 @@
     int sortDepth;
     int ndepth;
     int keyCap;
+    int candCap;
     int nodeCap;
     int outBase;
     float scale;
```

Result: no change. 79620 (median of 2 runs) (+0.5%).
